# xarray-contrib/xeofs

Measured on AMD Instinct MI355X. Metric: EOF randomized-SVD GB/s (algorithmic: 16 passes x n x p x 4 B per fit / fit time), higher is better.
Workload: dtype f32 data, split-fp16 MFMA (f16x3+f16x3), f32 accumulate

## Files before the change

xeofs_amd/csrc/eofx_abi.hip:

```cpp
#include <chrono>
#include "eofx_hfft.hpp"
#include "eofx_kernels.hpp"
#include "eofx_fit.hpp"
#include "eofx_gram.hpp"
#include "eofx_axb_dma.hpp"
#include "eofx_hosteig.hpp"
#include "eofx_hostla.hpp"
#include "eofx_lag.hpp"
#include "eofx_gw.hpp"
#include "eofx_spca.hpp"
#include "eofx_lagcov.hpp"
#include "eofx_lowpass.hpp"
#include "eofx_orderpos.hpp"
#include "eofx_colquad.hpp"
#include "eofx_pairmin.hpp"
#include "eofx_simplex.hpp"
#include "eofx_kmeans.hpp"
#include "eofx_ica.hpp"
#include "eofx_spectral.hpp"
#include "eofx_pcmul.hpp"
#include "eofx_viewcov.hpp"
#include "eofx_lrfill.hpp"
#include "eofx_plans.hpp"
#include "eofx_sketch.hpp"
// ... 536 lines not shown
  const int bx = (int)(M / ATB_BM);
  const bool wide = atb_wide(L) && prec == EOFX_PREC_F16X3;
  if (sym && !(wide && !aff && L == M)) sym = 0;
  const ColTiles tiles = atb_tiles(L, wide);
  const AtbPlan plan = atb_plan(M, K, L, wide);
  int best_s = plan.S;
  int64_t best_kps = plan.kps;
  ArenaScope scope(ctx);
  float* out = C;
  const int s_half = best_s;
  if (A2) best_s *= 2;
  if (best_s > 1) {
    out = arena_alloc<float>(ctx, (size_t)best_s * M * L);
    if (!out && A2) return set_err(ctx, EOFX_ERR_NOMEM, "arena exhausted (two-matrix partials)");
    if (!out) {
      best_s = 1;
      best_kps = K;
      out = C;
    }
  }
  float a_scale = 1.f;
  if (prec == EOFX_PREC_F16X3) {
    if (a_absmax > 0.f && std::isfinite(a_absmax)) {
      int e;
      (void)std::frexp(a_absmax, &e);
      a_scale = std::ldexp(1.f, 14 - e);
    }
    if (!b_absmax_dev && ldb == L && !A2) b_absmax_dev = amax_get(ctx, B);
    if (!b_absmax_dev) {
      unsigned* bm = arena_alloc<unsigned>(ctx, 1);
      if (!bm) return set_err(ctx, EOFX_ERR_NOMEM, "arena exhausted (panel max)");
      HIPCHK(hipMemsetAsync(bm, 0, sizeof(unsigned), ctx->stream));
      const int64_t total4 = K * (L / 4);
      hipLaunchKernelGGL(panel_absmax_kernel, dim3((int)std::max<int64_t>(1, std::min<int64_t>((total4 + 1023) / 1024, 1024))),
                         dim3(256), 0, ctx->stream, B, K, L, (int64_t)ldb, bm);
      KCHK();
      b_absmax_dev = reinterpret_cast<const float*>(bm);
    }
  }
  unsigned* amax_out = (prec == EOFX_PREC_F16X3 && !sym && !wide && !A2) ? amax_new(ctx, C) : (amax_forget(ctx, C), nullptr);
  hipEvent_t ev0 = nullptr, ev1 = nullptr;
  if (ctx->profile) {
    HIPCHK(hipEventCreate(&ev0));
    HIPCHK(hipEventCreate(&ev1));
    HIPCHK(hipEventRecord(ev0, ctx->stream));
  }
  if (prec == EOFX_PREC_F64) {
    double* outd = nullptr;
    if (best_s > 1) {
      outd = arena_alloc<double>(ctx, (size_t)best_s * M * L);
      if (!outd) return set_err(ctx, EOFX_ERR_NOMEM, "arena exhausted (float64 partials)");
    }
    for (int i = 0; i < tiles.n; ++i) {
      const ColTile& t = tiles.t[i];
      if (t.width == 64)
        hipLaunchKernelGGL(atb_f64_kernel<2>, dim3(bx, best_s, t.count), dim3(512), 0, ctx->stream, A, lda, B, ldb, C, outd, L, M, K,
                           best_kps, t.col_base);
      else
        hipLaunchKernelGGL(atb_f64_kernel<1>, dim3(bx, best_s, t.count), dim3(512), 0, ctx->stream, A, lda, B, ldb, C, outd, L, M, K,
                           best_kps, t.col_base);
      KCHK();
    }
    if (ctx->profile) {
      HIPCHK(hipEventRecord(ev1, ctx->stream));
      ctx->prof_events.emplace_back(ev0, ev1);
      ctx->prof_flops += 2.0 * (double)K * (double)M * (double)L;
      ctx->prof_bytes += (double)K * (double)M * 4.0 * tiles.columns();
    }
    if (outd) {
      const int64_t count = M * L;
      hipLaunchKernelGGL(splitk_reduce_f64_kernel, dim3((int)std::min<int64_t>((count + 255) / 256, 8192)), dim3(256), 0, ctx->stream,
                         outd, C, count, best_s);
      KCHK();
    }
    return EOFX_OK;
  }
  unsigned* amax_direct = best_s == 1 ? amax_out : nullptr;
  PlaneOut po_{nullptr, 0, 0.f};
  const PlaneOut* po = nullptr;
  if (planes && aff && !sym && !A2 && best_s == 1 && amax_direct && planes->bound > 0.f && std::isfinite(planes->bound)) {
    const int64_t K_all = round_up(aff->cols, AXB_KG);
    if (K_all <= M && axb_planes_reserve(ctx, axb_planes_bytes(K_all, L))) {
      po_ = {ctx->axb_planes, K_all, planes->bound};
      po = &po_;
      if (L % 64)
        HIPCHK(hipMemsetAsync(reinterpret_cast<char*>(ctx->axb_planes) + (size_t)(L / 64) * (K_all / AXB_KG) * AXB_PAIR_BYTES, 0,
                              (size_t)(K_all / AXB_KG) * AXB_PAIR_BYTES, ctx->stream));
      if (!planes->keep_f32 && !plane_check_on(ctx)) out = nullptr;
    }
  }
  for (int i = 0; i < tiles.n; ++i) {
    const ColTile& t = tiles.t[i];
    const dim3 grid(bx, best_s, t.count);
    if (t.width >= 96)
      launch_atb_variant<4>(prec, grid, ctx->stream, A, lda, B, ldb, out, L, M, K, best_kps, t.col_base, a_scale, b_absmax_dev, aff, A2, B2, s_half,
                            sym, amax_direct, t.width, po);
    else if (t.width == 64)
      launch_atb_variant<2>(prec, grid, ctx->stream, A, lda, B, ldb, out, L, M, K, best_kps, t.col_base, a_scale, b_absmax_dev, aff, A2, B2, s_half,
                            sym, amax_direct, 128, po);
    else
      launch_atb_variant<1>(prec, grid, ctx->stream, A, lda, B, ldb, out, L, M, K, best_kps, t.col_base, a_scale, b_absmax_dev, aff, A2, B2, s_half,
                            sym, amax_direct, 128, po);
    KCHK();
  }
  if (po) {
    ctx->planes_known.panel = C;
    ctx->planes_known.L = L;
    ctx->planes_known.K_all = po->rows;
    ctx->planes_known.bound = po->bound;
    ctx->planes_known.f32 = out != nullptr;
    ++ctx->plane_produced[0];
  }
  if (ctx->profile) {
    HIPCHK(hipEventRecord(ev1, ctx->stream));
    ctx->prof_events.emplace_back(ev0, ev1);
    ctx->prof_flops += 2.0 * (double)K * (double)M * (double)L * (A2 ? 2 : 1);
    ctx->prof_bytes += (double)K * (double)M * 4.0 * tiles.columns() * (A2 ? 2 : 1);
  }
  if (best_s > 1) {
    const int64_t count4 = M * L / 4;
    const int blocks = (int)std::min<int64_t>((count4 + 255) / 256, amax_out ? 2048 : 4096);
    hipLaunchKernelGGL(splitk_reduce_kernel, dim3(blocks), dim3(256), 0, ctx->stream, out, C, count4,
                       best_s, amax_out);
    KCHK();
  }
  if (sym) {
    const int nt = (int)((M + 63) / 64);
    hipLaunchKernelGGL(symmetrize_lower_kernel, dim3(nt, nt), dim3(256), 0, ctx->stream, C, M, (int64_t)L);
    KCHK();
  }
  return EOFX_OK;
}


static bool axb_takes_dma(eofx_ctx* ctx, int64_t rows_pad, int64_t K_all) {
  if (ctx->axb_dma < 0) {
    const char* ev = std::getenv("EOFX_AXB_DMA");
    ctx->axb_dma = ev ? (atoi(ev) != 0 ? 2 : 0) : EOFX_AXB_DMA_DEFAULT;
  }
  return ctx->axb_dma == 2 || (ctx->axb_dma == 1 && (double)rows_pad * (double)K_all >= 4.0e9);
}
static bool axb_planes_reserve(eofx_ctx* ctx, size_t need) {
  if (ctx->axb_planes_bytes >= need) return true;
  (void)hipStreamSynchronize(ctx->stream);
  if (ctx->axb_planes) (void)hipFree(ctx->axb_planes);
  ctx->axb_planes = nullptr;
  ctx->axb_planes_bytes = 0;
  ctx->planes_known = {};
  if (hipMalloc((void**)&ctx->axb_planes, need) != hipSuccess) {
    (void)hipGetLastError();
    ctx->axb_planes = nullptr;
    return false;
  }
  ctx->axb_planes_bytes = need;
  return true;
}
static bool plane_check_on(eofx_ctx* ctx) {
  if (ctx->plane_check < 0) {
    const char* ev = std::getenv("EOFX_AXB_CHECK_BOUND");
    ctx->plane_check = ev ? atoi(ev) : 0;
  }
  return ctx->plane_check >= 1;
}
static int plane_bound_check(eofx_ctx* ctx, const float* Y, int64_t K_all, int L, float bound) {
  ArenaScope scope(ctx);
  unsigned* bm = arena_alloc<unsigned>(ctx, 1);
  if (!bm) return set_err(ctx, EOFX_ERR_NOMEM, "arena exhausted (panel max)");
  HIPCHK(hipMemsetAsync(bm, 0, sizeof(unsigned), ctx->stream));
  const int64_t total4 = K_all * (L / 4);
  hipLaunchKernelGGL(panel_absmax_kernel, dim3((int)std::max<int64_t>(1, std::min<int64_t>((total4 + 1023) / 1024, 1024))),
                     dim3(256), 0, ctx->stream, Y, K_all, L, (int64_t)L, bm);
  KCHK();
  float mx = 0.f;
  HIPCHK(hipMemcpyAsync(&mx, bm, sizeof(float), hipMemcpyDeviceToHost, ctx->stream));
  HIPCHK(hipStreamSynchronize(ctx->stream));
  ++ctx->plane_checked;
  if (ctx->plane_check >= 2) fprintf(stderr, "eofx: X Y pass over produced planes: bound %g, max |panel| %g, bound / max %g\n", (double)bound, (double)mx, mx > 0.f ? (double)bound / (double)mx : 0.0);
  if (!(mx <= bound)) return set_err(ctx, EOFX_ERR_LINALG, "panel maximum %g above the bound %g its fp16 planes were split with", (double)mx, (double)bound);
  if (mx > 0.f) {
    const double slack = (double)bound / (double)mx;
    if (ctx->plane_min_slack == 0.0 || slack < ctx->plane_min_slack) ctx->plane_min_slack = slack;
    if (slack > ctx->plane_max_slack) ctx->plane_max_slack = slack;
  }
  return EOFX_OK;
}

static int launch_axb(eofx_ctx* ctx, const float* raw, int64_t ld, int64_t rows, int64_t cols, int64_t rows_pad,
                      const float* aff, int64_t aff_ld, float a_absmax, const float* Y, int L, float* W, bool masked = false,
                      const int* act = nullptr, int64_t n_act = 0) {
  const int64_t K_all = round_up(cols, AXB_KG);
  const int64_t K = (masked && act) ? n_act * AXB_KG : K_all;
  if (K == 0) {
    HIPCHK(hipMemsetAsync(W, 0, sizeof(float) * (size_t)rows_pad * L, ctx->stream));
    amax_forget(ctx, W);
    return EOFX_OK;
  }
  if (L % 32 || L <= 0 || rows_pad % AXB_BM || rows >= ((int64_t)1 << 31) || K_all * L >= ((int64_t)1 << 30) ||
      64 * ld + K_all >= ((int64_t)1 << 30))
    return set_err(ctx, EOFX_ERR_ARG, "axb: bad geometry rows=%lld cols=%lld L=%d", (long long)rows, (long long)cols, L);
  const AtbPlan plan = axb_plan(rows_pad, K);
  const int rt = (int)(rows_pad / AXB_BM);
  const ColTiles tiles = atb_tiles(L, false);
  ArenaScope scope(ctx);
  float* out = W;
  if (plan.S > 1) {
    out = arena_alloc<float>(ctx, (size_t)plan.S * rows_pad * L);
    if (!out) return set_err(ctx, EOFX_ERR_NOMEM, "arena exhausted (in-place product partials)");
  }
  float a_scale = 1.f;
  if (a_absmax > 0.f && std::isfinite(a_absmax)) {
    int e;
    (void)std::frexp(a_absmax, &e);
    a_scale = std::ldexp(1.f, 14 - e);
  }
  const float* bmax = amax_get(ctx, Y);
  if (!bmax) {
    unsigned* bm = arena_alloc<unsigned>(ctx, 1);
    if (!bm) return set_err(ctx, EOFX_ERR_NOMEM, "arena exhausted (panel max)");
    HIPCHK(hipMemsetAsync(bm, 0, sizeof(unsigned), ctx->stream));
    const int64_t total4 = K_all * (L / 4);
    hipLaunchKernelGGL(panel_absmax_kernel, dim3((int)std::max<int64_t>(1, std::min<int64_t>((total4 + 1023) / 1024, 1024))),
                       dim3(256), 0, ctx->stream, Y, K_all, L, (int64_t)L, bm);
    KCHK();
    bmax = reinterpret_cast<const float*>(bm);
  }
  unsigned* amax_out = plan.S > 1 ? amax_new(ctx, W) : (amax_forget(ctx, W), nullptr);
  hipEvent_t ev0 = nullptr, ev1 = nullptr;
  if (ctx->profile) {
    HIPCHK(hipEventCreate(&ev0));
    HIPCHK(hipEventCreate(&ev1));
    HIPCHK(hipEventRecord(ev0, ctx->stream));
  }
  const int gx = plan.S > 1 ? 8 * rt * ((plan.S + 7) / 8) : rt;
  bool dma = axb_takes_dma(ctx, rows_pad, K_all);
  const int ncb = tiles.columns();
  if (dma && !axb_planes_reserve(ctx, axb_planes_bytes(K_all, L))) dma = false;
  const int64_t pairs_all = K_all / AXB_KG;
  const eofx_ctx::PlanesKnown& pk = ctx->planes_known;
  const bool produced = dma && pk.panel == Y && pk.L == L && pk.K_all == K_all && amax_get(ctx, Y) == bmax;
  if (produced) {
    ++ctx->plane_consumed;
    if (pk.f32 && plane_check_on(ctx)) CHK(plane_bound_check(ctx, Y, K_all, L, pk.bound));
  } else if (pk.panel == Y && !pk.f32) {
    return set_err(ctx, EOFX_ERR_ARG, "axb: the panel exists as fp16 planes only and they cannot be used here");
  }
  if (dma && !produced) {
    ctx->planes_known = {};
    hipLaunchKernelGGL(axb_bsplit_kernel, dim3((unsigned)((K_all + 31) / 32), ncb), dim3(256), 0, ctx->stream, Y, L, L, K_all, bmax,
                       ctx->axb_planes);
    KCHK();
  }
  const int* const no_act = nullptr;
  for (int i = 0; i < tiles.n; ++i) {
    const ColTile& t = tiles.t[i];
    const dim3 grid(gx, t.count);
#define EOFX_AXB_ARGS(B, LDB) \
  grid, dim3(256), 0, ctx->stream, raw, ld, (int)rows, cols, aff, aff_ld, B, LDB, out, L, rows_pad, K, plan.kps, plan.S, rt, t.col_base, a_scale, bmax
    if (dma) {
      if (t.width == 64) {
        if (masked) hipLaunchKernelGGL((axb_f16_dma_kernel<4, 0, true>), EOFX_AXB_ARGS(ctx->axb_planes, pairs_all), act);
        else hipLaunchKernelGGL((axb_f16_dma_kernel<4, 0, false>), EOFX_AXB_ARGS(ctx->axb_planes, pairs_all), no_act);
      } else {
        if (masked) hipLaunchKernelGGL((axb_f16_dma_kernel<2, 0, true>), EOFX_AXB_ARGS(ctx->axb_planes, pairs_all), act);
        else hipLaunchKernelGGL((axb_f16_dma_kernel<2, 0, false>), EOFX_AXB_ARGS(ctx->axb_planes, pairs_all), no_act);
      }
    } else if (t.width == 64) {
      if (masked) hipLaunchKernelGGL((axb_f16_kernel<4, 0, true>), EOFX_AXB_ARGS(Y, L), act);
      else hipLaunchKernelGGL(axb_f16_kernel<4>, EOFX_AXB_ARGS(Y, L));
    } else {
      if (masked) hipLaunchKernelGGL((axb_f16_kernel<2, 0, true>), EOFX_AXB_ARGS(Y, L), act);
      else hipLaunchKernelGGL(axb_f16_kernel<2>, EOFX_AXB_ARGS(Y, L));
    }
#undef EOFX_AXB_ARGS
    KCHK();
  }
  if (ctx->profile) {
    HIPCHK(hipEventRecord(ev1, ctx->stream));
    ctx->prof_events.emplace_back(ev0, ev1, 1);
    ctx->prof_flops += 2.0 * (double)K * (double)rows_pad * (double)L;
    ctx->prof_bytes += (double)K * (double)rows * 4.0 * tiles.columns();
  }
  if (plan.S > 1) {
    const int64_t count4 = rows_pad * L / 4;
    hipLaunchKernelGGL(splitk_reduce_kernel, dim3((int)std::min<int64_t>((count4 + 255) / 256, amax_out ? 2048 : 4096)), dim3(256), 0,
                       ctx->stream, out, W, count4, plan.S, amax_out);
    KCHK();
  }
  return EOFX_OK;
}

static int launch_gram(eofx_ctx* ctx, const float* P, int64_t rows, int L, double* G) {
  const int nb = (L + 63) / 64;
  const int nbx = gram_parts(rows, L);
  ArenaScope scope(ctx);
  ARENA(double, part, (size_t)nbx * L * L);
  hipLaunchKernelGGL(gram_mfma_kernel, dim3(nbx, nb * nb), dim3(256), 0, ctx->stream, P, rows, L, part);
  KCHK();
  const int64_t count = (int64_t)L * L;
  hipLaunchKernelGGL(f64_reduce_kernel, dim3((int)((count + 63) / 64)), dim3(256), 0, ctx->stream,
                     part, G, count, nbx);
  KCHK();
  return EOFX_OK;
}
static int launch_matmul(eofx_ctx* ctx, const float* P, int64_t rows, int L, const double* Mx, int Lo,
                         float* out, bool upper = false, int64_t planes_rows = 0, float planes_bound = 0.f) {
  int KW = (int)std::min<int64_t>(round_up(L, 64), 256);
  if (L > 256) {
    static const int kw_env = std::getenv("EOFX_PMM_KW") ? atoi(std::getenv("EOFX_PMM_KW")) : 0;
    if (kw_env == 128 || kw_env == 256) KW = kw_env;
  }
  const size_t smem = (size_t)KW * PMM_LD * sizeof(double);
  if (smem > 64 * 1024)
    HIPCHK(hipFuncSetAttribute(reinterpret_cast<const void*>(panel_matmul_kernel<false>), hipFuncAttributeMaxDynamicSharedMemorySize, (int)smem));
  const int64_t units = (rows + 127) / 128;
  const int64_t gx = L <= KW ? std::min<int64_t>(units, 1024) : units;
  dim3 grid((int)std::max<int64_t>(1, gx), (Lo + 63) / 64);
  unsigned* amax_out = amax_new(ctx, out);
  if (planes_rows > 0 && Lo == L && amax_out && planes_rows % AXB_KG == 0 && planes_rows <= rows && rows % 8 == 0 && planes_bound > 0.f &&
      std::isfinite(planes_bound) && axb_planes_reserve(ctx, axb_planes_bytes(planes_rows, Lo))) {
    if (smem > 64 * 1024)
      HIPCHK(hipFuncSetAttribute(reinterpret_cast<const void*>(panel_matmul_kernel<false, true>), hipFuncAttributeMaxDynamicSharedMemorySize,
                                 (int)smem));
    hipLaunchKernelGGL((panel_matmul_kernel<false, true>), grid, dim3(256), smem, ctx->stream, P, rows, L, Mx, Lo, out, KW, amax_out,
                       (int64_t)0, (int64_t)0, 1, (const float*)nullptr, upper ? 1 : 0, ctx->axb_planes, planes_rows, planes_bound);
    KCHK();
    ctx->planes_known.panel = out;
    ctx->planes_known.L = Lo;
    ctx->planes_known.K_all = planes_rows;
    ctx->planes_known.bound = planes_bound;
    ctx->planes_known.f32 = true;
    ++ctx->plane_produced[1];
    return EOFX_OK;
  }
  hipLaunchKernelGGL(panel_matmul_kernel<false>, grid, dim3(256), smem, ctx->stream, P, rows, L, Mx, Lo, out, KW, amax_out,
                     (int64_t)0, (int64_t)0, 1, (const float*)nullptr, upper ? 1 : 0);
  KCHK();
  return EOFX_OK;
}
static int launch_matmul_gen(eofx_ctx* ctx, const float* P, int64_t ldp, int64_t slab, int cpb, int64_t rows, int L, const double* Mx, int Lo,
                             const float* sub, float* out) {
  const int KW = (int)std::min<int64_t>(round_up(L, 64), 256);
  const size_t smem = (size_t)KW * PMM_LD * sizeof(double);
  if (smem > 64 * 1024)
    HIPCHK(hipFuncSetAttribute(reinterpret_cast<const void*>(panel_matmul_kernel<true>), hipFuncAttributeMaxDynamicSharedMemorySize, (int)smem));
  const int64_t units = (rows + 127) / 128;
  const int64_t gx = L <= KW ? std::min<int64_t>(units, 1024) : units;
  dim3 grid((int)std::max<int64_t>(1, gx), (Lo + 63) / 64);
  hipLaunchKernelGGL(panel_matmul_kernel<true>, grid, dim3(256), smem, ctx->stream, P, rows, L, Mx, Lo, out, KW, amax_new(ctx, out), ldp,
                     slab, cpb, sub);
  KCHK();
  return EOFX_OK;
}
static int launch_xgram(eofx_ctx* ctx, const float* Pa, int64_t lda, int La, const float* Pb, int64_t ldb, int Lb, int64_t rows, double* C) {
  const int nbx = (int)std::max<int64_t>(1, std::min<int64_t>((rows + 127) / 128, std::max<int64_t>(1, ((int64_t)32 << 20) / ((int64_t)La * Lb * 8))));
  ArenaScope scope(ctx);
  ARENA(double, part, (size_t)nbx * La * Lb);
  hipLaunchKernelGGL(xgram_mfma_kernel, dim3(nbx, (La / 64) * (Lb / 64)), dim3(256), 0, ctx->stream, Pa, lda, Pb, ldb, rows, La, Lb, part);
  KCHK();
  const int64_t count = (int64_t)La * Lb;
  hipLaunchKernelGGL(f64_reduce_kernel, dim3((int)((count + 63) / 64)), dim3(256), 0, ctx->stream, part, C, count, nbx);
  KCHK();
  return EOFX_OK;
}

static int launch_rinv(eofx_ctx* ctx, const double* G, int L, int l, double* Rinv);
static size_t matmul_nt_scratch(eofx_ctx* ctx, int64_t rows, int L, int Lo);
static int launch_matmul_nt(eofx_ctx* ctx, const float* P, int64_t rows, int L, const double* Mx, int Lo, float* out);
constexpr float EOFX_CHOLQR_BOUND = 2.f;
static int launch_cholqr(eofx_ctx* ctx, const float* P, int64_t rows, int L, int l, const double* G,
                         float* out, int64_t planes_rows = 0) {
  ArenaScope scope(ctx);
  ARENA(double, Rinv, (size_t)L * L);
  CHK(launch_rinv(ctx, G, L, l, Rinv));
  return launch_matmul(ctx, P, rows, L, Rinv, L, out, true, planes_rows, EOFX_CHOLQR_BOUND);
}

static int launch_colminmax(eofx_ctx* ctx, const float* P, int64_t rows, int L, float* mx, float* mn) {
  const int nparts = (int)std::max<int64_t>(1, std::min<int64_t>((rows + 127) / 128, 1024));
  ArenaScope scope(ctx);
  ARENA(float, pmx, (size_t)nparts * L);
  ARENA(float, pmn, (size_t)nparts * L);
  hipLaunchKernelGGL(colminmax_part_kernel, dim3(nparts, (L + 63) / 64), dim3(256), 0, ctx->stream, P,
                     rows, L, pmx, pmn);
  KCHK();
  hipLaunchKernelGGL(colminmax_final_kernel, dim3((L + 63) / 64), dim3(256), 0, ctx->stream, pmx, pmn,
                     nparts, L, mx, mn);
  KCHK();
  return EOFX_OK;
}

static int export_panel(eofx_ctx* ctx, const float* P, int64_t rows, int L, int k, const double* sign,
                        float* dst) {
  if (!dst) return EOFX_OK;
  ArenaScope scope(ctx);
  double* dsign = nullptr;
  if (sign) {
    dsign = arena_alloc<double>(ctx, k);
    if (!dsign) return set_err(ctx, EOFX_ERR_NOMEM, "arena exhausted (export sign)");
    CHK(copy_in(ctx, dsign, sign, sizeof(double) * k));
  }
  float* tmp = dst;
  const bool dev = is_device_ptr(dst);
  if (!dev) {
    tmp = arena_alloc<float>(ctx, (size_t)rows * k);
    if (!tmp) return set_err(ctx, EOFX_ERR_NOMEM, "arena exhausted (export staging)");
  }
  const int64_t total = rows * k;
  const int blocks = (int)std::min<int64_t>((total + 255) / 256, 8192);
  hipLaunchKernelGGL(panel_export_kernel, dim3(blocks), dim3(256), 0, ctx->stream, P, rows, L, k, dsign,
                     tmp);
  KCHK();
  if (!dev) {
    CHK(copy_out(ctx, dst, tmp, sizeof(float) * total));
    HIPCHK(hipStreamSynchronize(ctx->stream));
  }
  return EOFX_OK;
}

static int import_panel(eofx_ctx* ctx, const float* src, int64_t rows, int l, float* P, int64_t rows_pad,
                        int L) {
  ArenaScope scope(ctx);
  const float* dsrc = src;
  if (!is_device_ptr(src)) {
    float* tmp = arena_alloc<float>(ctx, (size_t)rows * l);
    if (!tmp) return set_err(ctx, EOFX_ERR_NOMEM, "arena exhausted (import staging)");
    CHK(copy_in(ctx, tmp, src, sizeof(float) * rows * l));
    dsrc = tmp;
  }
  const int64_t total = rows_pad * (L / 4);
  const int blocks = (int)std::min<int64_t>((total + 255) / 256, 2048);
  hipLaunchKernelGGL(panel_import_kernel, dim3(blocks), dim3(256), 0, ctx->stream, dsrc, rows, l, P,
                     rows_pad, L, amax_new(ctx, P));
  KCHK();
  if (dsrc != src) HIPCHK(hipStreamSynchronize(ctx->stream));
  return EOFX_OK;
}

static void* pool_take(eofx_ctx* ctx, size_t bytes) {
  for (size_t i = 0; i < ctx->pool.size(); ++i)
    if (ctx->pool[i].second == bytes) {
      void* p = ctx->pool[i].first;
      ctx->pool_bytes -= bytes;
      ctx->pool.erase(ctx->pool.begin() + i);
      return p;
    }
  return nullptr;
}
static void pool_trim(eofx_ctx* ctx) {
  if (ctx->pool.empty()) return;
  (void)hipStreamSynchronize(ctx->stream);
  for (auto& e : ctx->pool) (void)hipFree(e.first);
  ctx->pool.clear();
  ctx->pool_bytes = 0;
}
static void pool_give(eofx_ctx* ctx, void* p, size_t bytes) {
  if (!p) return;
  if (!ctx || bytes > ctx->pool_cap) {
    (void)hipFree(p);
    return;
  }
  constexpr size_t POOL_MAX_ENTRIES = 48, POOL_EVICT_BATCH = 12;
  if (!ctx->pool.empty() && (ctx->pool_bytes + bytes > ctx->pool_cap || ctx->pool.size() >= POOL_MAX_ENTRIES)) {
    (void)hipStreamSynchronize(ctx->stream);
    size_t evicted = 0;
    while (!ctx->pool.empty() && (evicted < POOL_EVICT_BATCH || ctx->pool_bytes + bytes > ctx->pool_cap)) {
      (void)hipFree(ctx->pool.front().first);
      ctx->pool_bytes -= ctx->pool.front().second;
      ctx->pool.erase(ctx->pool.begin());
      ++evicted;
    }
  }
  ctx->pool.emplace_back(p, bytes);
  ctx->pool_bytes += bytes;
}
static hipError_t pool_malloc(eofx_ctx* ctx, void** out, size_t bytes) {
  *out = pool_take(ctx, bytes);
  if (*out) return hipSuccess;
  hipError_t e = hipMalloc(out, bytes);
  if (e != hipSuccess && !ctx->pool.empty()) {
    (void)hipGetLastError();
    pool_trim(ctx);
    e = hipMalloc(out, bytes);
  }
  return e;
}
extern "C" int eofx_ctx_trim(eofx_ctx* ctx) {
  if (!ctx) return EOFX_ERR_ARG;
  (void)hipSetDevice(ctx->device);
  pool_trim(ctx);
  if (ctx->axb_planes) {
    (void)hipStreamSynchronize(ctx->stream);
    (void)hipFree(ctx->axb_planes);
    ctx->axb_planes = nullptr;
    ctx->axb_planes_bytes = 0;
    ctx->planes_known = {};
  }
  return EOFX_OK;
}

static int mat_alloc(eofx_ctx* ctx, int64_t n, int64_t p, eofx_mat** out, bool want_x = true, bool want_xt = true) {
  eofx_mat* m = new eofx_mat();
  m->n = n;
  m->p = p;
  m->n_pad = round_up(n, ATB_BM);
  m->p_pad = round_up(p, ATB_BM);
  const size_t bytes = (size_t)m->n_pad * m->p_pad * sizeof(float);
  hipError_t e = want_x ? pool_malloc(ctx, (void**)&m->X, bytes) : hipSuccess;
  if (e == hipSuccess && want_xt) e = pool_malloc(ctx, (void**)&m->Xt, bytes);
  if (e == hipSuccess) e = pool_malloc(ctx, (void**)&m->absmax_dev, 256);
  if (e == hipSuccess) e = hipMemsetAsync(m->absmax_dev, 0, 256, ctx->stream);
  if (e != hipSuccess) {
    if (m->X) (void)hipFree(m->X);
    if (m->Xt) (void)hipFree(m->Xt);
    delete m;
    (void)hipGetLastError();
    return set_err(ctx, EOFX_ERR_NOMEM, "cannot allocate resident matrix %lld x %lld (2 x %.2f GB): %s",
                   (long long)n, (long long)p, bytes / 1e9, hipGetErrorString(e));
  }
  *out = m;
  return EOFX_OK;
}

extern "C" int eofx_mat_destroy(eofx_ctx* ctx, eofx_mat* m) {
  if (!m) return EOFX_OK;
  const size_t bytes = (size_t)m->n_pad * m->p_pad * sizeof(float);
  if (ctx) {
    (void)hipSetDevice(ctx->device);
    (void)hipStreamSynchronize(ctx->stream);
    if (m->X) pool_give(ctx, m->X, bytes);
    if (m->Xt) pool_give(ctx, m->Xt, bytes);
    if (m->act) pool_give(ctx, m->act, sizeof(int) * (size_t)(round_up(m->p, AXB_KG) / AXB_KG));
    pool_give(ctx, m->absmax_dev, 256);
    if (m->raw_owned) pool_give(ctx, m->raw_owned, m->raw_owned_bytes);
    if (m->rawT) pool_give(ctx, m->rawT, bytes);
  } else {
    if (m->X) (void)hipFree(m->X);
    if (m->Xt) (void)hipFree(m->Xt);
    if (m->act) (void)hipFree(m->act);
    if (m->raw_owned) (void)hipFree(m->raw_owned);
    if (m->rawT) (void)hipFree(m->rawT);
  }
  if (m->aff) {
    const size_t abytes = sizeof(float) * 3 * (size_t)m->p_pad;
    if (ctx) pool_give(ctx, m->aff, abytes);
    else (void)hipFree(m->aff);
  }
  delete m;
  return EOFX_OK;
}
extern "C" int eofx_mat_shape(const eofx_mat* m, int64_t* n, int64_t* p, int64_t* n_pad, int64_t* p_pad) {
  if (!m) return EOFX_ERR_ARG;
  if (n) *n = m->n;
  if (p) *p = m->p;
  if (n_pad) *n_pad = m->n_pad;
  if (p_pad) *p_pad = m->p_pad;
  return EOFX_OK;
}

struct Staged {
  const float* dev = nullptr;
  float* owned = nullptr;
  ~Staged() {
    if (owned) (void)hipFree(owned);
  }
};
static int stage_input(eofx_ctx* ctx, const float* X, size_t count, Staged& st) {
  if (is_device_ptr(X)) {
    st.dev = X;
    return EOFX_OK;
  }
  HIPCHK(hipMalloc((void**)&st.owned, count * sizeof(float)));
  HIPCHK(hipMemcpyAsync(st.owned, X, count * sizeof(float), hipMemcpyHostToDevice, ctx->stream));
  st.dev = st.owned;
  return EOFX_OK;
}

static void adopt_staged(eofx_mat** out, Staged& st, size_t bytes) {
  if (out && *out && (*out)->raw && (*out)->raw == st.owned) {
    (*out)->raw_owned = st.owned;
    (*out)->raw_owned_bytes = bytes;
    st.owned = nullptr;
  }
}

static int launch_apply(eofx_ctx* ctx, const float* Xsrc, int64_t ld_src, const int64_t* row_map,
                        const int64_t* col_map, const double* shift, const double* scale, eofx_mat* m,
                        int* nan_flag, const unsigned* absmax_src = nullptr) {
  dim3 grid((int)(m->p_pad / 64), (int)(m->n_pad / 64));
  const bool vec = apply_vec(col_map != nullptr, ld_src, (uintptr_t)Xsrc % 16 == 0);
  if (vec)
    hipLaunchKernelGGL(apply_kernel<true>, grid, dim3(256), 0, ctx->stream, Xsrc, ld_src, row_map, col_map,
                       shift, scale, m->n, m->p, m->X, m->p_pad, m->Xt, m->n_pad, nan_flag, (const float*)nullptr, (int64_t)0);
  else
    hipLaunchKernelGGL(apply_kernel<false>, grid, dim3(256), 0, ctx->stream, Xsrc, ld_src, row_map, col_map,
                       shift, scale, m->n, m->p, m->X, m->p_pad, m->Xt, m->n_pad, nan_flag, (const float*)nullptr, (int64_t)0);
  KCHK();
  if (absmax_src) {
    HIPCHK(hipMemcpyAsync(m->absmax_dev, absmax_src, sizeof(unsigned), hipMemcpyDeviceToDevice, ctx->stream));
  } else {
    const int64_t total4 = m->n_pad * (m->p_pad / 4);
    hipLaunchKernelGGL(panel_absmax_kernel, dim3((int)std::max<int64_t>(1, std::min<int64_t>((total4 + 1023) / 1024, 1024))), dim3(256), 0,
                       ctx->stream, m->Xt, m->p_pad, (int)m->n_pad, m->n_pad, m->absmax_dev);
    KCHK();
  }
  HIPCHK(hipMemcpyAsync(&m->absmax, m->absmax_dev, sizeof(float), hipMemcpyDeviceToHost, ctx->stream));
  return EOFX_OK;
}

static int ensure_Xt(eofx_ctx* ctx, const eofx_mat* cm) {
  eofx_mat* m = const_cast<eofx_mat*>(cm);
  if (m->Xt) return EOFX_OK;
  if (!m->X && !(m->raw && m->aff)) return set_err(ctx, EOFX_ERR_ARG, "matrix holds no data (raw field released?)");
  const size_t bytes = (size_t)m->n_pad * m->p_pad * sizeof(float);
  if (pool_malloc(ctx, (void**)&m->Xt, bytes) != hipSuccess) {
    (void)hipGetLastError();
    m->Xt = nullptr;
    return set_err(ctx, EOFX_ERR_NOMEM, "cannot allocate the sample-contiguous layout (%.2f GB)", bytes / 1e9);
  }
  if (m->X) {
    hipLaunchKernelGGL(transpose_kernel, dim3((int)(m->p_pad / 64), (int)(m->n_pad / 64)), dim3(256), 0, ctx->stream, m->X,
                       m->p_pad, m->Xt, m->n_pad);
  } else {
    hipLaunchKernelGGL(apply_kernel<true>, dim3((int)(m->p_pad / 64), (int)(m->n_pad / 64)), dim3(256), 0, ctx->stream, m->raw,
                       m->raw_ld, (const int64_t*)nullptr, (const int64_t*)nullptr, (const double*)nullptr, (const double*)nullptr,
                       m->n, m->p, (float*)nullptr, m->p_pad, m->Xt, m->n_pad, (int*)nullptr, (const float*)m->aff, m->p_pad);
  }
  KCHK();
  return EOFX_OK;
}
static int ensure_X(eofx_ctx* ctx, const eofx_mat* cm) {
  eofx_mat* m = const_cast<eofx_mat*>(cm);
  if (m->X) return EOFX_OK;
  CHK(ensure_Xt(ctx, m));
  const size_t bytes = (size_t)m->n_pad * m->p_pad * sizeof(float);
  if (pool_malloc(ctx, (void**)&m->X, bytes) != hipSuccess) {
    (void)hipGetLastError();
    m->X = nullptr;
    return set_err(ctx, EOFX_ERR_NOMEM, "cannot allocate the feature-contiguous layout (%.2f GB)", bytes / 1e9);
  }
  hipLaunchKernelGGL(transpose_kernel, dim3((int)(m->n_pad / 64), (int)(m->p_pad / 64)), dim3(256), 0, ctx->stream, m->Xt,
                     m->n_pad, m->X, m->p_pad);
  KCHK();
  return EOFX_OK;
}
extern "C" int eofx_ctx_set_layout(eofx_ctx* ctx, int keep_raw) {
  if (!ctx || keep_raw < 0 || keep_raw > 3) return EOFX_ERR_ARG;
  ctx->allow_masked = keep_raw == 3;
  if (keep_raw == 3) keep_raw = 2;
  ctx->keep_raw = keep_raw;
  return EOFX_OK;
}
extern "C" int eofx_ctx_set_sample_raw(eofx_ctx* ctx, int on) {
  if (!ctx) return EOFX_ERR_ARG;
  ctx->want_rawT = on != 0;
  return EOFX_OK;
}
extern "C" int eofx_mat_release_raw(eofx_ctx* ctx, eofx_mat* m) {
  if (!ctx || !m) return set_err(ctx, EOFX_ERR_ARG, "bad argument");
  ENTER(ctx);
  if (m->raw && !m->Xt && !m->X) CHK(ensure_Xt(ctx, m));
  HIPCHK(hipStreamSynchronize(ctx->stream));
  if (m->raw_owned) pool_give(ctx, m->raw_owned, m->raw_owned_bytes);
  m->raw_owned = nullptr;
  m->raw_owned_bytes = 0;
  m->raw = nullptr;
  return EOFX_OK;
}
extern "C" int eofx_mat_ensure_sample_layout(eofx_ctx* ctx, eofx_mat* m, int only_if_room, int* built) {
  if (!ctx || !m) return set_err(ctx, EOFX_ERR_ARG, "bad argument");
  ENTER(ctx);
  if (built) *built = m->Xt != nullptr;
  if (m->Xt || m->masked) return EOFX_OK;
  if (only_if_room) {
    size_t free_b = 0, total_b = 0;
    const size_t need_b = (size_t)m->n_pad * m->p_pad * sizeof(float);
    if (hipMemGetInfo(&free_b, &total_b) != hipSuccess) {
      (void)hipGetLastError();
      return EOFX_OK;
    }
    if (free_b + ctx->pool_bytes <= need_b + need_b / 2 + ((size_t)8 << 30)) return EOFX_OK;
  }
  CHK(ensure_Xt(ctx, m));
  if (built) *built = 1;
  return EOFX_OK;
}
extern "C" int eofx_mat_release_sample_layout(eofx_ctx* ctx, eofx_mat* m) {
  if (!ctx || !m) return set_err(ctx, EOFX_ERR_ARG, "bad argument");
// ... 372 lines not shown
  if (n_out) *n_out = ns;
  return EOFX_OK;
}

extern "C" int eofx_resample_f32(eofx_ctx* ctx, const eofx_mat* src, const int64_t* rows, int64_t n_rows,
                                 int center, eofx_mat** out, double* mean, double* total_variance) {
  if (!ctx || !src || !rows || !out || n_rows <= 0) return set_err(ctx, EOFX_ERR_ARG, "bad argument");
  ENTER(ctx);
  for (int64_t i = 0; i < n_rows; ++i)
    if (rows[i] < 0 || rows[i] >= src->n)
      return set_err(ctx, EOFX_ERR_ARG, "row index %lld out of range [0, %lld)", (long long)rows[i], (long long)src->n);
  const int64_t P = src->p;
  CHK(arena_reserve(ctx, colstats_scratch(n_rows, P)));
  ArenaScope scope(ctx);
  PreState ps;
  ARENA(int, cnt, P);
  ARENA(double, dmean, P);
  ARENA(double, dstd, P);
  ARENA(double, dshift, P);
  ARENA(double, dscale, P);
  ARENA(double, dm2, P);
  ARENA(unsigned, dabsmax, 1);
  ARENA(int64_t, drows, n_rows);
  ps = {cnt, dmean, dstd, dshift, dscale, dm2, dabsmax};
  CHK(copy_in(ctx, drows, rows, sizeof(int64_t) * n_rows));
  CHK(ensure_X(ctx, src));
  CHK(run_colstats(ctx, src->X, n_rows, P, center, 0, nullptr, ps, src->p_pad, drows));
  eofx_mat* m = nullptr;
  CHK(mat_alloc(ctx, n_rows, P, &m));
  ARENA(int, flag, 1);
  HIPCHK(hipMemsetAsync(flag, 0, sizeof(int), ctx->stream));
  int rc = launch_apply(ctx, src->X, src->p_pad, drows, nullptr, ps.shift, ps.scale, m, flag, ps.absmax);
  if (rc == EOFX_OK && mean)
    if (hipMemcpyAsync(mean, ps.mean, sizeof(double) * P, hipMemcpyDeviceToHost, ctx->stream) != hipSuccess) rc = EOFX_ERR_HIP;
  if (rc == EOFX_OK && total_variance) {
    FeatSummary fs;
    rc = run_feature_summary(ctx, ps, P, fs);
    if (rc == EOFX_OK) *total_variance = fs.tv;
  }
  if (rc == EOFX_OK && hipStreamSynchronize(ctx->stream) != hipSuccess) rc = EOFX_ERR_HIP;
  if (rc != EOFX_OK) {
    eofx_mat_destroy(ctx, m);
    return rc == EOFX_ERR_HIP ? set_err(ctx, EOFX_ERR_HIP, "resample: HIP failure") : rc;
  }
  *out = m;
  return EOFX_OK;
}

static bool tmul_nt_ok(const eofx_mat* m, int L);
static size_t tmul_nt_scratch(eofx_ctx* ctx, const eofx_mat* m, int L);
static int mat_tmul_nt(eofx_ctx* ctx, const eofx_mat* m, const float* Zn, float* Yp, int L);
static int panel_tmul(eofx_ctx* ctx, const eofx_mat* m, const float* Zn, float* Yp, int L, int prec, const PlaneReq* planes = nullptr) {
  if (prec == EOFX_PREC_F16X3 && tmul_nt_ok(m, L) && tmul_nt_scratch(ctx, m, L) > 0 &&
      ctx->arena_size - ctx->arena_off >= tmul_nt_scratch(ctx, m, L))
    return mat_tmul_nt(ctx, m, Zn, Yp, L);
  if (!m->X && m->raw && prec == EOFX_PREC_F16X3) {
    AffView av;
    av.aff = m->aff;
    av.ld = m->p_pad;
    av.rows = (int)m->n;
    av.cols = m->p;
    av.masked = m->masked;
    return launch_atb(ctx, m->raw, m->raw_ld, round_up(m->n, ATB_KG), m->p_pad, Zn, L, L, Yp, prec, m->absmax, nullptr, &av, nullptr, nullptr, 0,
                      planes);
  }
  CHK(ensure_X(ctx, m));
  return launch_atb(ctx, m->X, m->p_pad, round_up(m->n, ATB_KG), m->p_pad, Zn, L, L, Yp, prec, m->absmax);
}
static int ensure_active_pairs(eofx_ctx* ctx, const eofx_mat* cm) {
  eofx_mat* m = const_cast<eofx_mat*>(cm);
  if (!m->masked || m->n_act >= 0 || !m->aff) return EOFX_OK;
  const int64_t npairs = round_up(m->p, AXB_KG) / AXB_KG;
  std::vector<float> sc((size_t)m->p_pad);
  HIPCHK(hipMemcpyAsync(sc.data(), m->aff + 2 * m->p_pad, sizeof(float) * (size_t)m->p_pad, hipMemcpyDeviceToHost, ctx->stream));
  HIPCHK(hipStreamSynchronize(ctx->stream));
  std::vector<int> list;
  list.reserve((size_t)npairs);
  for (int64_t q = 0; q < npairs; ++q) {
    bool any = false;
    for (int64_t c = q * AXB_KG; c < std::min<int64_t>((q + 1) * AXB_KG, m->p) && !any; ++c) any = sc[(size_t)c] != 0.f;
    if (any) list.push_back((int)q);
  }
  m->n_act = (int64_t)list.size();
  if (m->n_act == npairs || m->n_act == 0) return EOFX_OK;
  if (pool_malloc(ctx, (void**)&m->act, sizeof(int) * (size_t)npairs) != hipSuccess) {
    (void)hipGetLastError();
    m->act = nullptr;
    return EOFX_OK;
  }
  HIPCHK(hipMemcpyAsync(m->act, list.data(), sizeof(int) * list.size(), hipMemcpyHostToDevice, ctx->stream));
  HIPCHK(hipStreamSynchronize(ctx->stream));
  return EOFX_OK;
}

static int64_t panel_mul_plane_rows(eofx_ctx* ctx, const eofx_mat* m, int L, int prec) {
  if (m->Xt || !m->raw || !m->aff || prec != EOFX_PREC_F16X3) return 0;
  if (!m->masked && L >= 96 && !std::getenv("EOFX_NO_WIDE_XT")) return 0;
  const int64_t K_all = round_up(m->p, AXB_KG);
  if (K_all * (int64_t)L >= ((int64_t)1 << 30) || 64 * m->raw_ld + K_all >= ((int64_t)1 << 30)) return 0;
  return axb_takes_dma(ctx, m->n_pad, K_all) ? K_all : 0;
}
static bool panel_tmul_plane_req(eofx_ctx* ctx, const eofx_mat* m, int L, int prec, bool keep_f32, PlaneReq* req) {
  if (m->X || panel_mul_plane_rows(ctx, m, L, prec) == 0) return false;
  const float bound = 2.f * std::sqrt((float)m->n) * m->absmax;
  if (!(bound > 0.f) || !std::isfinite(bound)) return false;
  req->bound = bound;
  req->keep_f32 = keep_f32;
  return true;
}
static int panel_mul(eofx_ctx* ctx, const eofx_mat* m, const float* Yp, float* Wn, int L, int prec) {
  if (!m->Xt && m->raw && m->aff && !m->masked && prec == EOFX_PREC_F16X3 && L >= 96 && !std::getenv("EOFX_NO_WIDE_XT")) {
    size_t free_b = 0, total_b = 0;
    const size_t need_b = (size_t)m->n_pad * m->p_pad * sizeof(float);
    if (hipMemGetInfo(&free_b, &total_b) == hipSuccess && free_b + ctx->pool_bytes > need_b + need_b / 2 + ((size_t)8 << 30))
      CHK(ensure_Xt(ctx, m));
    else
      (void)hipGetLastError();
  }
  if (!m->Xt && m->raw && m->aff && prec == EOFX_PREC_F16X3 &&
      round_up(m->p, AXB_KG) * (int64_t)L < ((int64_t)1 << 30) &&
      64 * m->raw_ld + round_up(m->p, AXB_KG) < ((int64_t)1 << 30)) {
    CHK(ensure_active_pairs(ctx, m));
    return launch_axb(ctx, m->raw, m->raw_ld, m->n, m->p, m->n_pad, m->aff, m->p_pad, m->absmax, Yp, L, Wn, m->masked, m->act,
                      m->n_act);
  }
  CHK(ensure_Xt(ctx, m));
  return launch_atb(ctx, m->Xt, m->n_pad, round_up(m->p, ATB_KG), m->n_pad, Yp, L, L, Wn, prec, m->absmax);
}
static bool valid_prec(int p) {
  return p == EOFX_PREC_F32 || p == EOFX_PREC_BF16X3 || p == EOFX_PREC_BF16X6 || p == EOFX_PREC_F16X3 || p == EOFX_PREC_F64;
}

extern "C" int eofx_ctx_set_precision(eofx_ctx* ctx, int power_passes, int final_passes) {
  if (!ctx || !valid_prec(power_passes) || !valid_prec(final_passes)) return set_err(ctx, EOFX_ERR_ARG, "bad precision");
  ctx->prec_power = power_passes;
  ctx->prec_final = final_passes;
  return EOFX_OK;
}

extern "C" int eofx_panel_tmul_f32(eofx_ctx* ctx, const eofx_mat* m, const float* Zn, float* Yp, int L,
                                   int prec) {
  if (!ctx || !m || !Zn || !Yp || !valid_prec(prec)) return set_err(ctx, EOFX_ERR_ARG, "bad argument");
  ENTER(ctx);
  size_t need = atb_scratch_bytes(m->p_pad, round_up(m->n, ATB_KG), L);
  if (prec == EOFX_PREC_F16X3 && tmul_nt_ok(m, L)) need = std::max(need, tmul_nt_scratch(ctx, m, L));
  CHK(arena_reserve(ctx, need));
  return panel_tmul(ctx, m, Zn, Yp, L, prec);
}
extern "C" int eofx_panel_mul_f32(eofx_ctx* ctx, const eofx_mat* m, const float* Yp, float* Wn, int L,
                                  int prec) {
  if (!ctx || !m || !Wn || !Yp || !valid_prec(prec)) return set_err(ctx, EOFX_ERR_ARG, "bad argument");
  ENTER(ctx);
  CHK(arena_reserve(ctx, atb_scratch_bytes(m->n_pad, round_up(m->p, ATB_KG), L)));
  return panel_mul(ctx, m, Yp, Wn, L, prec);
}
extern "C" int eofx_ctx_plane_stats(eofx_ctx* ctx, int64_t* counts4, double* slack2) {
  if (!ctx) return EOFX_ERR_ARG;
  if (counts4) {
    counts4[0] = ctx->plane_produced[0];
    counts4[1] = ctx->plane_produced[1];
    counts4[2] = ctx->plane_consumed;
    counts4[3] = ctx->plane_checked;
  }
  if (slack2) {
    slack2[0] = ctx->plane_min_slack;
    slack2[1] = ctx->plane_max_slack;
  }
  ctx->plane_produced[0] = ctx->plane_produced[1] = ctx->plane_consumed = ctx->plane_checked = 0;
  ctx->plane_min_slack = ctx->plane_max_slack = 0.0;
  return EOFX_OK;
}
extern "C" int eofx_axb_planes_probe_f32(eofx_ctx* ctx, const eofx_mat* m, const float* Zn, int L, int producer, float bound,
                                         void* planes_prod, void* planes_split, size_t plane_bytes, float* w_prod, float* w_split,
                                         float* w_reg, float* w_max, float* y_out, float* bound_out) {
  if (!ctx || !m || !Zn || !planes_prod || !planes_split || !w_prod || !w_split || !w_reg || !w_max || L <= 0 || L % 32 ||
      (producer != 0 && producer != 1))
    return set_err(ctx, EOFX_ERR_ARG, "bad argument");
  ENTER(ctx);
  const int prec = EOFX_PREC_F16X3;
  const int64_t K_all = panel_mul_plane_rows(ctx, m, L, prec);
  if (K_all == 0 || m->X) return set_err(ctx, EOFX_ERR_ARG, "planes probe: the matrix does not take the in-place LDS-DMA route");
  if (plane_bytes != axb_planes_bytes(K_all, L)) return set_err(ctx, EOFX_ERR_ARG, "planes probe: plane_bytes");
  CHK(arena_reserve(ctx, 2 * (size_t)m->p_pad * L * sizeof(float) + 4 * (size_t)L * L * sizeof(double) + (size_t)(4 * gram_parts(m->p_pad, L) + 1) * L * L * sizeof(double) +
                             std::max(atb_scratch_bytes(m->p_pad, round_up(m->n, ATB_KG), L), atb_scratch_bytes(m->n_pad, K_all, L)) + 65536));
  ArenaScope scope(ctx);
  AmaxScope amax_scope(ctx);
  ARENA(float, Y0, (size_t)m->p_pad * L);
  ARENA(float, Y1, (size_t)m->p_pad * L);
  ARENA(double, G, (size_t)L * L);
  float* Y = Y0;
  PlaneReq req;
  if (producer == 0) {
    if (!panel_tmul_plane_req(ctx, m, L, prec, true, &req)) return set_err(ctx, EOFX_ERR_ARG, "planes probe: no request");
    if (bound > 0.f) req.bound = bound;
    CHK(panel_tmul(ctx, m, Zn, Y0, L, prec, &req));
  } else {
    CHK(panel_tmul(ctx, m, Zn, Y0, L, prec));
    CHK(launch_gram(ctx, Y0, m->p_pad, L, G));
    if (bound > 0.f) {
      ArenaScope inner(ctx);
      ARENA(double, Rinv, (size_t)L * L);
      CHK(launch_rinv(ctx, G, L, L, Rinv));
      CHK(launch_matmul(ctx, Y0, m->p_pad, L, Rinv, L, Y1, true, K_all, bound));
    } else {
      CHK(launch_cholqr(ctx, Y0, m->p_pad, L, L, G, Y1, K_all));
    }
    Y = Y1;
  }
  const eofx_ctx::PlanesKnown pk = ctx->planes_known;
  if (pk.panel != Y || pk.K_all != K_all || pk.L != L) return set_err(ctx, EOFX_ERR_ARG, "planes probe: the producer wrote no planes");
  if (bound_out) *bound_out = pk.bound;
  HIPCHK(hipMemcpyAsync(planes_prod, ctx->axb_planes, plane_bytes, hipMemcpyDeviceToHost, ctx->stream));
  if (y_out) HIPCHK(hipMemcpyAsync(y_out, Y, sizeof(float) * (size_t)m->p_pad * L, hipMemcpyDeviceToDevice, ctx->stream));
  CHK(panel_mul(ctx, m, Y, w_prod, L, prec));
  if (ctx->planes_known.panel != Y) return set_err(ctx, EOFX_ERR_ARG, "planes probe: the planes were not taken as written");
  ctx->planes_known = {};
  HIPCHK(hipMemsetAsync(ctx->axb_planes, 0xff, plane_bytes, ctx->stream));
  CHK(panel_mul(ctx, m, Y, w_split, L, prec));
  HIPCHK(hipMemcpyAsync(planes_split, ctx->axb_planes, plane_bytes, hipMemcpyDeviceToHost, ctx->stream));
  const int dma_mode = ctx->axb_dma;
  ctx->axb_dma = 0;
  int rc = panel_mul(ctx, m, Y, w_reg, L, prec);
  if (rc == EOFX_OK) {
    amax_forget(ctx, Y);
    rc = panel_mul(ctx, m, Y, w_max, L, prec);
  }
  ctx->axb_dma = dma_mode;
  if (rc != EOFX_OK) return rc;
  HIPCHK(hipStreamSynchronize(ctx->stream));
  return EOFX_OK;
}
extern "C" int eofx_panel_gram_f64(eofx_ctx* ctx, const float* P, int64_t rows_pad, int L, double* G) {
  if (!ctx || !P || !G || L % 32) return set_err(ctx, EOFX_ERR_ARG, "bad argument");
  ENTER(ctx);
  CHK(arena_reserve(ctx, (size_t)(4 * gram_parts(rows_pad, L) + 1) * L * L * sizeof(double)));
  return launch_gram(ctx, P, rows_pad, L, G);
}
extern "C" int eofx_panel_cholqr_f32(eofx_ctx* ctx, const float* P, int64_t rows_pad, int L, int l,
                                     const double* G, float* out) {
  if (!ctx || !P || !G || !out || P == out) return set_err(ctx, EOFX_ERR_ARG, "bad argument");
  ENTER(ctx);
  CHK(arena_reserve(ctx, (size_t)2 * L * L * sizeof(double) + (l > 64 ? rinv_blocked_bytes(l) : 0)));
  return launch_cholqr(ctx, P, rows_pad, L, l, G, out);
}
extern "C" int eofx_panel_rinv_f64(eofx_ctx* ctx, const double* G, int L, int l, double* Rinv) {
  if (!ctx || !G || !Rinv || L <= 0 || l <= 0 || l > L || G == Rinv) return set_err(ctx, EOFX_ERR_ARG, "bad argument");
  ENTER(ctx);
  if (l > 64) CHK(arena_reserve(ctx, rinv_blocked_bytes(l)));
  return launch_rinv(ctx, G, L, l, Rinv);
}
extern "C" int eofx_panel_matmul_f32(eofx_ctx* ctx, const float* P, int64_t rows_pad, int L,
                                     const double* M, int Lo, float* out) {
  if (!ctx || !P || !M || !out || P == out) return set_err(ctx, EOFX_ERR_ARG, "bad argument");
  ENTER(ctx);
  if (matmul_nt_ok(rows_pad, L, Lo)) {
    const size_t need = matmul_nt_scratch(ctx, rows_pad, L, Lo);
    if (need && arena_reserve(ctx, need) == EOFX_OK) return launch_matmul_nt(ctx, P, rows_pad, L, M, Lo, out);
  }
  return launch_matmul(ctx, P, rows_pad, L, M, Lo, out);
}
extern "C" int eofx_panel_colminmax_f32(eofx_ctx* ctx, const float* P, int64_t rows, int L, float* mx,
                                        float* mn) {
  if (!ctx || !P || !mx || !mn) return set_err(ctx, EOFX_ERR_ARG, "bad argument");
  if (L <= 0 || L % 4 || rows < 0)
    return set_err(ctx, EOFX_ERR_ARG, "colminmax: L=%d must be a positive multiple of 4, rows=%lld non-negative", L, (long long)rows);
  ENTER(ctx);
  CHK(arena_reserve(ctx, (size_t)2 * 1024 * L * sizeof(float) + 4096));
  return launch_colminmax(ctx, P, rows, L, mx, mn);
}
extern "C" int eofx_panel_export_f32(eofx_ctx* ctx, const float* P, int64_t rows, int L, int k,
                                     const double* sign, float* dst) {
  if (!ctx || !P || !dst || k > L) return set_err(ctx, EOFX_ERR_ARG, "bad argument");
  ENTER(ctx);
  CHK(arena_reserve(ctx, (size_t)rows * k * sizeof(float) + 8192));
  return export_panel(ctx, P, rows, L, k, sign, dst);
}
extern "C" int eofx_panel_import_f32(eofx_ctx* ctx, const float* src, int64_t rows, int l, float* P,
                                     int64_t rows_pad, int L) {
  if (!ctx || !P || !src || l > L || rows > rows_pad) return set_err(ctx, EOFX_ERR_ARG, "bad argument");
  if (L <= 0 || L % 4 || l < 0 || rows < 0)
    return set_err(ctx, EOFX_ERR_ARG, "import: L=%d must be a positive multiple of 4, l=%d and rows=%lld non-negative", L, l, (long long)rows);
  ENTER(ctx);
  CHK(arena_reserve(ctx, (size_t)rows * l * sizeof(float) + 8192));
  return import_panel(ctx, src, rows, l, P, rows_pad, L);
}

struct LinOp {
  int64_t tall, small, tall_pad, small_pad;
  std::function<int(const float*, float*, int, int)> fwd;
  std::function<int(const float*, float*, int, int)> bwd;
  std::function<int(const float*, float*, int, int, bool)> fwd_to_bwd;
  std::function<int64_t(int, int)> bwd_plane_rows;
  std::function<int(double*, int64_t)> reduce_tall_gram;
  std::function<int(double*, int64_t)> reduce_small_gram;
  int64_t rule_tall_pad = 0;
};

struct RsvdOut {
  float* Tvec;
  float* Svec;
  int Lo;
  std::vector<double> s;
  int64_t tall_pad = 0, small_pad = 0;
};

extern "C" int eofx_orth_tall_rule(int64_t tall_rows_pad, int L, int prec_power) {
  return orth_tall_rule(tall_rows_pad, L, prec_power) ? 1 : 0;
}
extern "C" int eofx_peaked_spectrum(const double* G, int ld, int l) {
  if (!G || l <= 0) return 0;
  std::vector<double> A((size_t)l * l), w(l), V((size_t)l * l);
  for (int i = 0; i < l; ++i)
    for (int j = 0; j < l; ++j) A[(size_t)i * l + j] = 0.5 * (G[(size_t)i * ld + j] + G[(size_t)j * ld + i]);
  for (double v : A)
    if (!std::isfinite(v)) return 0;
  if (eofx_host_eigh_f64(A.data(), l, w.data(), V.data()) != EOFX_OK) return 1;
  if (!(w[0] > 0.0)) return 0;
  return hostla::peaked_spectrum(w.data(), l) ? 1 : 0;
}

static int launch_rinv_blocked(eofx_ctx* ctx, const double* G, int L, int l, double* Rinv) {
  const int Lb = (int)round_up(l, 64), nb = Lb / 64;
  ArenaScope scope(ctx);
  ARENA(double, S, (size_t)Lb * Lb);
  ARENA(double, X, (size_t)Lb * Lb);
  ARENA(double, T, (size_t)Lb * Lb / 2 + 64 * 64);
  ARENA(double, d0, Lb);
  hipLaunchKernelGGL(chol_blocked_init_kernel, dim3(512), dim3(256), 0, ctx->stream, G, L, l, S, Lb, d0);
  KCHK();
  HIPCHK(hipMemsetAsync(X, 0, sizeof(double) * (size_t)Lb * Lb, ctx->stream));
  for (int j = 0; j < nb; ++j) {
    const int64_t dj = (int64_t)64 * j * Lb + 64 * j;
    const int lj = std::min(64, l - 64 * j);
    hipLaunchKernelGGL(chol_rinv_kernel, dim3(1), dim3(256), 0, ctx->stream, (const double*)(S + dj), Lb, lj, X + dj, 1e-13,
                       (const double*)(d0 + 64 * j));
    KCHK();
    const int rest = nb - 1 - j;
    if (rest > 0) {
      double* row = S + dj + 64;
      hipLaunchKernelGGL(dgemm64_kernel<true>, dim3(rest, 1), dim3(256), 0, ctx->stream, (const double*)(X + dj), Lb,
                         (const double*)row, Lb, row, Lb, 64, 1.0, 0.0, 0);
      KCHK();
      double* trail = S + dj + (int64_t)64 * Lb + 64;
      hipLaunchKernelGGL(dgemm64_kernel<true>, dim3(rest, rest), dim3(256), 0, ctx->stream, (const double*)row, Lb,
                         (const double*)row, Lb, trail, Lb, 64, -1.0, 1.0, 1);
      KCHK();
    }
  }
  {
    std::vector<int> seg((size_t)nb, 1);
    while (seg.size() > 1) {
      std::vector<int> next;
      const size_t npairs = seg.size() / 2;
      bool uniform = true;
      for (size_t i = 0; i < 2 * npairs; ++i) uniform = uniform && seg[i] == seg[0];
      auto merge = [&](int64_t off, int m1, int m2, int batch, int64_t diag_stride) {
        hipLaunchKernelGGL(dgemm64_kernel<false>, dim3(m2 / 64, m1 / 64, batch), dim3(256), 0, ctx->stream,
                           (const double*)(S + off * Lb + off + m1), Lb, (const double*)(X + (off + m1) * Lb + off + m1), Lb, T, m2, m2, 1.0,
                           0.0, 0, diag_stride, diag_stride, (int64_t)m1 * m2);
        hipLaunchKernelGGL(dgemm64_kernel<false>, dim3(m2 / 64, m1 / 64, batch), dim3(256), 0, ctx->stream,
                           (const double*)(X + off * Lb + off), Lb, (const double*)T, m2, X + off * Lb + off + m1, Lb, m1, -1.0, 0.0, 0,
                           diag_stride, (int64_t)m1 * m2, diag_stride);
      };
      if (uniform && npairs > 0) {
        const int m = 64 * seg[0];
        merge(0, m, m, (int)npairs, (int64_t)2 * m * (Lb + 1));
        KCHK();
        for (size_t i = 0; i < npairs; ++i) next.push_back(2 * seg[0]);
      } else {
        int64_t off = 0;
        for (size_t i = 0; i < npairs; ++i) {
          const int m1 = 64 * seg[2 * i], m2 = 64 * seg[2 * i + 1];
          merge(off, m1, m2, 1, 0);
          KCHK();
          off += m1 + m2;
          next.push_back(seg[2 * i] + seg[2 * i + 1]);
        }
      }
      if (seg.size() & 1) next.push_back(seg.back());
      seg.swap(next);
    }
  }
  hipLaunchKernelGGL(chol_blocked_export_kernel, dim3(512), dim3(256), 0, ctx->stream, (const double*)X, Lb, l, Rinv, L);
  KCHK();
  return EOFX_OK;
}
static int launch_rinv(eofx_ctx* ctx, const double* G, int L, int l, double* Rinv) {
  if (l <= 64) {
    if (L > 64) HIPCHK(hipMemsetAsync(Rinv, 0, sizeof(double) * (size_t)L * L, ctx->stream));
    hipLaunchKernelGGL(chol_rinv_kernel, dim3(1), dim3(256), 0, ctx->stream, G, L, l, Rinv, 1e-13, (const double*)nullptr);
    KCHK();
  } else if (ctx->arena_size - ctx->arena_off >= rinv_blocked_bytes(l) && !std::getenv("EOFX_HOST_RINV")) {
    CHK(launch_rinv_blocked(ctx, G, L, l, Rinv));
  } else {
    std::vector<double> hG((size_t)L * L), hR((size_t)L * L);
    HIPCHK(hipMemcpyAsync(hG.data(), G, sizeof(double) * L * L, hipMemcpyDeviceToHost, ctx->stream));
    HIPCHK(hipStreamSynchronize(ctx->stream));
    hostla::chol_rinv_padded(hG.data(), L, l, hR.data(), 1e-13);
    HIPCHK(hipMemcpyAsync(Rinv, hR.data(), sizeof(double) * L * L, hipMemcpyHostToDevice, ctx->stream));
    HIPCHK(hipStreamSynchronize(ctx->stream));
  }
  return EOFX_OK;
}

constexpr int EOFX_FIT_FALLBACK = 1;
typedef std::function<int(const float*, float*, int)> FirstFwd;
typedef std::function<int(const float*, float*, int)> RangeFinder;
static int rsvd_core(eofx_ctx* ctx, const LinOp& op, int k, int l, int n_iter, const float* omega,
                     RsvdOut& out, const FirstFwd* first_fwd = nullptr, const RangeFinder* range = nullptr) {
  const int L = (int)round_up(l, 32);
  const int Lo = (int)round_up(k, 32);
  AmaxScope amax_scope(ctx);
  ARENA(float, Zs, (size_t)op.small_pad * L);
  ARENA(float, Ws, (size_t)op.small_pad * L);
  ARENA(float, Yt, (size_t)op.tall_pad * L);
  ARENA(float, Qt, (size_t)op.tall_pad * L);
  ARENA(float, Tv, (size_t)op.tall_pad * Lo);
  ARENA(float, Sv, (size_t)op.small_pad * Lo);
  ARENA(double, G, (size_t)L * L);
  ARENA(double, G0, (size_t)L * L);
  ARENA(double, R2, (size_t)L * L);
  ARENA(double, Md, (size_t)L * Lo);
  ARENA(double, Md2, (size_t)L * Lo);
  double* pin = nullptr;
  CHK(pinned_scratch(ctx, &pin));
  if ((size_t)2 * L * L > EOFX_PINNED_DOUBLES) return set_err(ctx, EOFX_ERR_ARG, "internal: sketch too wide for the host scratch");

  CHK(import_panel(ctx, omega, op.small, l, Zs, op.small_pad, L));
  bool first_done = false;
  auto fwd = [&](const float* z, float* y, int prec, int to_bwd = 0) -> int {
    if (first_fwd && !first_done) {
      first_done = true;
      return (*first_fwd)(z, y, L);
    }
    first_done = true;
    if (to_bwd && op.fwd_to_bwd) return op.fwd_to_bwd(z, y, L, prec, to_bwd == 1);
    return op.fwd(z, y, L, prec);
  };
  auto gram_tall = [&](const float* Pn, double* Gout) -> int {
    CHK(launch_gram(ctx, Pn, op.tall_pad, L, Gout));
    return op.reduce_tall_gram ? op.reduce_tall_gram(Gout, (int64_t)L * L) : EOFX_OK;
  };
  auto gram_small = [&](const float* Pn, double* Gout) -> int {
    CHK(launch_gram(ctx, Pn, op.small_pad, L, Gout));
    return op.reduce_small_gram ? op.reduce_small_gram(Gout, (int64_t)L * L) : EOFX_OK;
  };
  const int pp = ctx->prec_power, pf = ctx->prec_final;
  const bool orth_always = orth_tall_rule(op.rule_tall_pad > 0 ? op.rule_tall_pad : op.tall_pad, L, pp);
  bool orth_rest = orth_always;
  hipEvent_t peaked_ev = nullptr;
  bool peaked_pending = false;
  int rc = EOFX_OK;
  for (int it = 0; it < (range ? 0 : n_iter) && rc == EOFX_OK; ++it) {
    rc = fwd(Zs, Yt, pp, it == 0 ? 0 : peaked_pending ? 1 : orth_rest ? 0 : 2);
    if (rc != EOFX_OK) break;
    if (peaked_pending) {
      peaked_pending = false;
      if (hipEventSynchronize(peaked_ev) != hipSuccess) rc = set_err(ctx, EOFX_ERR_HIP, "event wait failed");
      else orth_rest = eofx_peaked_spectrum(pin, L, l) != 0;
      if (rc != EOFX_OK) break;
    }
    if (it == 0 || orth_rest) {
      if ((rc = gram_tall(Yt, G)) != EOFX_OK) break;
      if ((rc = launch_cholqr(ctx, Yt, op.tall_pad, L, l, G, Qt, op.bwd_plane_rows ? op.bwd_plane_rows(L, pp) : 0)) != EOFX_OK) break;
      rc = op.bwd(Qt, Ws, L, pp);
    } else {
      rc = op.bwd(Yt, Ws, L, pp);
    }
    if (rc != EOFX_OK) break;
    const bool ask = it == 0 && !orth_always && n_iter > 1;
    if ((rc = gram_small(Ws, ask ? G0 : G)) != EOFX_OK) break;
    if (ask) {
      if (hipMemcpyAsync(pin, G0, sizeof(double) * L * L, hipMemcpyDeviceToHost, ctx->stream) != hipSuccess ||
          (!peaked_ev && hipEventCreateWithFlags(&peaked_ev, hipEventDisableTiming) != hipSuccess) ||
          hipEventRecord(peaked_ev, ctx->stream) != hipSuccess) {
        rc = set_err(ctx, EOFX_ERR_HIP, "asynchronous Gram download failed");
        break;
      }
      peaked_pending = true;
    }
    rc = launch_cholqr(ctx, Ws, op.small_pad, L, l, ask ? G0 : G, Zs);
  }
  if (peaked_ev) {
    if (peaked_pending) (void)hipEventSynchronize(peaked_ev);
    (void)hipEventDestroy(peaked_ev);
  }
  if (rc != EOFX_OK) return rc;
  if (range) CHK((*range)(Zs, Yt, L));
  else CHK(fwd(Zs, Yt, pp));
  CHK(gram_tall(Yt, G));
  CHK(launch_cholqr(ctx, Yt, op.tall_pad, L, l, G, Qt, op.bwd_plane_rows ? op.bwd_plane_rows(L, pf) : 0));
  CHK(gram_tall(Qt, G));
  CHK(launch_rinv(ctx, G, L, l, R2));
  CHK(op.bwd(Qt, Zs, L, pf));
  CHK(launch_matmul(ctx, Zs, op.small_pad, L, R2, L, Ws));
  CHK(gram_small(Ws, G));
  double* hG = pin;
  double* hR2 = pin + (size_t)L * L;
  HIPCHK(hipMemcpyAsync(hG, G, sizeof(double) * L * L, hipMemcpyDeviceToHost, ctx->stream));
  HIPCHK(hipMemcpyAsync(hR2, R2, sizeof(double) * L * L, hipMemcpyDeviceToHost, ctx->stream));
  HIPCHK(hipStreamSynchronize(ctx->stream));
  std::vector<double> Gl((size_t)l * l), w(l), Uh((size_t)l * l);
  for (int i = 0; i < l; ++i)
    for (int j = 0; j < l; ++j) {
      const double v = 0.5 * (hG[(size_t)i * L + j] + hG[(size_t)j * L + i]);
      if (!std::isfinite(v))
        return set_err(ctx, EOFX_ERR_LINALG,
                       "SVD failed. This may be due to isolated NaN values in the data.");
      Gl[(size_t)i * l + j] = v;
    }
  eofx_host_eigh_f64(Gl.data(), l, w.data(), Uh.data());
  out.s.assign(k, 0.0);
  std::vector<double> M1((size_t)L * Lo, 0.0), M2((size_t)L * Lo, 0.0);
  std::vector<double> invs(k);
  for (int j = 0; j < k; ++j) {
    const double sv = std::sqrt(std::max(w[j], 0.0));
    out.s[j] = sv;
    invs[j] = sv > 0.0 ? 1.0 / sv : 0.0;
  }
  for (int i = 0; i < l; ++i) {
    double* m1 = &M1[(size_t)i * Lo];
    for (int q = 0; q < l; ++q) {
      const double r = hR2[(size_t)i * L + q];
      const double* uq = &Uh[(size_t)q * l];
      for (int j = 0; j < k; ++j) m1[j] += r * uq[j];
    }
    for (int j = 0; j < k; ++j) M2[(size_t)i * Lo + j] = Uh[(size_t)i * l + j] * invs[j];
  }
  HIPCHK(hipMemcpyAsync(Md, M1.data(), sizeof(double) * L * Lo, hipMemcpyHostToDevice, ctx->stream));
  HIPCHK(hipMemcpyAsync(Md2, M2.data(), sizeof(double) * L * Lo, hipMemcpyHostToDevice, ctx->stream));
  CHK(launch_matmul(ctx, Qt, op.tall_pad, L, Md, Lo, Tv));
  CHK(launch_matmul(ctx, Ws, op.small_pad, L, Md2, Lo, Sv));
  HIPCHK(hipStreamSynchronize(ctx->stream));
  out.Tvec = Tv;
  out.Svec = Sv;
  out.Lo = Lo;
  out.tall_pad = op.tall_pad;
  out.small_pad = op.small_pad;
  return EOFX_OK;
}

static int comm_allreduce(eofx_ctx* ctx, void* buf, int64_t count, int dtype, int op);
static int sign_rule(eofx_ctx* ctx, const float* Vpanel, int64_t rows, int Lo, int k,
                     std::vector<double>& sign, bool over_ranks = false) {
  ArenaScope scope(ctx);
  ARENA(float, mx, 2 * (size_t)Lo);
  float* mn = mx + Lo;
  CHK(launch_colminmax(ctx, Vpanel, rows, Lo, mx, mn));
  if (over_ranks) {
    hipLaunchKernelGGL(negate_kernel, dim3(1), dim3(256), 0, ctx->stream, mn, Lo);
    KCHK();
    CHK(comm_allreduce(ctx, mx, 2 * (int64_t)Lo, 0, 1));
  }
  std::vector<float> hmx(Lo), hmn(Lo);
  HIPCHK(hipMemcpyAsync(hmx.data(), mx, sizeof(float) * Lo, hipMemcpyDeviceToHost, ctx->stream));
  HIPCHK(hipMemcpyAsync(hmn.data(), mn, sizeof(float) * Lo, hipMemcpyDeviceToHost, ctx->stream));
  HIPCHK(hipStreamSynchronize(ctx->stream));
  sign.assign(k, 1.0);
  for (int j = 0; j < k; ++j) sign[j] = (std::fabs(hmx[j]) >= std::fabs(hmn[j])) ? 1.0 : -1.0;
  return EOFX_OK;
}

typedef std::function<int(double*, int64_t)> GramReduce;
static int fix_null_columns(eofx_ctx* ctx, float* P, int64_t rows, int64_t rows_pad, int Lo, int k, int first,
                            const GramReduce* reduce = nullptr, int64_t rows_total = -1) {
  if (rows_total < 0) rows_total = rows;
  if (first >= k || rows_total <= first) return EOFX_OK;
  if (!reduce) {
    if (ctx->arena_size - ctx->arena_off < null_repair_bytes(rows_pad, Lo)) return EOFX_OK;
  }
  ArenaScope scope(ctx);
  ARENA(double, G, (size_t)Lo * Lo);
  ARENA(double, Mx, (size_t)Lo * Lo);
  ARENA(float, tmp, (size_t)rows_pad * Lo);
  ARENA(int, dflag, Lo);
  std::vector<double> hG((size_t)Lo * Lo), hM((size_t)Lo * Lo);
  std::vector<int> flag(Lo, 0);
  const int blocks = (int)std::max<int64_t>(1, std::min<int64_t>((rows + 255) / 256, 4096));
  auto gram = [&]() -> int {
    CHK(launch_gram(ctx, P, rows_pad, Lo, G));
    if (reduce && *reduce) CHK((*reduce)(G, (int64_t)Lo * Lo));
    HIPCHK(hipMemcpyAsync(hG.data(), G, sizeof(double) * Lo * Lo, hipMemcpyDeviceToHost, ctx->stream));
    HIPCHK(hipStreamSynchronize(ctx->stream));
    return EOFX_OK;
  };
  auto refill = [&]() -> int {
    HIPCHK(hipMemcpyAsync(dflag, flag.data(), sizeof(int) * Lo, hipMemcpyHostToDevice, ctx->stream));
    hipLaunchKernelGGL(null_fill_kernel, dim3(blocks), dim3(256), 0, ctx->stream, P, rows, Lo, first, k, (const int*)dflag);
    KCHK();
    HIPCHK(hipStreamSynchronize(ctx->stream));
    return EOFX_OK;
  };
  int rounds_done = 0;
  for (int attempt = 0; attempt < 8 && rounds_done < 2; ++attempt) {
    CHK(gram());
    const int verdict = hostla::null_column_transform(hG.data(), Lo, first, k, rounds_done == 0, hM.data(), flag.data());
    if (verdict != hostla::NULLCOL_OK) {
      if (rounds_done > 0) break;
      CHK(refill());
      continue;
    }
    HIPCHK(hipMemcpyAsync(Mx, hM.data(), sizeof(double) * Lo * Lo, hipMemcpyHostToDevice, ctx->stream));
    CHK(launch_matmul(ctx, P, rows_pad, Lo, Mx, Lo, tmp));
    HIPCHK(hipMemcpy2DAsync(P + first, sizeof(float) * Lo, tmp + first, sizeof(float) * Lo, sizeof(float) * (size_t)(k - first), (size_t)rows_pad,
                            hipMemcpyDeviceToDevice, ctx->stream));
    HIPCHK(hipStreamSynchronize(ctx->stream));
    ++rounds_done;
  }
  return EOFX_OK;
}

static int fix_null_modes(eofx_ctx* ctx, const RsvdOut& ro, int64_t tall, int64_t small, int k,
                          const GramReduce* reduce_tall = nullptr, int64_t tall_total = -1,
                          const GramReduce* reduce_small = nullptr, int64_t small_total = -1) {
  int first_null = k;
  const double s0 = ro.s.empty() ? 0.0 : ro.s[0];
  for (int j = k - 1; j >= 0 && !(ro.s[j] > 1e-5 * s0); --j) first_null = j;
  if (first_null < k && s0 >= 0.0 && std::isfinite(s0) && ro.tall_pad >= tall && ro.small_pad >= small) {
    CHK(fix_null_columns(ctx, ro.Tvec, tall, ro.tall_pad, ro.Lo, k, first_null, reduce_tall, tall_total));
    CHK(fix_null_columns(ctx, ro.Svec, small, ro.small_pad, ro.Lo, k, first_null, reduce_small, small_total));
  }
  return EOFX_OK;
}

struct FactorShards {
  const GramReduce* reduce_tall = nullptr;
  int64_t tall_total = -1;
  const GramReduce* reduce_small = nullptr;
  int64_t small_total = -1;
};
static int rsvd_finish(eofx_ctx* ctx, const RsvdOut& ro, bool right_is_tall, int64_t left_rows, int64_t right_rows, int k, int flip,
                       float* left, float* s, float* right, double s_divisor = 1.0, const FactorShards* shards = nullptr,
                       std::vector<double>* sign_out = nullptr) {
  const int64_t tall = right_is_tall ? right_rows : left_rows, small = right_is_tall ? left_rows : right_rows;
  const FactorShards local, &sh = shards ? *shards : local;
  CHK(fix_null_modes(ctx, ro, tall, small, k, sh.reduce_tall, sh.tall_total, sh.reduce_small, sh.small_total));
  const float* Rp = right_is_tall ? ro.Tvec : ro.Svec;
  const float* Lp = right_is_tall ? ro.Svec : ro.Tvec;
  std::vector<double> sign;
  if (flip) CHK(sign_rule(ctx, Rp, right_rows, ro.Lo, k, sign, shards != nullptr));
  CHK(export_panel(ctx, Lp, left_rows, ro.Lo, k, flip ? sign.data() : nullptr, left));
  CHK(export_panel(ctx, Rp, right_rows, ro.Lo, k, flip ? sign.data() : nullptr, right));
  if (s) {
    std::vector<float> hs(k);
    for (int j = 0; j < k; ++j) hs[j] = (float)(ro.s[j] / s_divisor);
    HIPCHK(hipMemcpy(s, hs.data(), sizeof(float) * k, hipMemcpyDefault));
  }
  HIPCHK(hipStreamSynchronize(ctx->stream));
  if (sign_out) sign_out->swap(sign);
  return EOFX_OK;
}

static const float* identity_sketch(int64_t small, int l, std::vector<float>& eye) {
  eye.assign((size_t)small * l, 0.f);
  for (int64_t i = 0; i < l; ++i) eye[(size_t)i * l + i] = 1.f;
  return eye.data();
}

extern "C" int eofx_rsvd_f32(eofx_ctx* ctx, const eofx_mat* m, int k, int n_oversamples, int n_iter,
                             const float* omega, int flip, float* U, float* s, float* V) {
  if (!ctx || !m || !omega || k <= 0 || n_oversamples < 0) return set_err(ctx, EOFX_ERR_ARG, "bad argument");
  ENTER(ctx);
  const int64_t n = m->n, p = m->p;
  const RsvdPlan pl = rsvd_plan(n, p, k, n_oversamples, n_iter);
  if (pl.status == RSVD_PLAN_RANK)
    return set_err(ctx, EOFX_ERR_RANK,
                   "n_modes must be less than or equal to the rank of the dataset (rank = %lld).", (long long)pl.r);
  if (pl.status == RSVD_PLAN_WIDTH)
    return set_err(ctx, EOFX_ERR_ARG, "sketch width k+n_oversamples = %d > %d is not supported", pl.l, EOFX_MAX_SKETCH);
  LinOp op;
  if (pl.transposed) {
    op = {p, n, m->p_pad, m->n_pad,
          [&](const float* z, float* y, int L, int pr) { return panel_tmul(ctx, m, z, y, L, pr); },
          [&](const float* y, float* w, int L, int pr) { return panel_mul(ctx, m, y, w, L, pr); }};
    op.fwd_to_bwd = [&](const float* z, float* y, int L, int pr, bool keep) {
      PlaneReq req;
      return panel_tmul(ctx, m, z, y, L, pr, panel_tmul_plane_req(ctx, m, L, pr, keep, &req) ? &req : nullptr);
    };
    op.bwd_plane_rows = [&](int L, int pr) { return panel_mul_plane_rows(ctx, m, L, pr); };
  } else {
    op = {n, p, m->n_pad, m->p_pad,
          [&](const float* z, float* y, int L, int pr) { return panel_mul(ctx, m, z, y, L, pr); },
          [&](const float* y, float* w, int L, int pr) { return panel_tmul(ctx, m, y, w, L, pr); }};
  }
  CHK(arena_reserve(ctx, rsvd_scratch_bytes(op.tall_pad, op.small_pad, pl.l, k)));
  ArenaScope scope(ctx);
  std::vector<float> eye;
  const float* om = pl.full_width ? identity_sketch(op.small, pl.l, eye) : omega;
  RsvdOut ro;
  CHK(rsvd_core(ctx, op, k, pl.l, pl.n_iter, om, ro));
  return rsvd_finish(ctx, ro, pl.transposed, n, p, k, flip, U, s, V);
}

struct FitFirst {
  eofx_ctx* ctx = nullptr;
  const float* Xd = nullptr;
  int64_t n = 0, P = 0, p_pad = 0, n_pad = 0, K = 0;
  int center = 1, standardize = 0, l = 0, L = 0, S = 1;
  AtbPlan plan{1, 0};
  PreState ps{};
  double *dcorr = nullptr, *st_sq = nullptr, *wpart = nullptr, *wbar = nullptr, *wdev = nullptr;
  float *cshift = nullptr, *st_max = nullptr;
  int* dflags = nullptr;
  unsigned* hword = nullptr;
  float a_scale = 1.f;
  bool maybe_masked = false;
  bool sharded = false;
  eofx_mat* m = nullptr;
  FeatSummary fs;
  hipEvent_t ev[4] = {nullptr, nullptr, nullptr, nullptr};
  static constexpr int NPART = 64;
  ~FitFirst() {
    for (int i = 0; i < 4; ++i)
      if (ev[i]) (void)hipEventDestroy(ev[i]);
    if (m) eofx_mat_destroy(ctx, m);
  }
  static size_t bytes(int64_t n, int64_t P, int l) {
    const int L = (int)round_up(l, 32);
    const int64_t p_pad = round_up(P, ATB_BM);
    const int S = atb_plan(p_pad, round_up(n, ATB_KG), L).S;
    return (size_t)S * p_pad * (8 + 4) + (size_t)P * (4 + 6 * 8) + (size_t)p_pad * 4 + (size_t)P * 16 +
           (size_t)(NPART + 1) * L * 8 + (size_t)S * p_pad * L * 4 + (1 << 20);
  }
  int prepare(eofx_ctx* c, const float* X, int64_t n_, int64_t P_, int center_, int standardize_, const double* feat_weights,
              int l_) {
    ctx = c;
    Xd = X;
    n = n_;
    P = P_;
    center = center_;
    standardize = standardize_;
    l = l_;
    L = (int)round_up(l, 32);
    p_pad = round_up(P, ATB_BM);
    n_pad = round_up(n, ATB_BM);
    K = round_up(n, ATB_KG);
    plan = atb_plan(p_pad, K, L);
    S = plan.S;
    ARENA(int, cnt, P);
    ARENA(double, dmean, P);
    ARENA(double, dstd, P);
    ARENA(double, dshift, P);
    ARENA(double, dscale, P);
    ARENA(double, dm2, P);
    ARENA(unsigned, dabsmax, 4);
    ps = {cnt, dmean, dstd, dshift, dscale, dm2, dabsmax};
    ARENA(double, dcorr_, P);
    ARENA(float, cshift_, p_pad);
    ARENA(double, st_sq_, (size_t)S * p_pad);
    ARENA(float, st_max_, (size_t)S * p_pad);
    ARENA(double, wpart_, (size_t)NPART * L);
    ARENA(double, wbar_, L);
    ARENA(int, dflags_, 4);
    dcorr = dcorr_;
    cshift = cshift_;
    st_sq = st_sq_;
    st_max = st_max_;
    wpart = wpart_;
    wbar = wbar_;
    dflags = dflags_;
    if (feat_weights) {
      wdev = arena_alloc<double>(ctx, P);
      if (!wdev) return set_err(ctx, EOFX_ERR_NOMEM, "arena exhausted (weights)");
      CHK(copy_in(ctx, wdev, feat_weights, sizeof(double) * P));
    }
    double* pin = nullptr;
    CHK(pinned_scratch(ctx, &pin));
    hword = reinterpret_cast<unsigned*>(pin + EOFX_PINNED_DOUBLES - 8);
    if (ctx->profile) {
      for (int i = 0; i < 4; ++i) HIPCHK(hipEventCreate(&ev[i]));
      HIPCHK(hipEventRecord(ev[0], ctx->stream));
    }
    HIPCHK(hipMemsetAsync(ps.absmax, 0, sizeof(unsigned) * 4, ctx->stream));
    HIPCHK(hipMemsetAsync(dflags, 0, sizeof(int) * 4, ctx->stream));
    hipLaunchKernelGGL(fit_probe_kernel, dim3((int)((p_pad / 4 + 255) / 256)), dim3(256), 0, ctx->stream, Xd, n, P, P, p_pad, cshift,
                       ps.absmax + 1, dflags);
    KCHK();
    HIPCHK(hipMemcpyAsync(hword, ps.absmax + 1, sizeof(unsigned), hipMemcpyDeviceToHost, ctx->stream));
    HIPCHK(hipMemcpyAsync(hword + 1, dflags, sizeof(int), hipMemcpyDeviceToHost, ctx->stream));
    HIPCHK(hipStreamSynchronize(ctx->stream));
    float est;
    std::memcpy(&est, hword, sizeof(float));
    maybe_masked = (hword[1] & 2) != 0;
    if ((hword[1] & 1) || (maybe_masked && !ctx->allow_masked) || !(est > 0.f) || !std::isfinite(est)) {
      ctx->fit_info[2] = 1.0;
      return EOFX_FIT_FALLBACK;
    }
    int e2;
    (void)std::frexp(est, &e2);
    a_scale = std::ldexp(1.f, 14 - e2 - 6);
    CHK(mat_alloc(ctx, n, P, &m, false, false));
    if (pool_malloc(ctx, (void**)&m->aff, sizeof(float) * 3 * (size_t)p_pad) != hipSuccess) {
      (void)hipGetLastError();
      m->aff = nullptr;
      return set_err(ctx, EOFX_ERR_NOMEM, "cannot allocate the affine map");
    }
    m->raw = Xd;
    m->raw_ld = P;
    m->p_valid = P;
    m->masked = maybe_masked;
    return EOFX_OK;
  }
  int run(const float* Zs, float* Yt, int LL) {
    hipLaunchKernelGGL(panel_colsum_part_kernel, dim3(NPART), dim3(256), 0, ctx->stream, Zs, n, LL, wpart);
    KCHK();
    hipLaunchKernelGGL(panel_colsum_final_kernel, dim3(1), dim3(256), 0, ctx->stream, wpart, NPART, LL, wbar);
    KCHK();
    const float* bmax = amax_get(ctx, Zs);
    if (!bmax) {
      unsigned* bm = ps.absmax + 2;
      const int64_t total4 = n_pad * (LL / 4);
      hipLaunchKernelGGL(panel_absmax_kernel, dim3((int)std::max<int64_t>(1, std::min<int64_t>((total4 + 1023) / 1024, 1024))),
                         dim3(256), 0, ctx->stream, Zs, n_pad, LL, (int64_t)LL, bm);
      KCHK();
      bmax = reinterpret_cast<const float*>(bm);
    }
    float* part = Yt;
    if (S > 1) {
      part = arena_alloc<float>(ctx, (size_t)S * p_pad * LL);
      if (!part) return set_err(ctx, EOFX_ERR_NOMEM, "arena exhausted (first-pass partials)");
    }
    hipEvent_t p0 = nullptr, p1 = nullptr;
    if (ctx->profile) {
      HIPCHK(hipEventRecord(ev[1], ctx->stream));
      HIPCHK(hipEventCreate(&p0));
      HIPCHK(hipEventCreate(&p1));
      HIPCHK(hipEventRecord(p0, ctx->stream));
    }
    const dim3 grid((int)(p_pad / ATB_BM), S, 1);
    if (LL == 64)
      hipLaunchKernelGGL(atb_f16_fit_kernel<2>, grid, dim3(256), 0, ctx->stream, Xd, P, (int)n, P, cshift, Zs, LL, part, LL, p_pad, K,
                         plan.kps, a_scale, bmax, st_sq, st_max, p_pad);
    else
      hipLaunchKernelGGL(atb_f16_fit_kernel<1>, grid, dim3(256), 0, ctx->stream, Xd, P, (int)n, P, cshift, Zs, LL, part, LL, p_pad, K,
                         plan.kps, a_scale, bmax, st_sq, st_max, p_pad);
    KCHK();
    if (ctx->profile) {
      HIPCHK(hipEventRecord(p1, ctx->stream));
      ctx->prof_events.emplace_back(p0, p1, 0);
      ctx->prof_flops += 2.0 * (double)K * (double)p_pad * (double)LL;
      ctx->prof_bytes += (double)n * (double)P * 4.0;
      HIPCHK(hipEventRecord(ev[2], ctx->stream));
    }
    hipLaunchKernelGGL(fit_finalize_kernel, dim3((int)((p_pad + 255) / 256)), dim3(256), 0, ctx->stream, part, p_pad, LL, st_sq, st_max,
                       p_pad, S, Xd, P, n, K - n, P, p_pad, cshift, a_scale, center, standardize, wdev,
                       (double)1.1920928955078125e-07, bmax, ps.cnt, ps.mean, ps.stdv, ps.shift, ps.scale, ps.m2, m->aff, dcorr,
                       ps.absmax, dflags + 1);
    KCHK();
    HIPCHK(hipMemcpyAsync(hword + 2, dflags + 1, sizeof(int), hipMemcpyDeviceToHost, ctx->stream));
    HIPCHK(hipMemcpyAsync(hword + 3, ps.absmax, sizeof(unsigned), hipMemcpyDeviceToHost, ctx->stream));
    HIPCHK(hipMemcpyAsync(m->absmax_dev, ps.absmax, sizeof(unsigned), hipMemcpyDeviceToDevice, ctx->stream));
    hipLaunchKernelGGL(fit_reduce_kernel, dim3((int)std::min<int64_t>((p_pad * (LL / 4) + 255) / 256, 2048)), dim3(256), 0, ctx->stream,
                       part, Yt, p_pad, LL, l, S, P, dcorr, ps.scale, wbar, amax_new(ctx, Yt),
                       maybe_masked ? ps.cnt : (const int*)nullptr);
    KCHK();
    if (ctx->profile) HIPCHK(hipEventRecord(ev[3], ctx->stream));
    CHK(run_feature_summary(ctx, ps, P, fs));
    if (hword[2] & 3) {
      ctx->fit_info[2] = 2.0 + (double)(hword[2] & 3);
      return EOFX_FIT_FALLBACK;
    }
    if (hword[2] & 8) {
      ctx->fit_info[2] = 7.0;
      return EOFX_FIT_FALLBACK;
    }
    if (fs.pv < P) {
      if (!(ctx->allow_masked && (sharded || (10 * fs.pv >= 6 * P && n < fs.pv)))) {
        ctx->fit_info[2] = 6.0;
        return EOFX_FIT_FALLBACK;
      }
      m->p_valid = fs.pv;
      m->masked = true;
    } else {
      m->masked = false;
    }
    std::memcpy(&m->absmax, hword + 3, sizeof(float));
    return EOFX_OK;
  }
  int valid_features(uint8_t* valid_feature) {
    if (!valid_feature) return EOFX_OK;
    if (!m || !m->masked) {
      std::memset(valid_feature, 1, (size_t)P);
      return EOFX_OK;
    }
    std::vector<int> hc((size_t)P);
    HIPCHK(hipMemcpyAsync(hc.data(), ps.cnt, sizeof(int) * P, hipMemcpyDeviceToHost, ctx->stream));
    HIPCHK(hipStreamSynchronize(ctx->stream));
    for (int64_t c = 0; c < P; ++c) valid_feature[c] = hc[(size_t)c] > 0;
    return EOFX_OK;
  }
  int finish(double* mean, double* std_, double* total_variance, eofx_mat** out) {
    if (mean) HIPCHK(hipMemcpyAsync(mean, ps.mean, sizeof(double) * P, hipMemcpyDeviceToHost, ctx->stream));
    if (std_) HIPCHK(hipMemcpyAsync(std_, ps.stdv, sizeof(double) * P, hipMemcpyDeviceToHost, ctx->stream));
    HIPCHK(hipStreamSynchronize(ctx->stream));
    if (total_variance) *total_variance = fs.tv;
    if (ctx->profile) {
      float t01 = 0.f, t23 = 0.f;
      (void)hipEventElapsedTime(&t01, ev[0], ev[1]);
      (void)hipEventElapsedTime(&t23, ev[2], ev[3]);
      ctx->fit_info[1] = (double)t01 + (double)t23;
    }
    *out = m;
    m = nullptr;
    return EOFX_OK;
  }
};

static bool fit_first_eligible(const eofx_ctx* ctx, const float* Xdev, int64_t n, int64_t P, int l) {
  return fit_first_eligible(ctx->keep_raw, ctx->prec_power, ((uintptr_t)Xdev % 16) == 0, n, P, l);
}
static bool fused_fit_eligible(const eofx_ctx* ctx, const float* Xdev, int64_t n, int64_t P, int k, const RsvdPlan& sk, int64_t omega_rows,
                               const float* omega) {
  return fused_fit_eligible(ctx->keep_raw, ctx->prec_power, ((uintptr_t)Xdev % 16) == 0, n, P, k, sk, omega_rows, is_device_ptr(omega));
}

static int fit_fused(eofx_ctx* ctx, const float* Xd, int64_t n, int64_t P, int center, int standardize,
                     const double* feat_weights, int k, int l, int n_iter, const float* omega, int flip,
                     eofx_mat** out, double* mean, double* std_, double* total_variance, float* U, float* s, float* V,
                     uint8_t* valid_feature, int64_t* p_valid) {
  const int64_t p_pad = round_up(P, ATB_BM), n_pad = round_up(n, ATB_BM);
  CHK(arena_reserve(ctx, rsvd_scratch_bytes(p_pad, n_pad, l, k) + FitFirst::bytes(n, P, l)));
  ArenaScope scope(ctx);
  FitFirst ff;
  int rc = ff.prepare(ctx, Xd, n, P, center, standardize, feat_weights, l);
  if (rc != EOFX_OK) return rc;
  FirstFwd first = [&](const float* Zs, float* Yt, int LL) -> int { return ff.run(Zs, Yt, LL); };
  const eofx_mat* m = ff.m;
  LinOp op = {P, n, p_pad, n_pad,
              [&](const float* z, float* y, int LL, int pr) { return panel_tmul(ctx, m, z, y, LL, pr); },
              [&](const float* y, float* w, int LL, int pr) { return panel_mul(ctx, m, y, w, LL, pr); }};
  op.fwd_to_bwd = [&](const float* z, float* y, int LL, int pr, bool keep) {
    PlaneReq req;
    return panel_tmul(ctx, m, z, y, LL, pr, panel_tmul_plane_req(ctx, m, LL, pr, keep, &req) ? &req : nullptr);
  };
  op.bwd_plane_rows = [&](int LL, int pr) { return panel_mul_plane_rows(ctx, m, LL, pr); };
  RsvdOut ro;
  rc = rsvd_core(ctx, op, k, l, n_iter, omega, ro, &first);
  if (rc != EOFX_OK) return rc;
  CHK(rsvd_finish(ctx, ro, true, n, P, k, flip, U, s, V));
  CHK(ff.valid_features(valid_feature));
  if (p_valid) *p_valid = ff.m->masked ? ff.m->p_valid : P;
  return ff.finish(mean, std_, total_variance, out);
}

struct FitIO {
  Staged& st;
  int64_t n, P;
  int center, standardize;
  const double* feat_weights;
  int check_nans;
  eofx_mat** out;
  double *mean, *std_;
  uint8_t *valid_feature, *valid_sample;
  int64_t *n_out, *p_out;
  double* total_variance;
  int* fused;
};
static int fit_fused_done(eofx_ctx* ctx, const FitIO& io, int64_t pv) {
  adopt_staged(io.out, io.st, (size_t)io.n * io.P * sizeof(float));
  if (io.valid_sample) std::memset(io.valid_sample, 1, (size_t)io.n);
  if (io.n_out) *io.n_out = io.n;
  if (io.p_out) *io.p_out = pv;
  if (io.fused) *io.fused = 1;
  ctx->fit_info[0] = 1.0;
  return EOFX_OK;
}
static int destroy_keep_err(eofx_ctx* ctx, eofx_mat* m, int rc) {
  const std::string keep = ctx->err;
  eofx_mat_destroy(ctx, m);
  ctx->err = keep;
  return rc;
}
template <class FollowUp>
static int fit_two_step(eofx_ctx* ctx, const FitIO& io, FollowUp&& follow_up) {
  eofx_mat* m = nullptr;
  int64_t ns = 0, pv = 0;
  CHK(eofx_preprocess_f32(ctx, io.st.dev, io.n, io.P, io.center, io.standardize, io.feat_weights, io.check_nans, &m, io.mean, io.std_,
                          io.valid_feature, io.valid_sample, &ns, &pv, io.total_variance));
  adopt_staged(&m, io.st, (size_t)io.n * io.P * sizeof(float));
  if (io.n_out) *io.n_out = ns;
  if (io.p_out) *io.p_out = pv;
  const int rc = follow_up(m, ns);
  if (rc != EOFX_OK) return destroy_keep_err(ctx, m, rc);
  *io.out = m;
  return EOFX_OK;
}

extern "C" int eofx_fit_first_f32(eofx_ctx* ctx, const float* X, int64_t n, int64_t P, int center, int standardize,
                                  const double* feat_weights, int check_nans, const float* Zn, int L, int l, float* Yp,
                                  eofx_mat** out, double* mean, double* std_, uint8_t* valid_feature, uint8_t* valid_sample,
                                  int64_t* n_out, int64_t* p_out, double* total_variance, int* fused) {
  if (!ctx || !X || !out || !Zn || !Yp || n <= 0 || P <= 0 || L <= 0 || L % 32 || l <= 0 || l > L)
    return set_err(ctx, EOFX_ERR_ARG, "bad argument");
  ENTER(ctx);
  if (fused) *fused = 0;
  ctx->fit_info[0] = ctx->fit_info[1] = ctx->fit_info[2] = 0.0;
  Staged st;
  CHK(stage_input(ctx, X, (size_t)n * P, st));
  const FitIO io{st, n, P, center, standardize, feat_weights, check_nans, out, mean, std_, valid_feature, valid_sample, n_out, p_out,
                 total_variance, fused};
  if (fit_first_eligible(ctx, st.dev, n, P, l) && round_up(l, 32) == L) {
    CHK(arena_reserve(ctx, FitFirst::bytes(n, P, l) + atb_scratch_bytes(round_up(P, ATB_BM), round_up(n, ATB_KG), L)));
    ArenaScope scope(ctx);
    FitFirst ff;
    int rc = ff.prepare(ctx, st.dev, n, P, center, standardize, feat_weights, l);
    if (rc == EOFX_OK) rc = ff.run(Zn, Yp, L);
    if (rc < 0) return rc;
    if (rc == EOFX_OK) {
      CHK(ff.valid_features(valid_feature));
      const int64_t pv_fused = ff.m->masked ? ff.m->p_valid : P;
      CHK(ff.finish(mean, std_, total_variance, out));
      return fit_fused_done(ctx, io, pv_fused);
    }
  } else {
    ctx->fit_info[2] = -1.0;
  }
  return fit_two_step(ctx, io, [&](eofx_mat* m, int64_t ns) {
    return ns == n ? eofx_panel_tmul_f32(ctx, m, Zn, Yp, L, ctx->prec_power) : EOFX_OK;
  });
}

extern "C" int eofx_fit_f32(eofx_ctx* ctx, const float* X, int64_t n, int64_t P, int center, int standardize,
                            const double* feat_weights, int check_nans, int k, int n_oversamples, int n_iter,
                            const float* omega, int64_t omega_rows, int flip, eofx_mat** out, double* mean, double* std_,
                            uint8_t* valid_feature, uint8_t* valid_sample, int64_t* n_out, int64_t* p_out,
                            double* total_variance, float* U, float* s, float* V, int* fused) {
  if (!ctx || !X || !out || !omega || n <= 0 || P <= 0 || k <= 0 || n_oversamples < 0)
    return set_err(ctx, EOFX_ERR_ARG, "bad argument");
  ENTER(ctx);
  if (fused) *fused = 0;
  ctx->fit_info[0] = ctx->fit_info[1] = ctx->fit_info[2] = 0.0;
  Staged st;
  CHK(stage_input(ctx, X, (size_t)n * P, st));
  const FitIO io{st, n, P, center, standardize, feat_weights, check_nans, out, mean, std_, valid_feature, valid_sample, n_out, p_out,
                 total_variance, fused};
  const RsvdPlan pl = rsvd_plan(n, P, k, n_oversamples, n_iter);
  if (fused_fit_eligible(ctx, st.dev, n, P, k, pl, omega_rows, omega)) {
    int64_t pv_fused = P;
    const int rc = fit_fused(ctx, st.dev, n, P, center, standardize, feat_weights, k, pl.l, pl.n_iter, omega, flip, out, mean, std_,
                             total_variance, U, s, V, valid_feature, &pv_fused);
    if (rc < 0) return rc;
    if (rc == EOFX_OK) return fit_fused_done(ctx, io, pv_fused);
  } else {
    ctx->fit_info[2] = -1.0;
  }
  return fit_two_step(ctx, io, [&](eofx_mat* m, int64_t) {
    const int64_t small = std::min(m->n, m->p);
    if (omega_rows < small)
      return set_err(ctx, EOFX_ERR_ARG, "omega has %lld rows, the compacted matrix needs %lld", (long long)omega_rows, (long long)small);
    return eofx_rsvd_f32(ctx, m, k, n_oversamples, n_iter, omega, flip, U, s, V);
  });
}

struct RcclApi {
  void* lib = nullptr;
  int (*get_unique_id)(void*) = nullptr;
  int (*comm_init_rank)(void**, int, ncclUniqueIdCompat, int) = nullptr;
  int (*allreduce)(const void*, void*, size_t, int, int, void*, hipStream_t) = nullptr;
  int (*comm_destroy)(void*) = nullptr;
  const char* (*errstr)(int) = nullptr;
};
static int rccl_open(eofx_ctx* ctx, RcclApi& api) {
  static RcclApi cached;
  if (!cached.lib) {
    void* h = nullptr;
    for (const char* name : {"librccl.so.1", "librccl.so"})
      if (!h) h = dlopen(name, RTLD_NOW | RTLD_NOLOAD);
    if (!h)
      if (const char* ev = std::getenv("EOFX_RCCL_LIB")) h = dlopen(ev, RTLD_NOW | RTLD_GLOBAL);
    for (const char* name : {"librccl.so.1", "/opt/rocm/lib/librccl.so.1", "librccl.so"})
      if (!h) h = dlopen(name, RTLD_NOW | RTLD_GLOBAL);
    if (!h) return set_err(ctx, EOFX_ERR_HIP, "cannot open librccl (%s); set EOFX_RCCL_LIB", dlerror());
    cached.lib = h;
    cached.get_unique_id = reinterpret_cast<int (*)(void*)>(dlsym(h, "ncclGetUniqueId"));
    cached.comm_init_rank = reinterpret_cast<int (*)(void**, int, ncclUniqueIdCompat, int)>(dlsym(h, "ncclCommInitRank"));
    cached.allreduce = reinterpret_cast<int (*)(const void*, void*, size_t, int, int, void*, hipStream_t)>(dlsym(h, "ncclAllReduce"));
    cached.comm_destroy = reinterpret_cast<int (*)(void*)>(dlsym(h, "ncclCommDestroy"));
    cached.errstr = reinterpret_cast<const char* (*)(int)>(dlsym(h, "ncclGetErrorString"));
    if (!cached.get_unique_id || !cached.comm_init_rank || !cached.allreduce || !cached.comm_destroy) {
      cached = RcclApi();
      return set_err(ctx, EOFX_ERR_HIP, "librccl lacks ncclGetUniqueId / ncclCommInitRank / ncclAllReduce / ncclCommDestroy");
    }
  }
  api = cached;
  return EOFX_OK;
}
extern "C" int eofx_comm_unique_id(char* id128) {
  if (!id128) return EOFX_ERR_ARG;
  RcclApi api;
  CHK(rccl_open(nullptr, api));
  ncclUniqueIdCompat id;
  if (api.get_unique_id(&id) != 0) return EOFX_ERR_HIP;
  std::memcpy(id128, id.internal, 128);
  return EOFX_OK;
}
extern "C" int eofx_ctx_comm_clear(eofx_ctx* ctx) {
  if (!ctx) return EOFX_ERR_ARG;
  if (!ctx->comm) return EOFX_OK;
  (void)hipSetDevice(ctx->device);
  (void)hipStreamSynchronize(ctx->stream);
  for (auto& e : ctx->comm->events) {
    (void)hipEventDestroy(e.first);
    (void)hipEventDestroy(e.second);
  }
  if (ctx->comm->comm && ctx->comm->p_destroy) (void)ctx->comm->p_destroy(ctx->comm->comm);
  delete ctx->comm;
  ctx->comm = nullptr;
  return EOFX_OK;
}
extern "C" int eofx_ctx_comm_init_rccl(eofx_ctx* ctx, const char* id128, int world, int rank) {
  if (!ctx || !id128 || world < 1 || rank < 0 || rank >= world) return set_err(ctx, EOFX_ERR_ARG, "bad argument");
  ENTER(ctx);
  CHK(eofx_ctx_comm_clear(ctx));
  RcclApi api;
  CHK(rccl_open(ctx, api));
  ncclUniqueIdCompat id;
  std::memcpy(id.internal, id128, 128);
  void* comm = nullptr;
  const int rc = api.comm_init_rank(&comm, world, id, rank);
  if (rc != 0 || !comm)
    return set_err(ctx, EOFX_ERR_HIP, "ncclCommInitRank(world %d, rank %d) failed: %s", world, rank, api.errstr ? api.errstr(rc) : "?");
  auto* c = new EofxComm();
  c->world = world;
  c->rank = rank;
  c->lib = api.lib;
  c->comm = comm;
  c->p_allreduce = api.allreduce;
  c->p_destroy = api.comm_destroy;
  c->p_errstr = api.errstr;
  ctx->comm = c;
  return EOFX_OK;
}
extern "C" int eofx_ctx_comm_set_callback(eofx_ctx* ctx, eofx_allreduce_fn fn, void* user, int world, int rank) {
  if (!ctx || !fn || world < 1 || rank < 0 || rank >= world) return set_err(ctx, EOFX_ERR_ARG, "bad argument");
  CHK(eofx_ctx_comm_clear(ctx));
  auto* c = new EofxComm();
  c->world = world;
  c->rank = rank;
  c->fn = fn;
  c->user = user;
  ctx->comm = c;
  return EOFX_OK;
}
extern "C" int eofx_ctx_comm_stats(eofx_ctx* ctx, int64_t* calls, int64_t* bytes, double* ms) {
  if (!ctx) return EOFX_ERR_ARG;
  double t = 0.0;
  if (ctx->comm) {
    ENTER(ctx);
    HIPCHK(hipStreamSynchronize(ctx->stream));
    for (auto& e : ctx->comm->events) {
      float dt = 0.f;
      (void)hipEventElapsedTime(&dt, e.first, e.second);
      t += dt;
      (void)hipEventDestroy(e.first);
      (void)hipEventDestroy(e.second);
    }
    ctx->comm->events.clear();
  }
  if (calls) *calls = ctx->comm ? ctx->comm->calls : 0;
  if (bytes) *bytes = ctx->comm ? ctx->comm->bytes : 0;
  if (ms) *ms = t;
  if (ctx->comm) ctx->comm->calls = ctx->comm->bytes = 0;
  return EOFX_OK;
}
static int comm_allreduce(eofx_ctx* ctx, void* buf, int64_t count, int dtype, int op) {
  EofxComm* c = ctx->comm;
  if (!c) return EOFX_OK;
  static const int esize[3] = {4, 8, 4};
  c->calls += 1;
  c->bytes += count * esize[dtype];
  hipEvent_t e0 = nullptr, e1 = nullptr;
  if (ctx->profile) {
    HIPCHK(hipEventCreate(&e0));
    HIPCHK(hipEventCreate(&e1));
    HIPCHK(hipEventRecord(e0, ctx->stream));
  }
  if (c->fn) {
    if (c->fn(c->user, buf, count, dtype, op, (void*)ctx->stream) != 0)
      return set_err(ctx, EOFX_ERR_HIP, "the all-reduce callback failed");
  } else {
    static const int nccl_type[3] = {7, 8, 2};
    static const int nccl_op[3] = {0, 2, 3};
    const int rc = c->p_allreduce(buf, buf, (size_t)count, nccl_type[dtype], nccl_op[op], c->comm, ctx->stream);
    if (rc != 0) return set_err(ctx, EOFX_ERR_HIP, "ncclAllReduce failed: %s", c->p_errstr ? c->p_errstr(rc) : "?");
  }
  if (ctx->profile) {
    HIPCHK(hipEventRecord(e1, ctx->stream));
    c->events.emplace_back(e0, e1);
  }
  return EOFX_OK;
}
static int comm_vote(eofx_ctx* ctx, int local, int* global) {
  *global = local;
  if (!ctx->comm) return EOFX_OK;
  ArenaScope scope(ctx);
  ARENA(int, d, 4);
  HIPCHK(hipMemcpyAsync(d, &local, sizeof(int), hipMemcpyHostToDevice, ctx->stream));
  CHK(comm_allreduce(ctx, d, 1, 2, 1));
  HIPCHK(hipMemcpyAsync(global, d, sizeof(int), hipMemcpyDeviceToHost, ctx->stream));
  HIPCHK(hipStreamSynchronize(ctx->stream));
  return EOFX_OK;
}

static int comm_agree(eofx_ctx* ctx, int rc_local, int local_state, const char* what, int* verdict) {
  const std::string err_local = rc_local < 0 ? ctx->err : std::string();
  CHK(comm_vote(ctx, rc_local < 0 ? 2 : local_state, verdict));
  if (*verdict != 2) return EOFX_OK;
  return rc_local < 0 ? (ctx->err = err_local, rc_local) : set_err(ctx, EOFX_ERR_HIP, "%s failed on another rank", what);
}

static int comm_sum_i64(eofx_ctx* ctx, int64_t local, int64_t* global) {
  *global = local;
  if (!ctx->comm) return EOFX_OK;
  ArenaScope scope(ctx);
  ARENA(double, d, 2);
  const double v = (double)local;
  double r = 0.0;
  HIPCHK(hipMemcpyAsync(d, &v, sizeof(double), hipMemcpyHostToDevice, ctx->stream));
  CHK(comm_allreduce(ctx, d, 1, 1, 0));
  HIPCHK(hipMemcpyAsync(&r, d, sizeof(double), hipMemcpyDeviceToHost, ctx->stream));
  HIPCHK(hipStreamSynchronize(ctx->stream));
  *global = (int64_t)std::llround(r);
  return EOFX_OK;
}

extern "C" int eofx_ctx_comm_selftest(eofx_ctx* ctx, int* ok) {
  if (!ctx || !ok) return set_err(ctx, EOFX_ERR_ARG, "bad argument");
  *ok = 0;
  if (!ctx->comm) return set_err(ctx, EOFX_ERR_ARG, "no communicator attached");
  ENTER(ctx);
  CHK(arena_reserve(ctx, 4096));
  ArenaScope scope(ctx);
  ARENA(double, d, 8);
  const int world = ctx->comm->world, rank = ctx->comm->rank;
  const float vf = (float)(rank + 1);
  const double vd = (double)(rank + 1);
  const int vi = rank + 1;
  float* f = reinterpret_cast<float*>(d);
  double* dd = d + 2;
// ... 3050 lines not shown
```

xeofs_amd/csrc/eofx_fit.hpp:

```cpp
#pragma once
#include "eofx_kernels.hpp"

namespace eofx {

__global__ __launch_bounds__(256) void fit_probe_kernel(const float* __restrict__ X, int64_t n, int64_t P, int64_t ld,
                                                         int64_t p_pad, float* __restrict__ cshift,
                                                         unsigned* __restrict__ est, int* __restrict__ flags) {
  const int64_t c = ((int64_t)blockIdx.x * 256 + threadIdx.x) * 4;
  float m = 0.f;
  bool bad = false, cand = false;
  if (c < P) {
    f32x4 v[9];
#pragma unroll
    for (int t = 0; t < 9; ++t) {
      const int64_t r = t == 8 ? n - 1 : (n * t) / 8;
      v[t] = *reinterpret_cast<const f32x4*>(X + (r < n ? r : n - 1) * ld + c);
    }
    f32x4 c0 = {0.f, 0.f, 0.f, 0.f};
    int nn[4] = {0, 0, 0, 0};
#pragma unroll
    for (int t = 0; t < 9; ++t) {
      c0 += v[t];
#pragma unroll
      for (int e = 0; e < 4; ++e) nn[e] += v[t][e] != v[t][e];
    }
    c0 *= (1.f / 9.f);
#pragma unroll
    for (int e = 0; e < 4; ++e)
      if (nn[e] == 9) {
        cand = true;
        c0[e] = NAN;
      } else if (!(fabsf(c0[e]) < INFINITY)) {
        bad = true;
        c0[e] = 0.f;
      }
    *reinterpret_cast<f32x4*>(cshift + c) = c0;
#pragma unroll
    for (int t = 0; t < 9; ++t)
#pragma unroll
      for (int e = 0; e < 4; ++e) m = fmaxf(m, fabsf(v[t][e] - c0[e]));
  } else if (c < p_pad) {
    *reinterpret_cast<f32x4*>(cshift + c) = f32x4{0.f, 0.f, 0.f, 0.f};
  }
#pragma unroll
  for (int o = 32; o > 0; o >>= 1) m = fmaxf(m, __shfl_xor(m, o));
  const int anybad = (__any(bad) ? 1 : 0) | (__any(cand) ? 2 : 0);
  if ((threadIdx.x & 63) == 0) {
    if (m > 0.f) atomicMax(est, __float_as_uint(m));
    if (anybad) atomicOr(flags, anybad);
  }
}

constexpr int FIT_FLUSH = 16;
constexpr float FIT_ONE = 8192.f;

template <int NB>
__global__ __launch_bounds__(256, 2) void atb_f16_fit_kernel(const float* __restrict__ A, int64_t lda, int a_rows,
                                                              int64_t a_cols, const float* __restrict__ cshift,
                                                              const float* __restrict__ B, int ldb,
                                                              float* __restrict__ C, int ldc, int64_t M, int64_t K,
                                                              int64_t k_per_split, float a_scale,
                                                              const float* __restrict__ b_absmax,
                                                              double* __restrict__ st_sq,
                                                              float* __restrict__ st_max, int64_t st_ld) {
  __shared__ __attribute__((aligned(16))) _Float16 Bs[2][2][2][32 * NB][8];
  __shared__ double Sq[4][256];
  const int tid = threadIdx.x;
  const int lane = tid & 63;
  const int wave = tid >> 6;
  const int li = lane & 31, lh = lane >> 5;
  const int64_t m0 = (int64_t)blockIdx.x * ATB_BM + wave * ATB_WM;
  const int64_t kb = (int64_t)blockIdx.y * k_per_split;
  const int64_t ke = (kb + k_per_split < K) ? kb + k_per_split : K;
  const int nchunks = (int)((ke - kb) / ATB_KC);
  const float b_scale = f16_scale_for(*b_absmax);
  const float out_scale = 1.f / (a_scale * b_scale);

  f32x16 acc[4][NB];
#pragma unroll
  for (int j = 0; j < 4; ++j)
#pragma unroll
    for (int b = 0; b < NB; ++b)
#pragma unroll
      for (int r = 0; r < 16; ++r) acc[j][b][r] = 0.f;
#pragma unroll
  for (int j = 0; j < 4; ++j) Sq[j][tid] = 0.0;
  float qa[4] = {0.f, 0.f, 0.f, 0.f};
  float mall = 0.f;

  const bool colok = m0 + 4 * li < a_cols;
  const float* Ap = A + (colok ? m0 + 4 * li : 0);
  f32x4 cs_ = {0.f, 0.f, 0.f, 0.f};
  if (colok) cs_ = *reinterpret_cast<const f32x4*>(cshift + m0 + 4 * li);
  const float asc_ = colok ? a_scale : 0.f;
  f32x4 ncs_ = -cs_ * asc_;
#pragma unroll
  for (int e = 0; e < 4; ++e)
    if (cs_[e] != cs_[e]) ncs_[e] = INFINITY;
  float m1 = -1.f;
  asm volatile("" : "+v"(m1));
  constexpr int CP = 16 * NB;
  const bool b_odd = (tid >> 4) & 1;
  int b_off, b_w0, b_w1, b_r0;
  bool b_loader, b_ones;
  {
    const int tp_ = tid & 3, lh_ = (tid >> 4) & 1;
    const int cp_ = ((tid >> 2) & 3) | ((tid >> 5) << 2);
    b_loader = cp_ < CP;
    b_ones = cp_ == CP - 1;
    b_r0 = (int)kb + 4 * tp_ + lh_;
    b_off = (4 * tp_ + lh_) * ldb + 2 * cp_;
    const int w_ = ((lh_ * 32 * NB + 2 * cp_) * 8 + 2 * tp_) * 2;
    b_w0 = w_ + 16 * lh_;
    b_w1 = w_ + 16 * (1 - lh_);
  }
  char* const Bsb = reinterpret_cast<char*>(&Bs[0][0][0][0][0]);
  constexpr int B_PLANE = 2 * 32 * NB * 8 * 2, B_BUF = 2 * B_PLANE;

  f32x4 a0[8], a1[8];
  f32x4 bn = {0.f, 0.f, 0.f, 0.f};
#define EOFX_FIT_LOAD_B(chunk)                                                                   \
  do {                                                                                           \
    if (b_loader) {                                                                              \
      const float* bp_ = B + (kb + (int64_t)(chunk) * ATB_KC) * ldb + b_off;                       \
      const f32x2 lo_ = *reinterpret_cast<const f32x2*>(bp_);                                    \
      const f32x2 hi_ = *reinterpret_cast<const f32x2*>(bp_ + 2 * ldb);                          \
      bn = f32x4{lo_[0], lo_[1], hi_[0], hi_[1]};                                                \
      if (b_ones) {                                                                              \
        const int row_ = b_r0 + (chunk) * ATB_KC;                                                \
        bn[1] = row_ < a_rows ? FIT_ONE / b_scale : 0.f;                                         \
        bn[3] = row_ + 2 < a_rows ? FIT_ONE / b_scale : 0.f;                                     \
      }                                                                                          \
    }                                                                                            \
  } while (0)
#define EOFX_FIT_LOAD_A(areg, chunk)                                                             \
  do {                                                                                           \
    const int r0_ = (int)kb + (chunk) * ATB_KC + lh;                                             \
    if ((int)kb + (chunk) * ATB_KC + ATB_KC <= a_rows) {         \
      const float* pa_ = Ap + (int64_t)r0_ * lda;                                                \
      _Pragma("unroll") for (int i = 0; i < 8; ++i) areg[i] =                                    \
          __builtin_nontemporal_load(reinterpret_cast<const f32x4*>(pa_ + (int64_t)(2 * i) * lda)); \
    } else {                                                                                     \
      _Pragma("unroll") for (int i = 0; i < 8; ++i) {                                            \
        const int r_ = r0_ + 2 * i < a_rows ? r0_ + 2 * i : a_rows - 1;                          \
        areg[i] = __builtin_nontemporal_load(reinterpret_cast<const f32x4*>(Ap + (int64_t)r_ * lda)); \
      }                                                                                          \
    }                                                                                            \
  } while (0)
#define EOFX_FIT_STORE_B(buf)                                                                    \
  do {                                                                                           \
    if (b_loader) _Pragma("unroll") for (int e2 = 0; e2 < 2; ++e2) {                             \
      const bool sec_ = (e2 != 0) != b_odd;                                                      \
      const float v0_ = (sec_ ? bn[1] : bn[0]) * b_scale, v1_ = (sec_ ? bn[3] : bn[2]) * b_scale; \
      const fp16x2_t h_ = cvt_pk_rn(v0_, v1_);                                  \
      fp16x2_t l_;                                                                               \
      l_[0] = (__fp16)__builtin_fmaf((float)h_[0], m1, v0_);                                     \
      l_[1] = (__fp16)__builtin_fmaf((float)h_[1], m1, v1_);                                     \
      char* w_ = Bsb + (buf) * B_BUF + (e2 ? b_w1 : b_w0);                                       \
      *reinterpret_cast<unsigned*>(w_) = __builtin_bit_cast(unsigned, h_);                       \
      *reinterpret_cast<unsigned*>(w_ + B_PLANE) = __builtin_bit_cast(unsigned, l_);             \
    }                                                                                            \
  } while (0)
#define EOFX_FIT_CONVERT_J(areg, j, af_)                                                         \
  do {                                                                                           \
    f32x8 x_;                                                                                    \
    _Pragma("unroll") for (int t = 0; t < 8; ++t) {                                              \
      float xv_ = __builtin_fmaf(areg[t][j], asc_, ncs_[j]);                                     \
      asm("" : "+v"(xv_));                                                                       \
      x_[t] = xv_;                                                                               \
    }                                                                                            \
    {                                                                                            \
      float q_ = qa[j], mm_ = mall;                                                              \
      _Pragma("unroll") for (int t = 0; t < 8; ++t) {                                            \
        q_ = __builtin_fmaf(x_[t], x_[t], q_);                                                   \
        mm_ = __builtin_fmaxf(mm_, __builtin_fabsf(x_[t]));        \
      }                                                                                          \
      asm("" : "+v"(q_), "+v"(mm_));                                                             \
      qa[j] = q_;                                                                                \
      mall = mm_;                                                                                \
    }                                                                                            \
    split_f16_mix(x_, m1, af_);                                                                  \
  } while (0)
#define EOFX_FIT_MFMA_J(j, af_)                                                                  \
  _Pragma("unroll") for (int q = 0; q < NB; ++q) {                                               \
    acc[j][q] = __builtin_amdgcn_mfma_f32_32x32x16_f16(af_[1], bf_[0][q], acc[j][q], 0, 0, 0);   \
    acc[j][q] = __builtin_amdgcn_mfma_f32_32x32x16_f16(af_[0], bf_[1][q], acc[j][q], 0, 0, 0);   \
    acc[j][q] = __builtin_amdgcn_mfma_f32_32x32x16_f16(af_[0], bf_[0][q], acc[j][q], 0, 0, 0);   \
  }
#define EOFX_FIT_COMPUTE(areg, buf, refill)                                                      \
  do {                                                                                           \
    f16x8 bf_[2][NB];                                                                            \
    _Pragma("unroll") for (int s = 0; s < 2; ++s) _Pragma("unroll") for (int q = 0; q < NB; ++q) \
        bf_[s][q] = *reinterpret_cast<const f16x8*>(&Bs[buf][s][lh][32 * q + li][0]);            \
    _Pragma("unroll") for (int j = 0; j < 3; ++j) {                                              \
      f16x8 af_[2];                                                                              \
      EOFX_FIT_CONVERT_J(areg, j, af_);                                                          \
      EOFX_FIT_MFMA_J(j, af_)                                                                    \
    }                                                                                            \
    f16x8 al_[2];                                                                                \
    EOFX_FIT_CONVERT_J(areg, 3, al_);                                                            \
    __builtin_amdgcn_sched_barrier(0);                                                           \
    EOFX_FIT_LOAD_A(areg, refill);                                                               \
    __builtin_amdgcn_sched_barrier(0);                                                           \
    EOFX_FIT_MFMA_J(3, al_)                                                                      \
  } while (0)
#define EOFX_FIT_FLUSH()                                                                         \
  do {                                                                                           \
    _Pragma("unroll") for (int j = 0; j < 4; ++j) {                                              \
      (void)__hip_atomic_fetch_add(&Sq[j][tid], (double)qa[j], __ATOMIC_RELAXED, __HIP_MEMORY_SCOPE_WORKGROUP); \
      qa[j] = 0.f;                                                                               \
    }                                                                                            \
  } while (0)

  if (nchunks > 0) {
    EOFX_FIT_LOAD_B(0);
    EOFX_FIT_LOAD_A(a0, 0);
    EOFX_FIT_LOAD_A(a1, 1);
    EOFX_FIT_STORE_B(0);
    __syncthreads();
    for (int c = 0; c < nchunks; c += 2) {
      const int c2 = (c + 2 < nchunks) ? c + 2 : c;
      EOFX_FIT_LOAD_B(c + 1);
      EOFX_FIT_COMPUTE(a0, 0, c2);
      EOFX_FIT_STORE_B(1);
      __syncthreads();
      EOFX_FIT_LOAD_B(c2);
      EOFX_FIT_COMPUTE(a1, 1, c2 + 1);
      EOFX_FIT_STORE_B(0);
      if ((c & (FIT_FLUSH - 2)) == FIT_FLUSH - 2) EOFX_FIT_FLUSH();
      __syncthreads();
    }
  }
  EOFX_FIT_FLUSH();
#undef EOFX_FIT_LOAD_B
#undef EOFX_FIT_LOAD_A
#undef EOFX_FIT_COMPUTE
#undef EOFX_FIT_CONVERT_J
#undef EOFX_FIT_MFMA_J
#undef EOFX_FIT_STORE_B
#undef EOFX_FIT_FLUSH

  float* Cs = C + (int64_t)blockIdx.y * M * ldc;
#pragma unroll
  for (int j = 0; j < 4; ++j)
#pragma unroll
    for (int q = 0; q < NB; ++q)
#pragma unroll
      for (int r = 0; r < 16; ++r) {
        const int ii = (r & 3) + 8 * (r >> 2) + 4 * lh;
        const int64_t m = m0 + 4 * ii + j;
        Cs[m * ldc + 32 * q + li] = acc[j][q][r] * out_scale;
      }
  {
    f64x4 q4;
    f32x4 m4;
#pragma unroll
    for (int j = 0; j < 4; ++j) {
      const double q_ = Sq[j][tid];
      const double qo_ = __shfl_xor(q_, 32);
      const float mo_ = __shfl_xor(mall, 32);
      q4[j] = q_ + qo_;
      m4[j] = fmaxf(mall, mo_);
    }
    if (lh == 0 && colok) {
      const int64_t o = (int64_t)blockIdx.y * st_ld + m0 + 4 * li;
      *reinterpret_cast<f64x4*>(st_sq + o) = q4;
      *reinterpret_cast<f32x4*>(st_max + o) = m4;
    }
  }
}

__global__ __launch_bounds__(256) void fit_finalize_kernel(
    const float* __restrict__ part, int64_t part_rows, int L, const double* __restrict__ st_sq,
    const float* __restrict__ st_max, int64_t st_ld, int splits, const float* __restrict__ X, int64_t ld, int64_t n,
    int64_t extra, int64_t P, int64_t p_pad, const float* __restrict__ cshift, float a_scale, int center, int standardize,
    const double* __restrict__ weights, double eps, const float* __restrict__ b_absmax, int* __restrict__ cnt,
    double* __restrict__ mean, double* __restrict__ stdv, double* __restrict__ shift, double* __restrict__ scale,
    double* __restrict__ m2, float* __restrict__ aff, double* __restrict__ dcorr, unsigned* __restrict__ absmax,
    int* __restrict__ flags) {
  const int64_t c = (int64_t)blockIdx.x * 256 + threadIdx.x;
  float amax = 0.f;
  int fl = 0;
  if (c < P) {
    const double unit = (double)f16_scale_for(*b_absmax) / (double)FIT_ONE;
    double S1 = 0.0, q = 0.0;
    float mx = 0.f;
    for (int sp = 0; sp < splits; ++sp) {
      S1 += (double)part[((int64_t)sp * part_rows + c) * L + (L - 1)];
      q += st_sq[(int64_t)sp * st_ld + c];
      mx = fmaxf(mx, st_max[(int64_t)sp * st_ld + c]);
    }
    S1 *= unit;
    const float cs = cshift[c];
    if (cs != cs) {
      if (!(mx < 60000.f)) fl |= 2;
      fl |= 4;
      const double w = weights ? weights[c] : 1.0;
      cnt[c] = 0;
      mean[c] = NAN;
      stdv[c] = NAN;
      shift[c] = center ? NAN : 0.0;
      scale[c] = (standardize ? NAN : 1.0) * w;
      m2[c] = 0.0;
      dcorr[c] = 0.0;
      aff[c] = 0.f;
      aff[p_pad + c] = 0.f;
      aff[2 * p_pad + c] = 0.f;
    } else {
    if (extra > 0) {
      const float v = __builtin_fmaf(X[(n - 1) * ld + c], a_scale, -cs * a_scale);
      q -= (double)extra * ((double)v * (double)v);
    }
    if (!(fabs(S1) < INFINITY) || !(fabs(q) < INFINITY)) fl |= 1;
    if (!(mx < 60000.f)) fl |= 2;
    const double ia = 1.0 / (double)a_scale;
    const double nn = (double)n;
    const double mu = (double)cs + S1 / nn;
    double M2 = q * ia * ia - S1 * S1 / nn;
    if (!(M2 > 0.0)) M2 = 0.0;
    double sd = sqrt(M2 / nn);
    if (standardize && sd > eps && sd * (double)a_scale < 0.015625) fl |= 8;
    if (sd < eps) sd = eps;
    const double w = weights ? weights[c] : 1.0;
    const double sh = center ? mu : 0.0, sc = (standardize ? 1.0 / sd : 1.0) * w;
    cnt[c] = (int)n;
    mean[c] = mu;
    stdv[c] = sd;
    shift[c] = sh;
    scale[c] = sc;
    m2[c] = M2;
    dcorr[c] = sh - (double)cs;
    float hi, lo;
    aff_split(sh, hi, lo);
    aff[c] = hi;
    aff[p_pad + c] = lo;
    aff[2 * p_pad + c] = (float)sc;
    amax = (float)(((double)mx * ia + fabs(sh - (double)cs)) * fabs(sc) * 1.000001);
    }
  } else if (c < p_pad) {
    aff[c] = 0.f;
    aff[p_pad + c] = 0.f;
    aff[2 * p_pad + c] = 0.f;
  }
#pragma unroll
  for (int o = 32; o > 0; o >>= 1) amax = fmaxf(amax, __shfl_xor(amax, o));
  const int anyfl = (__any(fl & 1) ? 1 : 0) | (__any(fl & 2) ? 2 : 0) | (__any(fl & 4) ? 4 : 0) | (__any(fl & 8) ? 8 : 0);
  if ((threadIdx.x & 63) == 0) {
    if (amax > 0.f && amax < INFINITY) atomicMax(absmax, __float_as_uint(amax));
    if (anyfl) atomicOr(flags, anyfl);
  }
}

__global__ __launch_bounds__(256) void panel_colsum_part_kernel(const float* __restrict__ P, int64_t rows, int L,
                                                                 double* __restrict__ part) {
  __shared__ double red[4][64];
  const int col = threadIdx.x & 63, rq = threadIdx.x >> 6;
  const int64_t per = (rows + gridDim.x - 1) / gridDim.x;
  const int64_t r0 = (int64_t)blockIdx.x * per, r1 = r0 + per < rows ? r0 + per : rows;
  for (int cb = 0; cb < L; cb += 64) {
    double s = 0.0;
    if (cb + col < L)
      for (int64_t r = r0 + rq; r < r1; r += 4) s += (double)P[r * L + cb + col];
    red[rq][col] = s;
    __syncthreads();
    if (rq == 0 && cb + col < L) part[(int64_t)blockIdx.x * L + cb + col] = (red[0][col] + red[1][col]) + (red[2][col] + red[3][col]);
    __syncthreads();
  }
}
__global__ __launch_bounds__(256) void panel_colsum_final_kernel(const double* __restrict__ part, int nparts, int L,
                                                                  double* __restrict__ out) {
  for (int c = threadIdx.x; c < L; c += 256) {
    double s = 0.0;
    for (int p = 0; p < nparts; ++p) s += part[(int64_t)p * L + c];
    out[c] = s;
  }
}

__global__ __launch_bounds__(256) void fit_reduce_kernel(const float* part, float* out, int64_t rows_pad, int L, int l,
                                                          int splits, int64_t P, const double* __restrict__ dcorr,
                                                          const double* __restrict__ scale,
                                                          const double* __restrict__ wbar,
                                                          unsigned* __restrict__ amax_out, const int* __restrict__ cnt = nullptr) {
  const int l4 = L / 4;
  const int quad = threadIdx.x % l4, rslot = threadIdx.x / l4, rper = 256 / l4;
  const int c = 4 * quad;
  const int64_t count4 = rows_pad * l4;
  double w[4];
#pragma unroll
  for (int e = 0; e < 4; ++e) w[e] = c + e < l ? wbar[c + e] : 0.0;
  float m = 0.f;
  for (int64_t j = (int64_t)blockIdx.x * rper + rslot; j < rows_pad; j += (int64_t)gridDim.x * rper) {
    const int64_t i = j * l4 + quad;
    f32x4 o = {0.f, 0.f, 0.f, 0.f};
    if (j < P && !(cnt && cnt[j] == 0)) {
      double s0 = 0, s1 = 0, s2 = 0, s3 = 0;
      for (int s = 0; s < splits; ++s) {
        const f32x4 v = reinterpret_cast<const f32x4*>(part)[(int64_t)s * count4 + i];
        s0 += v[0];
        s1 += v[1];
        s2 += v[2];
        s3 += v[3];
      }
      const double d = dcorr[j], sc = scale[j];
      o[0] = c < l ? (float)((s0 - d * w[0]) * sc) : 0.f;
      o[1] = c + 1 < l ? (float)((s1 - d * w[1]) * sc) : 0.f;
      o[2] = c + 2 < l ? (float)((s2 - d * w[2]) * sc) : 0.f;
      o[3] = c + 3 < l ? (float)((s3 - d * w[3]) * sc) : 0.f;
      m = fmaxf(m, fmaxf(fmaxf(fabsf(o[0]), fabsf(o[1])), fmaxf(fabsf(o[2]), fabsf(o[3]))));
    }
    reinterpret_cast<f32x4*>(out)[i] = o;
  }
  if (amax_out) amax_commit(m, amax_out);
}

__global__ __launch_bounds__(256) void bst_gather_kernel(const float* __restrict__ P, const int64_t* __restrict__ idx,
                                                          int64_t n, int64_t rows_pad, int L, float* __restrict__ out) {
  const int l4 = L / 4;
  const int64_t total = rows_pad * l4;
  for (int64_t t = (int64_t)blockIdx.x * 256 + threadIdx.x; t < total; t += (int64_t)gridDim.x * 256) {
    const int64_t i = t / l4;
    const int q = (int)(t - i * l4);
    f32x4 v = {0.f, 0.f, 0.f, 0.f};
    if (i < n) v = reinterpret_cast<const f32x4*>(P)[idx[i] * l4 + q];
    reinterpret_cast<f32x4*>(out)[t] = v;
  }
}
__global__ __launch_bounds__(256) void bst_segsum_kernel(const float* __restrict__ Z, const int64_t* __restrict__ order,
                                                          const int64_t* __restrict__ rowptr, int64_t n, int64_t rows_pad,
                                                          int L, float* __restrict__ out) {
  const int l4 = L / 4;
  const int64_t total = rows_pad * l4;
  for (int64_t t = (int64_t)blockIdx.x * 256 + threadIdx.x; t < total; t += (int64_t)gridDim.x * 256) {
    const int64_t r = t / l4;
    const int q = (int)(t - r * l4);
    double s0 = 0, s1 = 0, s2 = 0, s3 = 0;
    if (r < n)
      for (int64_t i = rowptr[r]; i < rowptr[r + 1]; ++i) {
        const f32x4 v = reinterpret_cast<const f32x4*>(Z)[order[i] * l4 + q];
        s0 += v[0];
        s1 += v[1];
        s2 += v[2];
        s3 += v[3];
      }
    reinterpret_cast<f32x4*>(out)[t] = f32x4{(float)s0, (float)s1, (float)s2, (float)s3};
  }
}
__global__ __launch_bounds__(256) void bst_rankone_kernel(float* __restrict__ out, const double* __restrict__ colsum,
                                                           const int64_t* __restrict__ rowptr, int64_t n, int L) {
  const int l4 = L / 4;
  const int64_t total = n * l4;
  const double inv = 1.0 / (double)n;
  for (int64_t t = (int64_t)blockIdx.x * 256 + threadIdx.x; t < total; t += (int64_t)gridDim.x * 256) {
    const int64_t r = t / l4;
    const int c = (int)(t - r * l4) * 4;
    const double w = rowptr ? (double)(rowptr[r + 1] - rowptr[r]) * inv : inv;
    f32x4 v = reinterpret_cast<f32x4*>(out)[t];
#pragma unroll
    for (int e = 0; e < 4; ++e) v[e] = (float)((double)v[e] - w * colsum[c + e]);
    reinterpret_cast<f32x4*>(out)[t] = v;
  }
}

}
```

xeofs_amd/csrc/eofx_kernels.hpp:

```cpp
#pragma once
#include <hip/hip_runtime.h>
#include <stdint.h>

#include "eofx_mfma64.hpp"
#include "eofx_plans.hpp"

namespace eofx {

typedef float f32x16 __attribute__((ext_vector_type(16)));
typedef float f32x4 __attribute__((ext_vector_type(4)));
typedef float f32x2 __attribute__((ext_vector_type(2)));

__device__ __forceinline__ void aff_split(double sh, float& hi, float& lo) {
  hi = (float)sh;
  lo = (float)(sh - (double)hi);
}
__device__ __forceinline__ float aff_map(float x, float sh_hi, float sh_lo, float scale) {
  return ((x - sh_hi) - sh_lo) * scale;
}
__device__ __forceinline__ float aff_fma(float x, float sh_hi, float s, float nls) {
  return __builtin_fmaf(x - sh_hi, s, nls);
}

__device__ __forceinline__ void amax_commit(float mx, unsigned* __restrict__ amax_out) {
// ... 1054 lines not shown
    }
  }
}

__global__ __launch_bounds__(256) void f64_reduce_kernel(const double* __restrict__ part,
                                                         double* __restrict__ out, int64_t count,
                                                         int nparts) {
  __shared__ double red[4][64];
  const int li = threadIdx.x & 63, q = threadIdx.x >> 6;
  const int64_t i = (int64_t)blockIdx.x * 64 + li;
  double s = 0;
  if (i < count) {
#pragma unroll 4
    for (int b = q; b < nparts; b += 4) s += part[(int64_t)b * count + i];
  }
  red[q][li] = s;
  __syncthreads();
  if (q == 0 && i < count) out[i] = ((red[0][li] + red[1][li]) + red[2][li]) + red[3][li];
}

__global__ __launch_bounds__(256) void xgram_mfma_kernel(const float* __restrict__ Pa, int64_t lda, const float* __restrict__ Pb,
                                                          int64_t ldb, int64_t rows, int La, int Lb, double* __restrict__ part) {
  const int nbj = Lb / 64;
  const int bi = blockIdx.y / nbj, bj = blockIdx.y % nbj;
  const int lane = threadIdx.x & 63, wave = threadIdx.x >> 6;
  const int lc = lane & 15, lk = lane >> 4;
  const int ca = 64 * bi + 4 * lc, cb = 64 * bj + 4 * lc;
  f64x4 acc[4][4];
#pragma unroll
  for (int x = 0; x < 4; ++x)
#pragma unroll
    for (int y = 0; y < 4; ++y) acc[x][y] = f64x4{0.0, 0.0, 0.0, 0.0};
  const int64_t wstride = (int64_t)gridDim.x * 4 * 4;
  auto fetch = [&](int64_t r0, f32x4& va, f32x4& vb) {
    const int64_t r = r0 + lk;
    va = f32x4{0.f, 0.f, 0.f, 0.f};
    vb = va;
    if (r < rows) {
      va = *reinterpret_cast<const f32x4*>(Pa + r * lda + ca);
      vb = *reinterpret_cast<const f32x4*>(Pb + r * ldb + cb);
    }
  };
  constexpr int XG_PF = 4;
  int64_t r0 = ((int64_t)blockIdx.x * 4 + wave) * 4;
  f32x4 pa[XG_PF], pb[XG_PF];
#pragma unroll
  for (int d = 0; d < XG_PF; ++d) fetch(r0 + d * wstride, pa[d], pb[d]);
  for (; r0 < rows; r0 += XG_PF * wstride) {
#pragma unroll
    for (int d = 0; d < XG_PF; ++d) {
      const f32x4 va = pa[d], vb = pb[d];
      fetch(r0 + (XG_PF + d) * wstride, pa[d], pb[d]);
      __builtin_amdgcn_sched_barrier(0);
#pragma unroll
      for (int x = 0; x < 4; ++x)
#pragma unroll
        for (int y = 0; y < 4; ++y)
          acc[x][y] = __builtin_amdgcn_mfma_f64_16x16x4f64((double)va[x], (double)vb[y], acc[x][y], 0, 0, 0);
    }
  }
  __shared__ double Gs[64][65];
  for (int w = 0; w < 4; ++w) {
    if (wave == w) {
#pragma unroll
      for (int x = 0; x < 4; ++x)
#pragma unroll
        for (int y = 0; y < 4; ++y)
#pragma unroll
          for (int q = 0; q < 4; ++q) {
            const int i = 4 * (lk + 4 * q) + x, j = 4 * lc + y;
            if (w == 0) Gs[i][j] = acc[x][y][q];
            else Gs[i][j] += acc[x][y][q];
          }
    }
    __syncthreads();
  }
  double* G = part + (int64_t)blockIdx.x * (int64_t)La * Lb;
  for (int e = threadIdx.x; e < 64 * 64; e += 256) {
    const int i = e >> 6, j = e & 63;
    G[(int64_t)(64 * bi + i) * Lb + 64 * bj + j] = Gs[i][j];
  }
}

__global__ __launch_bounds__(256) void cproj_embed_kernel(const double* __restrict__ C, int nb, int LP, double* __restrict__ E) {
  const int h = LP / 2;
  const int64_t total = (int64_t)nb * h * h;
  for (int64_t t = (int64_t)blockIdx.x * blockDim.x + threadIdx.x; t < total; t += (int64_t)gridDim.x * blockDim.x) {
    const int b = (int)(t / (h * h)), i = (int)(t / h % h), j = (int)(t % h);
    const double* Cb = C + (int64_t)b * LP * LP;
    double* Eb = E + (int64_t)b * LP * LP;
    const double rr = Cb[i * LP + j], ii = Cb[(h + i) * LP + h + j], ri = Cb[i * LP + h + j], ir = Cb[(h + i) * LP + j];
    const double cr = rr + ii, ci = ri - ir;
    Eb[i * LP + j] = cr;
    Eb[(h + i) * LP + j] = -ci;
    Eb[i * LP + h + j] = ci;
    Eb[(h + i) * LP + h + j] = cr;
  }
}

__device__ __forceinline__ double rl_f64(double v, int lane) {
  const int lo = __builtin_amdgcn_readlane(__double2loint(v), lane);
  const int hi = __builtin_amdgcn_readlane(__double2hiint(v), lane);
  return __hiloint2double(hi, lo);
}

__global__ __launch_bounds__(256) void chol_rinv_kernel(const double* __restrict__ G, int L, int l,
                                                         double* __restrict__ Rinv, double tol,
                                                         const double* __restrict__ d0_ext = nullptr,
                                                         unsigned long long* __restrict__ prof = nullptr) {
#define EOFX_RINV_T(i) do { if (prof && threadIdx.x == 0) prof[i] = wall_clock64(); } while (0)
  EOFX_RINV_T(0);
  __shared__ double A[64][65];
  __shared__ double X[64][65];
  __shared__ double d0s[64], pivs[64];
  __shared__ double Tm[3][16][17];
  __shared__ int dead[64];
  const int tid = threadIdx.x;
  for (int i = tid; i < 64 * 64; i += 256) {
    const int r = i >> 6, c = i & 63;
    double v = (r == c) ? 1.0 : 0.0;
    if (r <= c && c < l) v = G[(int64_t)r * L + c];
    A[r][c] = v;
  }
  if (tid < 64) {
    d0s[tid] = (tid < l) ? (d0_ext ? d0_ext[tid] : G[(int64_t)tid * L + tid]) : 1.0;
    pivs[tid] = 1.0;
    dead[tid] = 0;
  }
  __syncthreads();
  EOFX_RINV_T(1);
  for (int jb = 0; jb < l; jb += 8) {
    const int je = jb + 8;
    unsigned long long tp0 = prof ? wall_clock64() : 0;
    if (tid < 64) {
      const int c = tid;
      double a[8];
#pragma unroll
      for (int u = 0; u < 8; ++u) a[u] = A[jb + u][c];
      const double d0c = d0s[c];
#pragma unroll
      for (int u = 0; u < 8; ++u) {
        const int j = jb + u;
        const double d = rl_f64(a[u], j);
        const double d0 = rl_f64(d0c, j);
        const bool dj = !(d > tol * d0) || !(d0 > 0.0);
        double piv = __builtin_amdgcn_rsq(dj ? 1.0 : d);
        piv = piv * (1.5 - 0.5 * d * piv * piv);
        piv = piv * (1.5 - 0.5 * d * piv * piv);
        if (dj) piv = 0.0;
        if (c == j) {
          dead[j] = dj;
          pivs[j] = dj ? 1.0 : piv;
        }
        a[u] = (c > j) ? a[u] * piv : 0.0;
#pragma unroll
        for (int u2 = u + 1; u2 < 8; ++u2) {
          const double rjr = rl_f64(a[u], jb + u2);
          if (c >= jb + u2) a[u2] -= rjr * a[u];
        }
      }
#pragma unroll
      for (int u = 0; u < 8; ++u)
        if (c > jb + u) A[jb + u][c] = a[u];
    }
    __syncthreads();
    if (prof && tid == 0) prof[5] += wall_clock64() - tp0;
    {
      const int c = tid & 63;
      double rc[8];
#pragma unroll
      for (int u = 0; u < 8; ++u) rc[u] = A[jb + u][c];
#pragma unroll 4
      for (int r = je + (tid >> 6); r < 64; r += 4) {
        double s = 0.0;
#pragma unroll
        for (int u = 0; u < 8; ++u) s += A[jb + u][r] * rc[u];
        if (r <= c) A[r][c] -= s;
      }
    }
    __syncthreads();
  }
  EOFX_RINV_T(2);
  if (tid < 64) {
    const int b16 = (tid >> 4) * 16, cc = tid & 15;
    double x[16];
#pragma unroll
    for (int r = 15; r >= 0; --r) {
      double s = 0.0;
#pragma unroll
      for (int t = r + 1; t < 16; ++t) s += A[b16 + r][b16 + t] * x[t];
      x[r] = (r <= cc) ? (((r == cc) ? 1.0 : 0.0) - s) * pivs[b16 + r] : 0.0;
    }
#pragma unroll
    for (int r = 0; r < 16; ++r) X[b16 + r][b16 + cc] = x[r];
  }
  __syncthreads();
  {
    const int rr = tid >> 4, cc = tid & 15;
    for (int d = 1; d < 4; ++d) {
      for (int i = 0; i + d < 4; ++i) {
        const int j = i + d;
        double t = 0.0;
        for (int k = i + 1; k <= j; ++k)
#pragma unroll 16
          for (int m = 0; m < 16; ++m) t += A[16 * i + rr][16 * k + m] * X[16 * k + m][16 * j + cc];
        Tm[i][rr][cc] = t;
      }
      __syncthreads();
      for (int i = 0; i + d < 4; ++i) {
        const int j = i + d;
        double x = 0.0;
#pragma unroll 16
        for (int m = 0; m < 16; ++m) x += X[16 * i + rr][16 * i + m] * Tm[i][m][cc];
        X[16 * i + rr][16 * j + cc] = -x;
      }
      __syncthreads();
    }
  }
  __syncthreads();
  EOFX_RINV_T(3);
  for (int i = tid; i < 64 * 64; i += 256) {
    const int r = i >> 6, c = i & 63;
    if (r < L && c < L) Rinv[(int64_t)r * L + c] = (r <= c && c < l && !dead[c]) ? X[r][c] : 0.0;
  }
  EOFX_RINV_T(4);
#undef EOFX_RINV_T
}

template <bool TA>
__global__ __launch_bounds__(256) void dgemm64_kernel(const double* __restrict__ A, int lda, const double* B, int ldb,
                                                       double* C, int ldc, int K, double alpha, double beta, int upper,
                                                       int64_t sA = 0, int64_t sB = 0, int64_t sC = 0) {
  __shared__ double As[16][65], Bs[16][65];
  const int bx = blockIdx.x, by = blockIdx.y;
  if (upper && by > bx) return;
  A += (int64_t)blockIdx.z * sA;
  B += (int64_t)blockIdx.z * sB;
  C += (int64_t)blockIdx.z * sC;
  const int tx = threadIdx.x & 15, ty = threadIdx.x >> 4;
  double acc[4][4];
#pragma unroll
  for (int i = 0; i < 4; ++i)
#pragma unroll
    for (int j = 0; j < 4; ++j) acc[i][j] = 0.0;
  for (int k0 = 0; k0 < K; k0 += 16) {
#pragma unroll
    for (int e = 0; e < 4; ++e) {
      const int idx = threadIdx.x + 256 * e;
      if (TA) {
        const int k = idx >> 6, m = idx & 63;
        As[k][m] = A[(int64_t)(k0 + k) * lda + 64 * by + m];
      } else {
        const int m = idx >> 4, k = idx & 15;
        As[k][m] = A[(int64_t)(64 * by + m) * lda + k0 + k];
      }
      const int kb = idx >> 6, n = idx & 63;
      Bs[kb][n] = B[(int64_t)(k0 + kb) * ldb + 64 * bx + n];
    }
    __syncthreads();
#pragma unroll
    for (int k = 0; k < 16; ++k) {
      double a[4], b[4];
#pragma unroll
      for (int i = 0; i < 4; ++i) a[i] = As[k][4 * ty + i];
#pragma unroll
      for (int j = 0; j < 4; ++j) b[j] = Bs[k][4 * tx + j];
#pragma unroll
      for (int i = 0; i < 4; ++i)
#pragma unroll
        for (int j = 0; j < 4; ++j) acc[i][j] = __builtin_fma(a[i], b[j], acc[i][j]);
    }
    __syncthreads();
  }
#pragma unroll
  for (int i = 0; i < 4; ++i)
#pragma unroll
    for (int j = 0; j < 4; ++j) {
      double* c = C + (int64_t)(64 * by + 4 * ty + i) * ldc + 64 * bx + 4 * tx + j;
      *c = beta == 0.0 ? alpha * acc[i][j] : alpha * acc[i][j] + beta * *c;
    }
}

__global__ void chol_blocked_init_kernel(const double* __restrict__ G, int L, int l, double* __restrict__ S, int Lb,
                                          double* __restrict__ d0) {
  const int64_t total = (int64_t)Lb * Lb;
  for (int64_t i = (int64_t)blockIdx.x * blockDim.x + threadIdx.x; i < total; i += (int64_t)gridDim.x * blockDim.x) {
    const int r = (int)(i / Lb), c = (int)(i % Lb);
    double v = (r == c) ? 1.0 : 0.0;
    if (r < l && c < l) v = G[(int64_t)r * L + c];
    S[i] = v;
    if (r == c) d0[r] = v;
  }
}
__global__ void chol_blocked_export_kernel(const double* __restrict__ X, int Lb, int l, double* __restrict__ Rinv, int L) {
  const int64_t total = (int64_t)L * L;
  for (int64_t i = (int64_t)blockIdx.x * blockDim.x + threadIdx.x; i < total; i += (int64_t)gridDim.x * blockDim.x) {
    const int r = (int)(i / L), c = (int)(i % L);
    Rinv[i] = (r <= c && c < l) ? X[(int64_t)r * Lb + c] : 0.0;
  }
}

constexpr int PMM_LD = 66;

template <bool GEN = false, bool PLANES = false>
__global__ __launch_bounds__(256) void panel_matmul_kernel(const float* __restrict__ P,
                                                           int64_t rows, int L,
                                                           const double* __restrict__ Mx, int Lo,
                                                           float* __restrict__ out, int KW,
                                                           unsigned* __restrict__ amax_out = nullptr,
                                                           int64_t ldp = 0, int64_t slab = 0, int cpb = 1,
                                                           const float* __restrict__ sub = nullptr, int upper = 0,
                                                           void* __restrict__ planes = nullptr, int64_t plane_rows = 0,
                                                           float plane_bound = 0.f) {
  static_assert(!(GEN && PLANES), "the plane epilogue belongs to the plain form");
  extern __shared__ __attribute__((aligned(16))) double Ms[];
  float amx = 0.f;
  const int tid = threadIdx.x;
  const int lane = tid & 63, wave = tid >> 6;
  const int li = lane & 15, lk = lane >> 4;
  const int by = upper ? (int)(gridDim.y - 1 - blockIdx.y) : (int)blockIdx.y;
  const int c0 = by * 64;
  const int Lc_all = (L + 63) / 64;
  const int Lc = upper ? (Lc_all < by + 1 ? Lc_all : by + 1) : Lc_all;
  const int Le = L < 64 * Lc ? L : 64 * Lc;
  const int64_t ngroups = (rows + 31) / 32;
  const int64_t g0 = (int64_t)blockIdx.x * 4 + wave;
  auto stage = [&](int k0) {
    for (int i = tid; i < KW * 64; i += 256) {
      const int r = i >> 6, c = i & 63;
      Ms[r * PMM_LD + c] = (k0 + r < L && c0 + c < Lo) ? Mx[(int64_t)(k0 + r) * Lo + c0 + c] : 0.0;
    }
  };
  auto fetch = [&](bool valid, int64_t g, int kc, f32x4 (&a)[2][4]) {
#pragma unroll
    for (int t = 0; t < 2; ++t) {
      const int64_t r = 32 * g + (PLANES ? 8 * (li & 3) + 4 * t + (li >> 2) : 16 * t + li);
#pragma unroll
      for (int tt = 0; tt < 4; ++tt) {
        const int k = kc + 16 * tt + 4 * lk;
        if constexpr (GEN)
          a[t][tt] = (valid && r < rows && k < L) ? *reinterpret_cast<const f32x4*>(P + (int64_t)((k >> 6) / cpb) * slab + ((k >> 6) % cpb) * 64 + r * ldp + (k & 63))
                                                 : f32x4{0.f, 0.f, 0.f, 0.f};
        else
          a[t][tt] = (valid && r < rows && k < L) ? *reinterpret_cast<const f32x4*>(P + r * L + k)
                                                 : f32x4{0.f, 0.f, 0.f, 0.f};
      }
    }
  };
  f64x4 acc[2][4];
  auto compute = [&](int64_t g, int kc, int ms0, const f32x4 (&a)[2][4]) {
    if (kc == 0) {
#pragma unroll
      for (int t = 0; t < 2; ++t)
#pragma unroll
        for (int q = 0; q < 4; ++q) acc[t][q] = f64x4{0.0, 0.0, 0.0, 0.0};
    }
#pragma unroll
    for (int tt = 0; tt < 4; ++tt)
#pragma unroll
      for (int c = 0; c < 4; ++c) {
        double b[4];
#pragma unroll
        for (int q = 0; q < 4; ++q) b[q] = Ms[(kc - ms0 + 16 * tt + 4 * lk + c) * PMM_LD + 16 * q + li];
#pragma unroll
        for (int t = 0; t < 2; ++t)
#pragma unroll
          for (int q = 0; q < 4; ++q)
            acc[t][q] = __builtin_amdgcn_mfma_f64_16x16x4f64((double)a[t][tt][c], b[q], acc[t][q], 0, 0, 0);
      }
    if (kc + 64 >= Le) {
#pragma unroll
      for (int t = 0; t < 2; ++t)
#pragma unroll
        for (int r = 0; r < 4; ++r) {
          const int64_t row = 32 * g + (PLANES ? 8 * lk + 4 * t + r : 16 * t + lk + 4 * r);
          if (row >= rows) continue;
#pragma unroll
          for (int q = 0; q < 4; ++q) {
            const int col = c0 + 16 * q + li;
            if (col < Lo) {
              float o_ = (float)acc[t][q][r];
              if constexpr (GEN) {
                if (sub) o_ = (float)((double)sub[row * Lo + col] - acc[t][q][r]);
              }
              out[row * Lo + col] = o_;
              amx = fmaxf(amx, fabsf(o_));
            }
          }
        }
      if constexpr (PLANES) {
        const int64_t k = 32 * g + 8 * lk;
        if (k < plane_rows) {
          const float p_scale = f16_scale_for(plane_bound);
          float m1 = -1.f;
          asm volatile("" : "+v"(m1));
#pragma unroll
          for (int q = 0; q < 4; ++q) {
            const int col = c0 + 16 * q + li;
            u32x4 hi, lo;
#pragma unroll
            for (int t = 0; t < 2; ++t)
#pragma unroll
              for (int r = 0; r < 4; r += 2) {
                const bool in_ = col < Lo && k + 4 * t + r < rows;
                const float v0 = (in_ ? (float)acc[t][q][r] : 0.f) * p_scale;
                const float v1 = (in_ ? (float)acc[t][q][r + 1] : 0.f) * p_scale;
                const fp16x2_t h = cvt_pk_rn(v0, v1);
                fp16x2_t l;
                l[0] = (__fp16)__builtin_fmaf((float)h[0], m1, v0);
                l[1] = (__fp16)__builtin_fmaf((float)h[1], m1, v1);
                hi[2 * t + (r >> 1)] = __builtin_bit_cast(unsigned, h);
                lo[2 * t + (r >> 1)] = __builtin_bit_cast(unsigned, l);
              }
            char* base = reinterpret_cast<char*>(planes) + axb_plane_offset(by, plane_rows, k, 16 * q + li, 0);
            *reinterpret_cast<u32x4*>(base) = hi;
            *reinterpret_cast<u32x4*>(base + AXB_PLANE_BYTES) = lo;
          }
        }
      }
    }
  };
  f32x4 a0[2][4], a1[2][4];
  if (Lc * 64 <= KW) {
    stage(0);
    __syncthreads();
    const int64_t gstride = (int64_t)gridDim.x * 4;
    const int64_t nitems = g0 < ngroups ? ((ngroups - g0 + gstride - 1) / gstride) * Lc : 0;
    fetch(nitems > 0, g0, 0, a0);
    for (int64_t item = 0; item < nitems; item += 2) {
      fetch(item + 1 < nitems, g0 + ((item + 1) / Lc) * gstride, (int)((item + 1) % Lc) * 64, a1);
      __builtin_amdgcn_sched_barrier(0);
      compute(g0 + (item / Lc) * gstride, (int)(item % Lc) * 64, 0, a0);
      if (item + 1 < nitems) {
        fetch(item + 2 < nitems, g0 + ((item + 2) / Lc) * gstride, (int)((item + 2) % Lc) * 64, a0);
        __builtin_amdgcn_sched_barrier(0);
        compute(g0 + ((item + 1) / Lc) * gstride, (int)((item + 1) % Lc) * 64, 0, a1);
      }
    }
  } else {
    const bool active = g0 < ngroups;
    const int wc = KW / 64;
    fetch(active, g0, 0, a0);
    for (int w0 = 0; w0 < Lc; w0 += wc) {
      __syncthreads();
      stage(64 * w0);
      __syncthreads();
      const int we = w0 + wc < Lc ? w0 + wc : Lc;
      for (int ch = w0; ch < we; ch += 2) {
        fetch(active && ch + 1 < Lc, g0, 64 * (ch + 1), a1);
        __builtin_amdgcn_sched_barrier(0);
        if (active) compute(g0, 64 * ch, 64 * w0, a0);
        fetch(active && ch + 2 < Lc, g0, 64 * (ch + 2), a0);
        __builtin_amdgcn_sched_barrier(0);
        if (active && ch + 1 < we) compute(g0, 64 * (ch + 1), 64 * w0, a1);
      }
    }
  }
  if constexpr (PLANES) {
    if (amax_out && blockIdx.x == 0 && blockIdx.y == 0 && tid == 0) *amax_out = __float_as_uint(plane_bound);
  } else if (amax_out) {
    amax_commit(amx, amax_out);
  }
}

__global__ __launch_bounds__(256) void colminmax_part_kernel(const float* __restrict__ P,
                                                             int64_t rows, int L,
                                                             float* __restrict__ pmx,
                                                             float* __restrict__ pmn) {
  __shared__ float smx[16][64], smn[16][64];
  const int tid = threadIdx.x;
  const int cq = tid & 15, rl = tid >> 4;
  const int c = blockIdx.y * 64 + 4 * cq;
  f32x4 mx = {-INFINITY, -INFINITY, -INFINITY, -INFINITY}, mn = {INFINITY, INFINITY, INFINITY, INFINITY};
  if (c < L) {
    const int64_t step = (int64_t)gridDim.x * 16;
    int64_t r = (int64_t)blockIdx.x * 16 + rl;
    for (; r + 7 * step < rows; r += 8 * step) {
      f32x4 v[8];
#pragma unroll
      for (int u = 0; u < 8; ++u) v[u] = *reinterpret_cast<const f32x4*>(P + (r + u * step) * L + c);
#pragma unroll
      for (int u = 0; u < 8; ++u)
#pragma unroll
        for (int e = 0; e < 4; ++e) {
          mx[e] = fmaxf(mx[e], v[u][e]);
          mn[e] = fminf(mn[e], v[u][e]);
        }
    }
    for (; r < rows; r += step) {
      const f32x4 v = *reinterpret_cast<const f32x4*>(P + r * L + c);
#pragma unroll
      for (int e = 0; e < 4; ++e) {
        mx[e] = fmaxf(mx[e], v[e]);
        mn[e] = fminf(mn[e], v[e]);
      }
    }
  }
#pragma unroll
  for (int e = 0; e < 4; ++e) {
    smx[rl][4 * cq + e] = mx[e];
    smn[rl][4 * cq + e] = mn[e];
  }
  __syncthreads();
  if (tid < 64 && blockIdx.y * 64 + tid < L) {
    float a = smx[0][tid], b = smn[0][tid];
    for (int q = 1; q < 16; ++q) {
      a = fmaxf(a, smx[q][tid]);
      b = fminf(b, smn[q][tid]);
    }
    pmx[(int64_t)blockIdx.x * L + blockIdx.y * 64 + tid] = a;
    pmn[(int64_t)blockIdx.x * L + blockIdx.y * 64 + tid] = b;
  }
}
__global__ __launch_bounds__(256) void colminmax_final_kernel(const float* __restrict__ pmx,
                                                              const float* __restrict__ pmn, int nparts, int L,
                                                              float* __restrict__ mx, float* __restrict__ mn) {
  __shared__ float sa[4][64], sb[4][64];
  const int li = threadIdx.x & 63, qq = threadIdx.x >> 6;
  const int c = blockIdx.x * 64 + li;
  float a = -INFINITY, b = INFINITY;
  if (c < L) {
#pragma unroll 8
    for (int q = qq; q < nparts; q += 4) {
      a = fmaxf(a, pmx[(int64_t)q * L + c]);
      b = fminf(b, pmn[(int64_t)q * L + c]);
    }
  }
  sa[qq][li] = a;
  sb[qq][li] = b;
  __syncthreads();
  if (qq == 0 && c < L) {
    mx[c] = fmaxf(fmaxf(sa[0][li], sa[1][li]), fmaxf(sa[2][li], sa[3][li]));
    mn[c] = fminf(fminf(sb[0][li], sb[1][li]), fminf(sb[2][li], sb[3][li]));
  }
}

__global__ __launch_bounds__(256) void panel_export_kernel(const float* __restrict__ P,
                                                           int64_t rows, int L, int k,
                                                           const double* __restrict__ sign,
                                                           float* __restrict__ dst) {
  const int64_t total = rows * k;
  const int64_t stride = (int64_t)gridDim.x * blockDim.x;
  for (int64_t i = (int64_t)blockIdx.x * blockDim.x + threadIdx.x; i < total; i += stride) {
    const int64_t r = i / k;
    const int c = (int)(i - r * k);
    float v = P[r * L + c];
    if (sign) v *= (float)sign[c];
    dst[i] = v;
  }
}
__global__ __launch_bounds__(256) void panel_import_kernel(const float* __restrict__ src,
                                                           int64_t rows, int l,
                                                           float* __restrict__ P, int64_t rows_pad,
                                                           int L, unsigned* __restrict__ amax_out = nullptr) {
  const int l4 = L / 4;
  const int64_t total = rows_pad * l4;
  const int64_t stride = (int64_t)gridDim.x * blockDim.x;
  const bool small = total < ((int64_t)1 << 31);
  float mx = 0.f;
  for (int64_t i = (int64_t)blockIdx.x * blockDim.x + threadIdx.x; i < total; i += stride) {
    int64_t r;
    int c;
    if (small) {
      const unsigned iu = (unsigned)i, ru = iu / (unsigned)l4;
      r = ru;
      c = (int)(iu - ru * (unsigned)l4) * 4;
    } else {
      r = i / l4;
      c = (int)(i - r * l4) * 4;
    }
    f32x4 v = {0.f, 0.f, 0.f, 0.f};
    if (r < rows) {
      const float* sp = src + r * l + c;
#pragma unroll
      for (int e = 0; e < 4; ++e)
        if (c + e < l) v[e] = sp[e];
    }
    reinterpret_cast<f32x4*>(P)[i] = v;
    mx = fmaxf(mx, fmaxf(fmaxf(fabsf(v[0]), fabsf(v[1])), fmaxf(fabsf(v[2]), fabsf(v[3]))));
  }
  if (amax_out) amax_commit(mx, amax_out);
}

__global__ __launch_bounds__(256) void colstats_shift_kernel(const float* __restrict__ X, int64_t n, int64_t P, int64_t ld,
                                                              const int64_t* __restrict__ row_map, float* __restrict__ cshift) {
  const int64_t c = (int64_t)blockIdx.x * 256 + threadIdx.x;
  if (c >= P) return;
  float s = 0.f;
  for (int t = 0; t < 9; ++t) {
    const int64_t r = t == 8 ? n - 1 : (n * t) / 8;
    const float v = X[(row_map ? row_map[r] : r) * ld + c];
    if (fabsf(v) < INFINITY) {
      s = v;
      break;
    }
  }
  cshift[c] = s;
}

__global__ __launch_bounds__(256) void colstats_kernel(const float* __restrict__ X, int64_t n,
                                                        int64_t P, int64_t ld,
                                                        const int64_t* __restrict__ row_map,
                                                        int64_t rows_per_split,
                                                        const float* __restrict__ cshift,
                                                        int* __restrict__ cnt,
                                                        double* __restrict__ sum,
                                                        double* __restrict__ sumsq,
                                                        float* __restrict__ vmin,
                                                        float* __restrict__ vmax) {
  const int64_t c = (int64_t)blockIdx.x * 256 + threadIdx.x;
  if (c >= P) return;
  const int64_t r0 = (int64_t)blockIdx.y * rows_per_split;
  const int64_t r1 = (r0 + rows_per_split < n) ? r0 + rows_per_split : n;
  int k = 0;
  double s = 0.0, q = 0.0;
  const double cs = (double)cshift[c];
  float lo = INFINITY, hi = -INFINITY;
  int64_t r = r0;
  for (; r + 8 <= r1; r += 8) {
    float v[8];
#pragma unroll
    for (int u = 0; u < 8; ++u) {
      const int64_t rr = row_map ? row_map[r + u] : r + u;
      v[u] = __builtin_nontemporal_load(X + rr * ld + c);
    }
#pragma unroll
    for (int u = 0; u < 8; ++u) {
      lo = fminf(lo, v[u]);
      hi = fmaxf(hi, v[u]);
      if (v[u] == v[u]) {
        const double d = (double)v[u] - cs;
        ++k;
        s += d;
        q += d * d;
      }
    }
  }
  for (; r < r1; ++r) {
    const int64_t rr = row_map ? row_map[r] : r;
    const float v = X[rr * ld + c];
    lo = fminf(lo, v);
    hi = fmaxf(hi, v);
    if (v == v) {
      const double d = (double)v - cs;
      ++k;
      s += d;
      q += d * d;
    }
  }
  const int64_t o = (int64_t)blockIdx.y * P + c;
  cnt[o] = k;
  sum[o] = s;
  sumsq[o] = q;
  vmin[o] = lo;
  vmax[o] = hi;
}

__global__ __launch_bounds__(256) void colstats4_kernel(const float* __restrict__ X, int64_t n, int64_t P, int64_t ld,
                                                         const int64_t* __restrict__ row_map, int64_t rows_per_split,
                                                         const float* __restrict__ cshift, int* __restrict__ cnt, double* __restrict__ sum,
                                                         double* __restrict__ sumsq, float* __restrict__ vmin,
                                                         float* __restrict__ vmax) {
  const int64_t c = ((int64_t)blockIdx.x * 256 + threadIdx.x) * 4;
  if (c >= P) return;
  const int64_t r0 = (int64_t)blockIdx.y * rows_per_split;
  const int64_t r1 = (r0 + rows_per_split < n) ? r0 + rows_per_split : n;
  int k[4] = {0, 0, 0, 0};
  double s[4] = {0.0, 0.0, 0.0, 0.0}, q[4] = {0.0, 0.0, 0.0, 0.0};
  float lo[4] = {INFINITY, INFINITY, INFINITY, INFINITY}, hi[4] = {-INFINITY, -INFINITY, -INFINITY, -INFINITY};
  const f32x4 cs4 = *reinterpret_cast<const f32x4*>(cshift + c);
  const double cs[4] = {(double)cs4[0], (double)cs4[1], (double)cs4[2], (double)cs4[3]};
  auto take = [&](const f32x4& v) {
#pragma unroll
    for (int e = 0; e < 4; ++e) {
      lo[e] = fminf(lo[e], v[e]);
      hi[e] = fmaxf(hi[e], v[e]);
      if (v[e] == v[e]) {
        const double d = (double)v[e] - cs[e];
        ++k[e];
        s[e] += d;
        q[e] += d * d;
      }
    }
  };
  int64_t r = r0;
  for (; r + 8 <= r1; r += 8) {
    f32x4 v[8];
#pragma unroll
    for (int u = 0; u < 8; ++u) {
      const int64_t rr = row_map ? row_map[r + u] : r + u;
      v[u] = __builtin_nontemporal_load(reinterpret_cast<const f32x4*>(X + rr * ld + c));
    }
#pragma unroll
    for (int u = 0; u < 8; ++u) take(v[u]);
  }
  for (; r < r1; ++r) {
    const int64_t rr = row_map ? row_map[r] : r;
    take(*reinterpret_cast<const f32x4*>(X + rr * ld + c));
  }
  const int64_t o = (int64_t)blockIdx.y * P + c;
#pragma unroll
  for (int e = 0; e < 4; ++e) {
    cnt[o + e] = k[e];
    sum[o + e] = s[e];
    sumsq[o + e] = q[e];
    vmin[o + e] = lo[e];
    vmax[o + e] = hi[e];
  }
}

__global__ __launch_bounds__(256) void colstats_tr_kernel(const float* __restrict__ X, int64_t n, int64_t P, int64_t ld,
                                                           int64_t rows_per_split, const float* __restrict__ cshift,
                                                           int* __restrict__ cnt, double* __restrict__ sum,
                                                           double* __restrict__ sumsq, float* __restrict__ vmin,
                                                           float* __restrict__ vmax, float* __restrict__ Xt, int64_t n_pad) {
  __shared__ float T[64][65];
  __shared__ double Sd[16][64];
  __shared__ float Sf[16][64];
  const int tid = threadIdx.x, tq = tid & 15, tr = tid >> 4;
  const int64_t c0 = (int64_t)blockIdx.x * 64, cb = c0 + 4 * tq;
  const bool live = cb < P;
  const int64_t rs0 = (int64_t)blockIdx.y * rows_per_split;
  const int64_t rs1 = (rs0 + rows_per_split < n) ? rs0 + rows_per_split : n;
  int k[4] = {0, 0, 0, 0};
  double s[4] = {0.0, 0.0, 0.0, 0.0}, qq[4] = {0.0, 0.0, 0.0, 0.0};
  float lo[4] = {INFINITY, INFINITY, INFINITY, INFINITY}, hi[4] = {-INFINITY, -INFINITY, -INFINITY, -INFINITY};
  const f32x4 cs4 = live ? *reinterpret_cast<const f32x4*>(cshift + cb) : f32x4{0.f, 0.f, 0.f, 0.f};
  const double cs[4] = {(double)cs4[0], (double)cs4[1], (double)cs4[2], (double)cs4[3]};
  for (int64_t r0 = rs0; r0 < rs1; r0 += 64) {
    f32x4 v[4];
#pragma unroll
    for (int q = 0; q < 4; ++q) {
      const int64_t r = r0 + tr + 16 * q;
      v[q] = (live && r < rs1) ? __builtin_nontemporal_load(reinterpret_cast<const f32x4*>(X + r * ld + cb)) : f32x4{0.f, 0.f, 0.f, 0.f};
    }
#pragma unroll
    for (int q = 0; q < 4; ++q) {
      const bool in = live && r0 + tr + 16 * q < rs1;
#pragma unroll
      for (int e = 0; e < 4; ++e) {
        const float x = v[q][e];
        T[tr + 16 * q][4 * tq + e] = x;
        if (in) {
          lo[e] = fminf(lo[e], x);
          hi[e] = fmaxf(hi[e], x);
          if (x == x) {
            const double d = (double)x - cs[e];
            ++k[e];
            s[e] += d;
            qq[e] += d * d;
          }
        }
      }
    }
    __syncthreads();
#pragma unroll
    for (int q = 0; q < 4; ++q) {
      const int cc = tr + 16 * q;
      if (c0 + cc < P) {
        f32x4 o;
#pragma unroll
        for (int e = 0; e < 4; ++e) o[e] = T[4 * tq + e][cc];
        *reinterpret_cast<f32x4*>(Xt + (c0 + cc) * n_pad + r0 + 4 * tq) = o;
      }
// ... 845 lines not shown
```

Baseline: 6032.

## Fuse column extrema into final matmul, fit epilogue, and defer probe sync

The final tall-panel matmul can now also produce per-column min/max partials, so the sign rule reuses them and skips a separate colminmax pass over the panel. When there is a single split, the fit kernel gets an epilogue that performs finalize and reduce in place of the separate fit_finalize and fit_reduce launches. The first-pass probe replaces a stream synchronize with an event, so matrix allocation and the colsum kernels overlap the host wait. The probe kernel's atomics are also reduced per block through shared memory. These changes add template variants and env toggles, and carry a risk of register pressure in the fused kernels.

```diff
diff --git a/xeofs_amd/csrc/eofx_abi.hip b/xeofs_amd/csrc/eofx_abi.hip
--- a/xeofs_amd/csrc/eofx_abi.hip
+++ b/xeofs_amd/csrc/eofx_abi.hip
@@ -862,8 +862,11 @@
   KCHK();
   return EOFX_OK;
 }
+static int launch_colminmax_final(eofx_ctx* ctx, const float* pmx, const float* pmn, int nparts, int L, float* mx, float* mn);
 static int launch_matmul(eofx_ctx* ctx, const float* P, int64_t rows, int L, const double* Mx, int Lo,
-                         float* out, bool upper = false, int64_t planes_rows = 0, float planes_bound = 0.f) {
+                         float* out, bool upper = false, int64_t planes_rows = 0, float planes_bound = 0.f,
+                         float* ext_mxmn = nullptr, int64_t ext_rows = 0, bool* ext_done = nullptr) {
+  if (ext_done) *ext_done = false;
   int KW = (int)std::min<int64_t>(round_up(L, 64), 256);
   if (L > 256) {
     static const int kw_env = std::getenv("EOFX_PMM_KW") ? atoi(std::getenv("EOFX_PMM_KW")) : 0;
@@ -892,6 +895,23 @@
     ++ctx->plane_produced[1];
     return EOFX_OK;
   }
+  if (ext_mxmn && ext_done) {
+    ArenaScope scope(ctx);
+    float* pm = arena_alloc<float>(ctx, 2 * (size_t)grid.x * Lo);
+    if (pm) {
+      float* pn = pm + (size_t)grid.x * Lo;
+      if (smem > 64 * 1024)
+        HIPCHK(hipFuncSetAttribute(reinterpret_cast<const void*>(panel_matmul_kernel<false, false, true>),
+                                   hipFuncAttributeMaxDynamicSharedMemorySize, (int)smem));
+      hipLaunchKernelGGL((panel_matmul_kernel<false, false, true>), grid, dim3(256), smem, ctx->stream, P, rows, L, Mx, Lo, out, KW,
+                         amax_out, (int64_t)0, (int64_t)0, 1, (const float*)nullptr, upper ? 1 : 0, (void*)nullptr, (int64_t)0, 0.f, pm, pn,
+                         ext_rows);
+      KCHK();
+      CHK(launch_colminmax_final(ctx, pm, pn, (int)grid.x, Lo, ext_mxmn, ext_mxmn + Lo));
+      *ext_done = true;
+      return EOFX_OK;
+    }
+  }
   hipLaunchKernelGGL(panel_matmul_kernel<false>, grid, dim3(256), smem, ctx->stream, P, rows, L, Mx, Lo, out, KW, amax_out,
                      (int64_t)0, (int64_t)0, 1, (const float*)nullptr, upper ? 1 : 0);
   KCHK();
@@ -943,6 +963,9 @@
   hipLaunchKernelGGL(colminmax_part_kernel, dim3(nparts, (L + 63) / 64), dim3(256), 0, ctx->stream, P,
                      rows, L, pmx, pmn);
   KCHK();
+  return launch_colminmax_final(ctx, pmx, pmn, nparts, L, mx, mn);
+}
+static int launch_colminmax_final(eofx_ctx* ctx, const float* pmx, const float* pmn, int nparts, int L, float* mx, float* mn) {
   hipLaunchKernelGGL(colminmax_final_kernel, dim3((L + 63) / 64), dim3(256), 0, ctx->stream, pmx, pmn,
                      nparts, L, mx, mn);
   KCHK();
@@ -1921,6 +1944,8 @@
   int Lo;
   std::vector<double> s;
   int64_t tall_pad = 0, small_pad = 0;
+  bool want_tall_extrema = false;
+  float* Tmxmn = nullptr;
 };
 
 extern "C" int eofx_orth_tall_rule(int64_t tall_rows_pad, int L, int prec_power) {
@@ -2148,7 +2173,15 @@
   }
   HIPCHK(hipMemcpyAsync(Md, M1.data(), sizeof(double) * L * Lo, hipMemcpyHostToDevice, ctx->stream));
   HIPCHK(hipMemcpyAsync(Md2, M2.data(), sizeof(double) * L * Lo, hipMemcpyHostToDevice, ctx->stream));
-  CHK(launch_matmul(ctx, Qt, op.tall_pad, L, Md, Lo, Tv));
+  out.Tmxmn = nullptr;
+  if (out.want_tall_extrema) {
+    ARENA(float, mxmn, 2 * (size_t)Lo);
+    bool done = false;
+    CHK(launch_matmul(ctx, Qt, op.tall_pad, L, Md, Lo, Tv, false, 0, 0.f, mxmn, op.tall, &done));
+    if (done) out.Tmxmn = mxmn;
+  } else {
+    CHK(launch_matmul(ctx, Qt, op.tall_pad, L, Md, Lo, Tv));
+  }
   CHK(launch_matmul(ctx, Ws, op.small_pad, L, Md2, Lo, Sv));
   HIPCHK(hipStreamSynchronize(ctx->stream));
   out.Tvec = Tv;
@@ -2161,11 +2194,15 @@
 
 static int comm_allreduce(eofx_ctx* ctx, void* buf, int64_t count, int dtype, int op);
 static int sign_rule(eofx_ctx* ctx, const float* Vpanel, int64_t rows, int Lo, int k,
-                     std::vector<double>& sign, bool over_ranks = false) {
-  ArenaScope scope(ctx);
-  ARENA(float, mx, 2 * (size_t)Lo);
+                     std::vector<double>& sign, bool over_ranks = false, float* known = nullptr) {
+  ArenaScope scope(ctx);
+  float* mx = known;
+  if (!mx) {
+    mx = arena_alloc<float>(ctx, 2 * (size_t)Lo);
+    if (!mx) return set_err(ctx, EOFX_ERR_NOMEM, "arena exhausted (sign rule)");
+    CHK(launch_colminmax(ctx, Vpanel, rows, Lo, mx, mx + Lo));
+  }
   float* mn = mx + Lo;
-  CHK(launch_colminmax(ctx, Vpanel, rows, Lo, mx, mn));
   if (over_ranks) {
     hipLaunchKernelGGL(negate_kernel, dim3(1), dim3(256), 0, ctx->stream, mn, Lo);
     KCHK();
@@ -2180,6 +2217,10 @@
   return EOFX_OK;
 }
 
+static bool sign_extrema_from_producer() {
+  const char* ev = std::getenv("EOFX_SIGN_EXTREMA");
+  return !(ev && atoi(ev) == 0);
+}
 typedef std::function<int(double*, int64_t)> GramReduce;
 static int fix_null_columns(eofx_ctx* ctx, float* P, int64_t rows, int64_t rows_pad, int Lo, int k, int first,
                             const GramReduce* reduce = nullptr, int64_t rows_total = -1) {
@@ -2231,11 +2272,13 @@
 
 static int fix_null_modes(eofx_ctx* ctx, const RsvdOut& ro, int64_t tall, int64_t small, int k,
                           const GramReduce* reduce_tall = nullptr, int64_t tall_total = -1,
-                          const GramReduce* reduce_small = nullptr, int64_t small_total = -1) {
+                          const GramReduce* reduce_small = nullptr, int64_t small_total = -1, bool* touched = nullptr) {
+  if (touched) *touched = false;
   int first_null = k;
   const double s0 = ro.s.empty() ? 0.0 : ro.s[0];
   for (int j = k - 1; j >= 0 && !(ro.s[j] > 1e-5 * s0); --j) first_null = j;
   if (first_null < k && s0 >= 0.0 && std::isfinite(s0) && ro.tall_pad >= tall && ro.small_pad >= small) {
+    if (touched) *touched = true;
     CHK(fix_null_columns(ctx, ro.Tvec, tall, ro.tall_pad, ro.Lo, k, first_null, reduce_tall, tall_total));
     CHK(fix_null_columns(ctx, ro.Svec, small, ro.small_pad, ro.Lo, k, first_null, reduce_small, small_total));
   }
@@ -2253,11 +2296,13 @@
                        std::vector<double>* sign_out = nullptr) {
   const int64_t tall = right_is_tall ? right_rows : left_rows, small = right_is_tall ? left_rows : right_rows;
   const FactorShards local, &sh = shards ? *shards : local;
-  CHK(fix_null_modes(ctx, ro, tall, small, k, sh.reduce_tall, sh.tall_total, sh.reduce_small, sh.small_total));
+  bool touched = false;
+  CHK(fix_null_modes(ctx, ro, tall, small, k, sh.reduce_tall, sh.tall_total, sh.reduce_small, sh.small_total, &touched));
   const float* Rp = right_is_tall ? ro.Tvec : ro.Svec;
   const float* Lp = right_is_tall ? ro.Svec : ro.Tvec;
   std::vector<double> sign;
-  if (flip) CHK(sign_rule(ctx, Rp, right_rows, ro.Lo, k, sign, shards != nullptr));
+  float* known = right_is_tall && !touched && !shards ? ro.Tmxmn : nullptr;
+  if (flip) CHK(sign_rule(ctx, Rp, right_rows, ro.Lo, k, sign, shards != nullptr, known));
   CHK(export_panel(ctx, Lp, left_rows, ro.Lo, k, flip ? sign.data() : nullptr, left));
   CHK(export_panel(ctx, Rp, right_rows, ro.Lo, k, flip ? sign.data() : nullptr, right));
   if (s) {
@@ -2307,6 +2352,7 @@
   std::vector<float> eye;
   const float* om = pl.full_width ? identity_sketch(op.small, pl.l, eye) : omega;
   RsvdOut ro;
+  ro.want_tall_extrema = flip && pl.transposed && sign_extrema_from_producer();
   CHK(rsvd_core(ctx, op, k, pl.l, pl.n_iter, om, ro));
   return rsvd_finish(ctx, ro, pl.transposed, n, p, k, flip, U, s, V);
 }
@@ -2328,10 +2374,12 @@
   eofx_mat* m = nullptr;
   FeatSummary fs;
   hipEvent_t ev[4] = {nullptr, nullptr, nullptr, nullptr};
+  hipEvent_t probe_ev = nullptr;
   static constexpr int NPART = 64;
   ~FitFirst() {
     for (int i = 0; i < 4; ++i)
       if (ev[i]) (void)hipEventDestroy(ev[i]);
+    if (probe_ev) (void)hipEventDestroy(probe_ev);
     if (m) eofx_mat_destroy(ctx, m);
   }
   static size_t bytes(int64_t n, int64_t P, int l) {
@@ -2397,7 +2445,25 @@
     KCHK();
     HIPCHK(hipMemcpyAsync(hword, ps.absmax + 1, sizeof(unsigned), hipMemcpyDeviceToHost, ctx->stream));
     HIPCHK(hipMemcpyAsync(hword + 1, dflags, sizeof(int), hipMemcpyDeviceToHost, ctx->stream));
-    HIPCHK(hipStreamSynchronize(ctx->stream));
+    HIPCHK(hipEventCreateWithFlags(&probe_ev, hipEventDisableTiming));
+    HIPCHK(hipEventRecord(probe_ev, ctx->stream));
+    CHK(mat_alloc(ctx, n, P, &m, false, false));
+    if (pool_malloc(ctx, (void**)&m->aff, sizeof(float) * 3 * (size_t)p_pad) != hipSuccess) {
+      (void)hipGetLastError();
+      m->aff = nullptr;
+      return set_err(ctx, EOFX_ERR_NOMEM, "cannot allocate the affine map");
+    }
+    m->raw = Xd;
+    m->raw_ld = P;
+    m->p_valid = P;
+    return EOFX_OK;
+  }
+  int run(const float* Zs, float* Yt, int LL) {
+    hipLaunchKernelGGL(panel_colsum_part_kernel, dim3(NPART), dim3(256), 0, ctx->stream, Zs, n, LL, wpart);
+    KCHK();
+    hipLaunchKernelGGL(panel_colsum_final_kernel, dim3(1), dim3(256), 0, ctx->stream, wpart, NPART, LL, wbar);
+    KCHK();
+    HIPCHK(hipEventSynchronize(probe_ev));
     float est;
     std::memcpy(&est, hword, sizeof(float));
     maybe_masked = (hword[1] & 2) != 0;
@@ -2408,23 +2474,7 @@
     int e2;
     (void)std::frexp(est, &e2);
     a_scale = std::ldexp(1.f, 14 - e2 - 6);
-    CHK(mat_alloc(ctx, n, P, &m, false, false));
-    if (pool_malloc(ctx, (void**)&m->aff, sizeof(float) * 3 * (size_t)p_pad) != hipSuccess) {
-      (void)hipGetLastError();
-      m->aff = nullptr;
-      return set_err(ctx, EOFX_ERR_NOMEM, "cannot allocate the affine map");
-    }
-    m->raw = Xd;
-    m->raw_ld = P;
-    m->p_valid = P;
     m->masked = maybe_masked;
-    return EOFX_OK;
-  }
-  int run(const float* Zs, float* Yt, int LL) {
-    hipLaunchKernelGGL(panel_colsum_part_kernel, dim3(NPART), dim3(256), 0, ctx->stream, Zs, n, LL, wpart);
-    KCHK();
-    hipLaunchKernelGGL(panel_colsum_final_kernel, dim3(1), dim3(256), 0, ctx->stream, wpart, NPART, LL, wbar);
-    KCHK();
     const float* bmax = amax_get(ctx, Zs);
     if (!bmax) {
       unsigned* bm = ps.absmax + 2;
@@ -2447,12 +2497,21 @@
       HIPCHK(hipEventRecord(p0, ctx->stream));
     }
     const dim3 grid((int)(p_pad / ATB_BM), S, 1);
-    if (LL == 64)
-      hipLaunchKernelGGL(atb_f16_fit_kernel<2>, grid, dim3(256), 0, ctx->stream, Xd, P, (int)n, P, cshift, Zs, LL, part, LL, p_pad, K,
-                         plan.kps, a_scale, bmax, st_sq, st_max, p_pad);
-    else
-      hipLaunchKernelGGL(atb_f16_fit_kernel<1>, grid, dim3(256), 0, ctx->stream, Xd, P, (int)n, P, cshift, Zs, LL, part, LL, p_pad, K,
-                         plan.kps, a_scale, bmax, st_sq, st_max, p_pad);
+    const FitFin fin{Xd, P, n, K - n, P, p_pad, cshift, a_scale, center, standardize, wdev, (double)1.1920928955078125e-07, bmax,
+                     ps.cnt, ps.mean, ps.stdv, ps.shift, ps.scale, ps.m2, m->aff, dcorr, ps.absmax, dflags + 1};
+    bool epilogue = S == 1;
+    if (const char* ev_ = std::getenv("EOFX_FIT_EPILOGUE"))
+      if (atoi(ev_) == 0) epilogue = false;
+#define EOFX_FIT_ARGS Xd, P, (int)n, P, cshift, Zs, LL, part, LL, p_pad, K, plan.kps, a_scale, bmax, st_sq, st_max, p_pad
+    if (epilogue) {
+      const FitEpi epi{fin, l, wbar, amax_new(ctx, Yt)};
+      if (LL == 64) hipLaunchKernelGGL((atb_f16_fit_kernel<2, true>), grid, dim3(256), 0, ctx->stream, EOFX_FIT_ARGS, epi);
+      else hipLaunchKernelGGL((atb_f16_fit_kernel<1, true>), grid, dim3(256), 0, ctx->stream, EOFX_FIT_ARGS, epi);
+    } else {
+      if (LL == 64) hipLaunchKernelGGL((atb_f16_fit_kernel<2, false>), grid, dim3(256), 0, ctx->stream, EOFX_FIT_ARGS, FitNoEpi{});
+      else hipLaunchKernelGGL((atb_f16_fit_kernel<1, false>), grid, dim3(256), 0, ctx->stream, EOFX_FIT_ARGS, FitNoEpi{});
+    }
+#undef EOFX_FIT_ARGS
     KCHK();
     if (ctx->profile) {
       HIPCHK(hipEventRecord(p1, ctx->stream));
@@ -2461,18 +2520,20 @@
       ctx->prof_bytes += (double)n * (double)P * 4.0;
       HIPCHK(hipEventRecord(ev[2], ctx->stream));
     }
-    hipLaunchKernelGGL(fit_finalize_kernel, dim3((int)((p_pad + 255) / 256)), dim3(256), 0, ctx->stream, part, p_pad, LL, st_sq, st_max,
-                       p_pad, S, Xd, P, n, K - n, P, p_pad, cshift, a_scale, center, standardize, wdev,
-                       (double)1.1920928955078125e-07, bmax, ps.cnt, ps.mean, ps.stdv, ps.shift, ps.scale, ps.m2, m->aff, dcorr,
-                       ps.absmax, dflags + 1);
-    KCHK();
+    if (!epilogue) {
+      hipLaunchKernelGGL(fit_finalize_kernel, dim3((int)((p_pad + 255) / 256)), dim3(256), 0, ctx->stream, part, p_pad, LL, st_sq, st_max,
+                         p_pad, S, fin);
+      KCHK();
+    }
     HIPCHK(hipMemcpyAsync(hword + 2, dflags + 1, sizeof(int), hipMemcpyDeviceToHost, ctx->stream));
     HIPCHK(hipMemcpyAsync(hword + 3, ps.absmax, sizeof(unsigned), hipMemcpyDeviceToHost, ctx->stream));
     HIPCHK(hipMemcpyAsync(m->absmax_dev, ps.absmax, sizeof(unsigned), hipMemcpyDeviceToDevice, ctx->stream));
-    hipLaunchKernelGGL(fit_reduce_kernel, dim3((int)std::min<int64_t>((p_pad * (LL / 4) + 255) / 256, 2048)), dim3(256), 0, ctx->stream,
-                       part, Yt, p_pad, LL, l, S, P, dcorr, ps.scale, wbar, amax_new(ctx, Yt),
-                       maybe_masked ? ps.cnt : (const int*)nullptr);
-    KCHK();
+    if (!epilogue) {
+      hipLaunchKernelGGL(fit_reduce_kernel, dim3((int)std::min<int64_t>((p_pad * (LL / 4) + 255) / 256, 2048)), dim3(256), 0, ctx->stream,
+                         part, Yt, p_pad, LL, l, S, P, dcorr, ps.scale, wbar, amax_new(ctx, Yt),
+                         maybe_masked ? ps.cnt : (const int*)nullptr);
+      KCHK();
+    }
     if (ctx->profile) HIPCHK(hipEventRecord(ev[3], ctx->stream));
     CHK(run_feature_summary(ctx, ps, P, fs));
     if (hword[2] & 3) {
@@ -2554,6 +2615,7 @@
   };
   op.bwd_plane_rows = [&](int LL, int pr) { return panel_mul_plane_rows(ctx, m, LL, pr); };
   RsvdOut ro;
+  ro.want_tall_extrema = flip && sign_extrema_from_producer();
   rc = rsvd_core(ctx, op, k, l, n_iter, omega, ro, &first);
   if (rc != EOFX_OK) return rc;
   CHK(rsvd_finish(ctx, ro, true, n, P, k, flip, U, s, V));
diff --git a/xeofs_amd/csrc/eofx_fit.hpp b/xeofs_amd/csrc/eofx_fit.hpp
--- a/xeofs_amd/csrc/eofx_fit.hpp
+++ b/xeofs_amd/csrc/eofx_fit.hpp
@@ -1,4 +1,6 @@
 #pragma once
+#include <type_traits>
+
 #include "eofx_kernels.hpp"
 
 namespace eofx {
@@ -45,16 +47,124 @@
 #pragma unroll
   for (int o = 32; o > 0; o >>= 1) m = fmaxf(m, __shfl_xor(m, o));
   const int anybad = (__any(bad) ? 1 : 0) | (__any(cand) ? 2 : 0);
+  __shared__ float wm_[4];
+  __shared__ int wf_[4];
   if ((threadIdx.x & 63) == 0) {
-    if (m > 0.f) atomicMax(est, __float_as_uint(m));
-    if (anybad) atomicOr(flags, anybad);
+    wm_[threadIdx.x >> 6] = m;
+    wf_[threadIdx.x >> 6] = anybad;
+  }
+  __syncthreads();
+  if (threadIdx.x == 0) {
+    const float mw = fmaxf(fmaxf(wm_[0], wm_[1]), fmaxf(wm_[2], wm_[3]));
+    const int fw = wf_[0] | wf_[1] | wf_[2] | wf_[3];
+    if (mw > 0.f) atomicMax(est, __float_as_uint(mw));
+    if (fw) atomicOr(flags, fw);
   }
 }
 
 constexpr int FIT_FLUSH = 16;
 constexpr float FIT_ONE = 8192.f;
 
-template <int NB>
+struct FitFin {
+  const float* X;
+  int64_t ld, n, extra, P, p_pad;
+  const float* cshift;
+  float a_scale;
+  int center, standardize;
+  const double* weights;
+  double eps;
+  const float* b_absmax;
+  int* cnt;
+  double *mean, *stdv, *shift, *scale, *m2;
+  float* aff;
+  double* dcorr;
+  unsigned* absmax;
+  int* flags;
+};
+__device__ __forceinline__ int fit_finalize_feature(const FitFin& a, int64_t c, double S1, double q, float mx, float& amax,
+                                                    double& d, double& sc_out, bool& alive) {
+  int fl = 0;
+  d = 0.0;
+  sc_out = 0.0;
+  alive = false;
+  const int64_t p_pad = a.p_pad;
+  if (c < a.P) {
+    const double unit = (double)f16_scale_for(*a.b_absmax) / (double)FIT_ONE;
+    S1 *= unit;
+    const float cs = a.cshift[c];
+    if (cs != cs) {
+      if (!(mx < 60000.f)) fl |= 2;
+      fl |= 4;
+      const double w = a.weights ? a.weights[c] : 1.0;
+      a.cnt[c] = 0;
+      a.mean[c] = NAN;
+      a.stdv[c] = NAN;
+      a.shift[c] = a.center ? NAN : 0.0;
+      a.scale[c] = (a.standardize ? NAN : 1.0) * w;
+      a.m2[c] = 0.0;
+      a.dcorr[c] = 0.0;
+      a.aff[c] = 0.f;
+      a.aff[p_pad + c] = 0.f;
+      a.aff[2 * p_pad + c] = 0.f;
+    } else {
+      if (a.extra > 0) {
+        const float v = __builtin_fmaf(a.X[(a.n - 1) * a.ld + c], a.a_scale, -cs * a.a_scale);
+        q -= (double)a.extra * ((double)v * (double)v);
+      }
+      if (!(fabs(S1) < INFINITY) || !(fabs(q) < INFINITY)) fl |= 1;
+      if (!(mx < 60000.f)) fl |= 2;
+      const double ia = 1.0 / (double)a.a_scale;
+      const double nn = (double)a.n;
+      const double mu = (double)cs + S1 / nn;
+      double M2 = q * ia * ia - S1 * S1 / nn;
+      if (!(M2 > 0.0)) M2 = 0.0;
+      double sd = sqrt(M2 / nn);
+      if (a.standardize && sd > a.eps && sd * (double)a.a_scale < 0.015625) fl |= 8;
+      if (sd < a.eps) sd = a.eps;
+      const double w = a.weights ? a.weights[c] : 1.0;
+      const double sh = a.center ? mu : 0.0, sc = (a.standardize ? 1.0 / sd : 1.0) * w;
+      a.cnt[c] = (int)a.n;
+      a.mean[c] = mu;
+      a.stdv[c] = sd;
+      a.shift[c] = sh;
+      a.scale[c] = sc;
+      a.m2[c] = M2;
+      a.dcorr[c] = sh - (double)cs;
+      float hi, lo;
+      aff_split(sh, hi, lo);
+      a.aff[c] = hi;
+      a.aff[p_pad + c] = lo;
+      a.aff[2 * p_pad + c] = (float)sc;
+      amax = fmaxf(amax, (float)(((double)mx * ia + fabs(sh - (double)cs)) * fabs(sc) * 1.000001));
+      d = sh - (double)cs;
+      sc_out = sc;
+      alive = true;
+    }
+  } else if (c < p_pad) {
+    a.aff[c] = 0.f;
+    a.aff[p_pad + c] = 0.f;
+    a.aff[2 * p_pad + c] = 0.f;
+  }
+  return fl;
+}
+__device__ __forceinline__ void fit_finalize_commit(const FitFin& a, float amax, int fl) {
+#pragma unroll
+  for (int o = 32; o > 0; o >>= 1) amax = fmaxf(amax, __shfl_xor(amax, o));
+  const int anyfl = (__any(fl & 1) ? 1 : 0) | (__any(fl & 2) ? 2 : 0) | (__any(fl & 4) ? 4 : 0) | (__any(fl & 8) ? 8 : 0);
+  if ((threadIdx.x & 63) == 0) {
+    if (amax > 0.f && amax < INFINITY) atomicMax(a.absmax, __float_as_uint(amax));
+    if (anyfl) atomicOr(a.flags, anyfl);
+  }
+}
+
+struct FitEpi {
+  FitFin fin;
+  int l;
+  const double* wbar;
+  unsigned* amax_out;
+};
+struct FitNoEpi {};
+template <int NB, bool EPI = false>
 __global__ __launch_bounds__(256, 2) void atb_f16_fit_kernel(const float* __restrict__ A, int64_t lda, int a_rows,
                                                               int64_t a_cols, const float* __restrict__ cshift,
                                                               const float* __restrict__ B, int ldb,
@@ -62,7 +172,8 @@
                                                               int64_t k_per_split, float a_scale,
                                                               const float* __restrict__ b_absmax,
                                                               double* __restrict__ st_sq,
-                                                              float* __restrict__ st_max, int64_t st_ld) {
+                                                              float* __restrict__ st_max, int64_t st_ld,
+                                                              const typename std::conditional<EPI, FitEpi, FitNoEpi>::type epi) {
   __shared__ __attribute__((aligned(16))) _Float16 Bs[2][2][2][32 * NB][8];
   __shared__ double Sq[4][256];
   const int tid = threadIdx.x;
@@ -240,18 +351,12 @@
 #undef EOFX_FIT_STORE_B
 #undef EOFX_FIT_FLUSH
 
-  float* Cs = C + (int64_t)blockIdx.y * M * ldc;
-#pragma unroll
-  for (int j = 0; j < 4; ++j)
-#pragma unroll
-    for (int q = 0; q < NB; ++q)
-#pragma unroll
-      for (int r = 0; r < 16; ++r) {
-        const int ii = (r & 3) + 8 * (r >> 2) + 4 * lh;
-        const int64_t m = m0 + 4 * ii + j;
-        Cs[m * ldc + 32 * q + li] = acc[j][q][r] * out_scale;
-      }
-  {
+  if constexpr (EPI) {
+    double* const eQ = &Sq[0][0];
+    double* const eD = &Sq[2][0];
+    float* const eS1 = reinterpret_cast<float*>(Bsb);
+    float* const eMx = eS1 + ATB_BM;
+    static_assert(ATB_BM == 512 && sizeof(Bs) >= 2 * ATB_BM * sizeof(float), "the epilogue's per-feature words live in Bs");
     f64x4 q4;
     f32x4 m4;
 #pragma unroll
@@ -262,6 +367,93 @@
       q4[j] = q_ + qo_;
       m4[j] = fmaxf(mall, mo_);
     }
+    __syncthreads();
+    if (lh == 0) {
+#pragma unroll
+      for (int j = 0; j < 4; ++j) {
+        eQ[wave * ATB_WM + 4 * li + j] = q4[j];
+        eMx[wave * ATB_WM + 4 * li + j] = m4[j];
+      }
+    }
+    if (li == 31) {
+#pragma unroll
+      for (int j = 0; j < 4; ++j)
+#pragma unroll
+        for (int r = 0; r < 16; ++r) {
+          const int ii = (r & 3) + 8 * (r >> 2) + 4 * lh;
+          eS1[wave * ATB_WM + 4 * ii + j] = acc[j][NB - 1][r] * out_scale;
+        }
+    }
+    __syncthreads();
+    {
+      float amax = 0.f;
+      int fl = 0;
+      for (int h = 0; h < ATB_BM / 256; ++h) {
+        const int f = tid + 256 * h;
+        const int64_t c = (int64_t)blockIdx.x * ATB_BM + f;
+        double S1 = 0.0, q = 0.0;
+        S1 += (double)eS1[f];
+        q += eQ[f];
+        const float mx = fmaxf(0.f, eMx[f]);
+        double d, sc;
+        bool alive;
+        fl |= fit_finalize_feature(epi.fin, c, S1, q, mx, amax, d, sc, alive);
+        eQ[f] = sc;
+        eD[f] = d;
+        eS1[f] = alive ? 1.f : 0.f;
+      }
+      fit_finalize_commit(epi.fin, amax, fl);
+    }
+    __syncthreads();
+    double wb[NB];
+#pragma unroll
+    for (int q = 0; q < NB; ++q) wb[q] = 32 * q + li < epi.l ? epi.wbar[32 * q + li] : 0.0;
+    float mo = 0.f;
+#pragma unroll
+    for (int j = 0; j < 4; ++j)
+#pragma unroll
+      for (int r = 0; r < 16; ++r) {
+        const int ii = (r & 3) + 8 * (r >> 2) + 4 * lh;
+        const int f = wave * ATB_WM + 4 * ii + j;
+        const double d = eD[f], sc = eQ[f];
+        const bool alive = eS1[f] != 0.f;
+#pragma unroll
+        for (int q = 0; q < NB; ++q) {
+          float o = 0.f;
+          if (alive && 32 * q + li < epi.l) {
+            double s = 0.0;
+            s += (double)(acc[j][q][r] * out_scale);
+            o = (float)((s - d * wb[q]) * sc);
+            mo = fmaxf(mo, fabsf(o));
+          }
+          C[(m0 + 4 * ii + j) * ldc + 32 * q + li] = o;
+        }
+      }
+    if (epi.amax_out) amax_commit(mo, epi.amax_out);
+    return;
+  }
+  float* Cs = C + (int64_t)blockIdx.y * M * ldc;
+#pragma unroll
+  for (int j = 0; j < 4; ++j)
+#pragma unroll
+    for (int q = 0; q < NB; ++q)
+#pragma unroll
+      for (int r = 0; r < 16; ++r) {
+        const int ii = (r & 3) + 8 * (r >> 2) + 4 * lh;
+        const int64_t m = m0 + 4 * ii + j;
+        Cs[m * ldc + 32 * q + li] = acc[j][q][r] * out_scale;
+      }
+  {
+    f64x4 q4;
+    f32x4 m4;
+#pragma unroll
+    for (int j = 0; j < 4; ++j) {
+      const double q_ = Sq[j][tid];
+      const double qo_ = __shfl_xor(q_, 32);
+      const float mo_ = __shfl_xor(mall, 32);
+      q4[j] = q_ + qo_;
+      m4[j] = fmaxf(mall, mo_);
+    }
     if (lh == 0 && colok) {
       const int64_t o = (int64_t)blockIdx.y * st_ld + m0 + 4 * li;
       *reinterpret_cast<f64x4*>(st_sq + o) = q4;
@@ -270,85 +462,27 @@
   }
 }
 
-__global__ __launch_bounds__(256) void fit_finalize_kernel(
-    const float* __restrict__ part, int64_t part_rows, int L, const double* __restrict__ st_sq,
-    const float* __restrict__ st_max, int64_t st_ld, int splits, const float* __restrict__ X, int64_t ld, int64_t n,
-    int64_t extra, int64_t P, int64_t p_pad, const float* __restrict__ cshift, float a_scale, int center, int standardize,
-    const double* __restrict__ weights, double eps, const float* __restrict__ b_absmax, int* __restrict__ cnt,
-    double* __restrict__ mean, double* __restrict__ stdv, double* __restrict__ shift, double* __restrict__ scale,
-    double* __restrict__ m2, float* __restrict__ aff, double* __restrict__ dcorr, unsigned* __restrict__ absmax,
-    int* __restrict__ flags) {
+__global__ __launch_bounds__(256) void fit_finalize_kernel(const float* __restrict__ part, int64_t part_rows, int L,
+                                                            const double* __restrict__ st_sq,
+                                                            const float* __restrict__ st_max, int64_t st_ld, int splits,
+                                                            const FitFin a) {
   const int64_t c = (int64_t)blockIdx.x * 256 + threadIdx.x;
   float amax = 0.f;
   int fl = 0;
-  if (c < P) {
-    const double unit = (double)f16_scale_for(*b_absmax) / (double)FIT_ONE;
+  if (c < a.p_pad) {
     double S1 = 0.0, q = 0.0;
     float mx = 0.f;
-    for (int sp = 0; sp < splits; ++sp) {
-      S1 += (double)part[((int64_t)sp * part_rows + c) * L + (L - 1)];
-      q += st_sq[(int64_t)sp * st_ld + c];
-      mx = fmaxf(mx, st_max[(int64_t)sp * st_ld + c]);
-    }
-    S1 *= unit;
-    const float cs = cshift[c];
-    if (cs != cs) {
-      if (!(mx < 60000.f)) fl |= 2;
-      fl |= 4;
-      const double w = weights ? weights[c] : 1.0;
-      cnt[c] = 0;
-      mean[c] = NAN;
-      stdv[c] = NAN;
-      shift[c] = center ? NAN : 0.0;
-      scale[c] = (standardize ? NAN : 1.0) * w;
-      m2[c] = 0.0;
-      dcorr[c] = 0.0;
-      aff[c] = 0.f;
-      aff[p_pad + c] = 0.f;
-      aff[2 * p_pad + c] = 0.f;
-    } else {
-    if (extra > 0) {
-      const float v = __builtin_fmaf(X[(n - 1) * ld + c], a_scale, -cs * a_scale);
-      q -= (double)extra * ((double)v * (double)v);
-    }
-    if (!(fabs(S1) < INFINITY) || !(fabs(q) < INFINITY)) fl |= 1;
-    if (!(mx < 60000.f)) fl |= 2;
-    const double ia = 1.0 / (double)a_scale;
-    const double nn = (double)n;
-    const double mu = (double)cs + S1 / nn;
-    double M2 = q * ia * ia - S1 * S1 / nn;
-    if (!(M2 > 0.0)) M2 = 0.0;
-    double sd = sqrt(M2 / nn);
-    if (standardize && sd > eps && sd * (double)a_scale < 0.015625) fl |= 8;
-    if (sd < eps) sd = eps;
-    const double w = weights ? weights[c] : 1.0;
-    const double sh = center ? mu : 0.0, sc = (standardize ? 1.0 / sd : 1.0) * w;
-    cnt[c] = (int)n;
-    mean[c] = mu;
-    stdv[c] = sd;
-    shift[c] = sh;
-    scale[c] = sc;
-    m2[c] = M2;
-    dcorr[c] = sh - (double)cs;
-    float hi, lo;
-    aff_split(sh, hi, lo);
-    aff[c] = hi;
-    aff[p_pad + c] = lo;
-    aff[2 * p_pad + c] = (float)sc;
-    amax = (float)(((double)mx * ia + fabs(sh - (double)cs)) * fabs(sc) * 1.000001);
-    }
-  } else if (c < p_pad) {
-    aff[c] = 0.f;
-    aff[p_pad + c] = 0.f;
-    aff[2 * p_pad + c] = 0.f;
-  }
-#pragma unroll
-  for (int o = 32; o > 0; o >>= 1) amax = fmaxf(amax, __shfl_xor(amax, o));
-  const int anyfl = (__any(fl & 1) ? 1 : 0) | (__any(fl & 2) ? 2 : 0) | (__any(fl & 4) ? 4 : 0) | (__any(fl & 8) ? 8 : 0);
-  if ((threadIdx.x & 63) == 0) {
-    if (amax > 0.f && amax < INFINITY) atomicMax(absmax, __float_as_uint(amax));
-    if (anyfl) atomicOr(flags, anyfl);
-  }
+    if (c < a.P)
+      for (int sp = 0; sp < splits; ++sp) {
+        S1 += (double)part[((int64_t)sp * part_rows + c) * L + (L - 1)];
+        q += st_sq[(int64_t)sp * st_ld + c];
+        mx = fmaxf(mx, st_max[(int64_t)sp * st_ld + c]);
+      }
+    double d, sc;
+    bool alive;
+    fl = fit_finalize_feature(a, c, S1, q, mx, amax, d, sc, alive);
+  }
+  fit_finalize_commit(a, amax, fl);
 }
 
 __global__ __launch_bounds__(256) void panel_colsum_part_kernel(const float* __restrict__ P, int64_t rows, int L,
diff --git a/xeofs_amd/csrc/eofx_kernels.hpp b/xeofs_amd/csrc/eofx_kernels.hpp
--- a/xeofs_amd/csrc/eofx_kernels.hpp
+++ b/xeofs_amd/csrc/eofx_kernels.hpp
@@ -1380,7 +1380,7 @@
 
 constexpr int PMM_LD = 66;
 
-template <bool GEN = false, bool PLANES = false>
+template <bool GEN = false, bool PLANES = false, bool EXT = false>
 __global__ __launch_bounds__(256) void panel_matmul_kernel(const float* __restrict__ P,
                                                            int64_t rows, int L,
                                                            const double* __restrict__ Mx, int Lo,
@@ -1389,8 +1389,11 @@
                                                            int64_t ldp = 0, int64_t slab = 0, int cpb = 1,
                                                            const float* __restrict__ sub = nullptr, int upper = 0,
                                                            void* __restrict__ planes = nullptr, int64_t plane_rows = 0,
-                                                           float plane_bound = 0.f) {
+                                                           float plane_bound = 0.f, float* __restrict__ ext_mx = nullptr,
+                                                           float* __restrict__ ext_mn = nullptr, int64_t ext_rows = 0) {
   static_assert(!(GEN && PLANES), "the plane epilogue belongs to the plain form");
+  static_assert(!(EXT && (GEN || PLANES)), "the column extrema belong to the plain form");
+  float emx[4] = {-INFINITY, -INFINITY, -INFINITY, -INFINITY}, emn[4] = {INFINITY, INFINITY, INFINITY, INFINITY};
   extern __shared__ __attribute__((aligned(16))) double Ms[];
   float amx = 0.f;
   const int tid = threadIdx.x;
@@ -1463,6 +1466,12 @@
               }
               out[row * Lo + col] = o_;
               amx = fmaxf(amx, fabsf(o_));
+              if constexpr (EXT) {
+                if (row < ext_rows) {
+                  emx[q] = fmaxf(emx[q], o_);
+                  emn[q] = fminf(emn[q], o_);
+                }
+              }
             }
           }
         }
@@ -1538,6 +1547,26 @@
     if (amax_out && blockIdx.x == 0 && blockIdx.y == 0 && tid == 0) *amax_out = __float_as_uint(plane_bound);
   } else if (amax_out) {
     amax_commit(amx, amax_out);
+  }
+  if constexpr (EXT) {
+    __shared__ float exs[2][4][64];
+#pragma unroll
+    for (int q = 0; q < 4; ++q) {
+#pragma unroll
+      for (int o = 16; o < 64; o <<= 1) {
+        emx[q] = fmaxf(emx[q], __shfl_xor(emx[q], o));
+        emn[q] = fminf(emn[q], __shfl_xor(emn[q], o));
+      }
+      if (lk == 0) {
+        exs[0][wave][16 * q + li] = emx[q];
+        exs[1][wave][16 * q + li] = emn[q];
+      }
+    }
+    __syncthreads();
+    if (tid < 64 && c0 + tid < Lo) {
+      ext_mx[(int64_t)blockIdx.x * Lo + c0 + tid] = fmaxf(fmaxf(exs[0][0][tid], exs[0][1][tid]), fmaxf(exs[0][2][tid], exs[0][3][tid]));
+      ext_mn[(int64_t)blockIdx.x * Lo + c0 + tid] = fminf(fminf(exs[1][0][tid], exs[1][1][tid]), fminf(exs[1][2][tid], exs[1][3][tid]));
+    }
   }
 }
 
```

Result: no change. 6067, median of 6 (+0.6%).
